# AIML-IfI/openset-imagenet

Hardware: AMD Instinct MI355X
Metric: images/sec (whole node) ResNet-50 + entropic-open-set, Protocol 2, 1/2/4/8 GPUs (higher is better)
Workload: dtype f32; 1 GPU; Protocol 2, ResNet-50, entropic open-set loss, batch 128/GPU; workload_key=p2, classes=30, batch_per_gpu=128, global_batch=128, image=3x224x224, loss=entropic, optimizer=adam lr=1e-3, parallelism=dp1

## Files before the change

### include/osi.h

```cpp
#ifndef OSI_H
#define OSI_H

#include <stddef.h>

#ifdef __cplusplus
extern "C" {
#endif

#define OSI_OK 0
#define OSI_ERR_ARG (-1)
#define OSI_ERR_LAUNCH (-2)
#define OSI_ERR_STATE (-3)

typedef void* osi_stream_t;

int osi_abi_version(void);
const char* osi_build_arch(void);
const char* osi_strerror(int code);
int osi_set_tuning(const char* name, int value);
int osi_get_tuning(const char* name, int* value);

typedef struct {
    int B, H, W, Cin;
    int Ho, Wo, Cout;
    int R, S, stride, pad;
} osi_conv_desc;

enum { OSI_TILE_AUTO = 0, OSI_TILE_128x128 = 1, OSI_TILE_128x64 = 2, OSI_TILE_64x128 = 3, OSI_TILE_64x64 = 4,
       OSI_TILE_64x64_S1 = 5, OSI_TILE_64x128_S1 = 6, OSI_TILE_128x128_S1 = 7, OSI_TILE_128x64_S1 = 8  };

int osi_conv_fwd(const osi_conv_desc* d, const float* x, const float* w, float* y, int tile, osi_stream_t stream);
size_t osi_conv_fwd_bnstats_workspace(const osi_conv_desc* d);
int osi_conv_fwd_bnstats(const osi_conv_desc* d, const float* x, const float* w, float* y, int tile, float* pstats,
                         size_t pstats_bytes, int* P, int* rows_per_block, osi_stream_t stream);
int osi_conv_fwd_act(const osi_conv_desc* d, const float* x, const float* in_scale, const float* in_shift, const float* w, float* y,
                     int tile, float* pstats, size_t pstats_bytes, int* P, int* rows_per_block, osi_stream_t stream);
int osi_conv_fwd_act2(const osi_conv_desc* d, const float* x, const float* in_scale, const float* in_shift, const float* res,
                      const float* w, float* y, int tile, float* pstats, size_t pstats_bytes, int* P, int* rows_per_block,
                      osi_stream_t stream);
int osi_conv_wino_eligible(const osi_conv_desc* d, int input_gradient);
size_t osi_conv_wino_workspace(const osi_conv_desc* d);
size_t osi_conv_wino_weights_bytes(const osi_conv_desc* d);
size_t osi_conv_wino_slab_bytes(void);
int osi_conv_wino_transform_weights(const osi_conv_desc* d, const float* w, int input_gradient, float* u, size_t u_bytes, osi_stream_t stream);
int osi_conv_fwd_wino_pre(const osi_conv_desc* d, const float* x, const float* in_scale, const float* in_shift, const float* u, float* y,
                          void* slab, size_t slab_bytes, float* pstats, size_t pstats_bytes, int* P, int* rows_per_block, osi_stream_t stream);
int osi_conv_fwd_wino(const osi_conv_desc* d, const float* x, const float* in_scale, const float* in_shift, const float* w, float* y,
                      void* ws, size_t ws_bytes, float* pstats, size_t pstats_bytes, int* P, int* rows_per_block, osi_stream_t stream);
typedef struct {
    const float* scale;
    const float* shift;
    const float* residual;
    int relu;
} osi_conv_epilogue;
size_t osi_conv_fwd_epilogue_workspace(const osi_conv_desc* d);
int osi_conv_fwd_epilogue(const osi_conv_desc* d, const float* x, const float* w, float* out, const osi_conv_epilogue* e, void* ws,
                          size_t ws_bytes, osi_stream_t stream);
int osi_conv_fwd_wino_epilogue_pre(const osi_conv_desc* d, const float* x, const float* u, float* out, const osi_conv_epilogue* e, void* slab,
                                   size_t slab_bytes, osi_stream_t stream);
int osi_conv_dgrad(const osi_conv_desc* d, const float* dy, const float* w, float* dx, int accumulate, int tile,
                   osi_stream_t stream);
typedef struct {
    const void* relu_mask;
    const float* y0;
    const float* mean0;
    const float* invstd0;
    const float* y1;
    const float* mean1;
    const float* invstd1;
    float* partials;
    size_t partials_bytes;
    const float* scale0;
    const float* shift0;
    const void* pool_idx;
    int pool_H, pool_W;
    int addend_stride;
} osi_dgrad_fusion;
size_t osi_conv_dgrad_fused_workspace(const osi_conv_desc* d);
int osi_conv_dgrad_fused(const osi_conv_desc* d, const float* dy, const float* w, float* dx, const float* addend,
                         const osi_dgrad_fusion* f, int tile, int* P, osi_stream_t stream);
int osi_conv_dgrad_fused_frozen(const osi_conv_desc* d, const float* dy, const float* w, float* dx, const osi_dgrad_fusion* f, int tile,
                                int* P, osi_stream_t stream);
int osi_conv_dgrad_fused_wino(const osi_conv_desc* d, const float* dy, const float* w, float* dx, const osi_dgrad_fusion* f, void* ws,
                              size_t ws_bytes, int* P, osi_stream_t stream);
int osi_conv_dgrad_fused_wino_pre(const osi_conv_desc* d, const float* dy, const float* u, float* dx, const osi_dgrad_fusion* f, void* slab,
                                  size_t slab_bytes, int* P, osi_stream_t stream);
size_t osi_conv_wgrad_workspace(const osi_conv_desc* d);
int osi_conv_wgrad(const osi_conv_desc* d, const float* dy, const float* x, float* dw, void* ws, size_t ws_bytes,
                   osi_stream_t stream);
int osi_conv_wgrad_act(const osi_conv_desc* d, const float* dy, const float* x, const float* in_scale, const float* in_shift, float* dw,
                       void* ws, size_t ws_bytes, osi_stream_t stream);
size_t osi_conv_wgrad_wino_workspace(const osi_conv_desc* d);
int osi_conv_wgrad_wino(const osi_conv_desc* d, const float* dy, const float* x, const float* in_scale, const float* in_shift, float* dw,
                        void* ws, size_t ws_bytes, osi_stream_t stream);
int osi_stem_weight_pack(const float* w_krsc3, float* w_packed, int Cout, osi_stream_t stream);
size_t osi_stem_wgrad_direct_workspace(const osi_conv_desc* d);
int osi_stem_wgrad_direct(const osi_conv_desc* d, const float* dy, const float* x4, float* dw_krsc3, void* ws, size_t ws_bytes,
                          osi_stream_t stream);
size_t osi_stem_wgrad_fused_workspace(const osi_conv_desc* d);
int osi_stem_wgrad_fused(const osi_conv_desc* d, const float* gpool, const void* pool_idx, const float* y, const float* x4,
                         const float* gamma, const float* mean, const float* invstd, const float* dgamma, const float* dbeta,
                         float* dw_krsc3, void* ws, size_t ws_bytes, osi_stream_t stream);
int osi_stem_grad_unpack(const float* g_packed, float* g_krsc3, int Cout, osi_stream_t stream);
int osi_stem_dgrad(const float* dy, const float* w_krsc3, float* dx_nchw, int B, int H, int W, osi_stream_t stream);
int osi_stem_dgrad_fgsm(const float* dy, const float* w_krsc3, const float* x_nhwc4, float* x_adv_nhwc4, float eps, float lo, float hi,
                        int B, int H, int W, osi_stream_t stream);

size_t osi_bn_workspace(int M, int C);
int osi_bn_train_stats(const float* y, int M, int C, const float* gamma, const float* beta, float eps, float momentum,
                       float* running_mean, float* running_var, float* mean, float* invstd, float* scale, float* shift,
                       void* ws, size_t ws_bytes, osi_stream_t stream);
int osi_bn_finalize_stats(float* pstats, size_t pstats_bytes, int P, int rows_per_block, int M, int C, const float* gamma,
                          const float* beta, float eps, float momentum, float* running_mean, float* running_var, float* mean,
                          float* invstd, float* scale, float* shift, osi_stream_t stream);
int osi_bn_eval_coeffs(const float* running_mean, const float* running_var, const float* gamma, const float* beta, float eps,
                       int C, float* scale, float* shift, osi_stream_t stream);
#define OSI_BN_MULTI_MAX 64
typedef struct {
    const float *running_mean, *running_var, *gamma, *beta;
    float *scale, *shift;
    int C;
} osi_bn_eval_layer;
int osi_bn_eval_coeffs_multi(const osi_bn_eval_layer* layers, int n, float eps, osi_stream_t stream);
#define OSI_BN_FROZEN_MAX 54
typedef struct {
    const float *running_mean, *running_var, *gamma, *beta;
    float *scale, *shift, *mean, *invstd;
    int C;
} osi_bn_frozen_layer;
int osi_bn_frozen_coeffs_multi(const osi_bn_frozen_layer* layers, int n, float eps, osi_stream_t stream);
int osi_bn_apply(const float* y, const float* residual, const float* scale, const float* shift, float* out, int M, int C,
                 int relu, osi_stream_t stream);
size_t osi_bn_backward_workspace(int M, int C);
int osi_bn_backward(const float* dout, const float* act, const float* y, const float* mean, const float* invstd,
                    const float* gamma, float* dy, float* gmasked, float* dgamma, float* dbeta, int M, int C, void* ws,
                    size_t ws_bytes, osi_stream_t stream);

size_t osi_bn_relu_mask_bytes(int M, int C);
int osi_bn_apply_relu_mask(const float* y, const float* residual, const float* scale, const float* shift, float* out,
                           void* relu_mask, int M, int C, osi_stream_t stream);
int osi_bn_apply_relu_mask2(const float* y, const float* scale, const float* shift, const float* res_y, const float* res_scale,
                            const float* res_shift, float* out, void* relu_mask, int M, int C, osi_stream_t stream);
int osi_bn_backward_relu_mask(const float* dout, const void* relu_mask, const float* y, const float* mean, const float* invstd,
                              const float* gamma, float* dy, float* gmasked, float* dgamma, float* dbeta, int M, int C, void* ws,
                              size_t ws_bytes, osi_stream_t stream);

int osi_bn_backward_fused(const float* g, const float* y, const float* mean, const float* invstd, const float* gamma,
                          const float* psum_g, const float* psum_gx, int P, float* dy, float* dgamma, float* dbeta, int M, int C,
                          void* ws, size_t ws_bytes, osi_stream_t stream);

typedef struct {
    const float *y, *mean, *invstd;
    const float* scale;
    float* dy;
    float *dgamma, *dbeta;
} osi_bn_frozen_consumer;
int osi_bn_backward_frozen(const float* dout, const void* relu_mask, const osi_bn_frozen_consumer* consumers, int n, float* gmasked, int M,
                           int C, void* ws, size_t ws_bytes, osi_stream_t stream);

int osi_nchw3_to_nhwc4(const float* x_nchw, float* y_nhwc4, int B, int H, int W, osi_stream_t stream);
int osi_u8hwc3_to_nhwc4(const unsigned char* x_u8_nhwc, const unsigned char* flip, float* y_nhwc4, int B, int H, int W,
                        osi_stream_t stream);
int osi_u8_crop_flip_to_nhwc4(const unsigned char* canvas_u8, const int* crop_xy, const unsigned char* flip, float* y_nhwc4, int B, int Hc,
                              int Wc, int H, int W, osi_stream_t stream);
int osi_maxpool3x3s2_fwd(const float* x, float* y, void* idx, int B, int H, int W, int C, osi_stream_t stream);
int osi_maxpool3x3s2_bwd(const float* dy, const void* idx, float* dx, int B, int H, int W, int C, osi_stream_t stream);
int osi_bn_backward_reduce(const float* psum_g, const float* psum_gx, int P, float* dgamma, float* dbeta, int M, int C, void* ws,
                           size_t ws_bytes, osi_stream_t stream);
int osi_bn_relu_maxpool_fwd(const float* y, const float* scale, const float* shift, float* pooled, void* idx, int B, int H, int W,
                            int C, osi_stream_t stream);
int osi_bn_relu_maxpool_bwd(const float* gpool, const void* idx, const float* y, const float* mean, const float* invstd,
                            const float* gamma, float* dy, float* dgamma, float* dbeta, int B, int H, int W, int C, void* ws,
                            size_t ws_bytes, osi_stream_t stream);
int osi_bn_relu_maxpool_bwd_frozen(const float* gpool, const void* idx, const float* y, const float* mean, const float* invstd,
                                   const float* scale, float* dy, float* dgamma, float* dbeta, int B, int H, int W, int C, void* ws,
                                   size_t ws_bytes, osi_stream_t stream);
int osi_avgpool_fwd(const float* x, float* y, int B, int HW, int C, osi_stream_t stream);
int osi_avgpool_bwd(const float* dy, float* dx, int B, int HW, int C, osi_stream_t stream);

int osi_linear_fwd(const float* x, const float* w, const float* bias, float* y, int B, int K, int O, osi_stream_t stream);
int osi_linear_bwd(const float* dy, const float* x, const float* w, float* dx, int dx_accumulate, float* dw, float* db, int B,
                   int K, int O, osi_stream_t stream);

enum { OSI_LOSS_ENTROPIC = 0, OSI_LOSS_SOFTMAX = 1, OSI_LOSS_GARBAGE = 2 };
int osi_loss_fwd_bwd(int mode, const float* logits, const long long* target, int B, int C, float unk_weight,
                     long long ignore_index, const float* class_weights, const float* features, int F, float xi, float alpha,
                     float* loss, float* dlogits, float* dfeatures, osi_stream_t stream);
int osi_softmax(const float* logits, float* out, int B, int C, osi_stream_t stream);
int osi_confidence_accumulate(const float* logits, const long long* target, int B, int C, float offset, long long unknown_class,
                              int last_valid_class, double* acc4, osi_stream_t stream);
int osi_confidence_from_scores(const float* scores, const long long* target, int B, int C, float offset, long long unknown_class,
                               int last_valid_class, double* acc4, osi_stream_t stream);

size_t osi_oscr_workspace(int N);
int osi_oscr_f32(const float* scores, const long long* gt, int N, int C, long long unk_label, void* ws, size_t ws_bytes,
                 float* taus, long long* ccr_count, long long* fpr_count, long long* totals, osi_stream_t stream);
int osi_oscr_f64(const double* scores, const long long* gt, int N, int C, long long unk_label, void* ws, size_t ws_bytes,
                 double* taus, long long* ccr_count, long long* fpr_count, long long* totals, osi_stream_t stream);

int osi_adam_step(float* param, const float* grad, float* exp_avg, float* exp_avg_sq, size_t n, double lr, double beta1,
                  double beta2, double eps, long long step, float grad_scale, osi_stream_t stream);
int osi_sgd_step(float* param, const float* grad, float* momentum_buf, size_t n, float lr, float momentum, int first_step,
                 float grad_scale, osi_stream_t stream);
#define OSI_OPT_MAX_SEGMENTS 192
#define OSI_OPT_MAX_GROUPS 16
typedef struct {
    unsigned int begin4, end4;
    int group;
} osi_opt_segment;
typedef struct {
    double lr, beta1, beta2, eps, weight_decay;
    long long step;
    int decoupled;
    int amsgrad, maximize;
} osi_adam_group;
typedef struct {
    double lr, momentum, dampening, weight_decay;
    int nesterov;
    int first_step;
    int maximize;
} osi_sgd_group;
int osi_adam_step_groups(float* param, const float* grad, float* exp_avg, float* exp_avg_sq, float* max_exp_avg_sq, size_t n,
                         const osi_opt_segment* segments, int n_segments, const osi_adam_group* groups, int n_groups,
                         float grad_scale, osi_stream_t stream);
int osi_sgd_step_groups(float* param, const float* grad, float* momentum_buf, size_t n, const osi_opt_segment* segments,
                        int n_segments, const osi_sgd_group* groups, int n_groups, float grad_scale, osi_stream_t stream);
int osi_fill_f32(float* p, size_t n, float value, osi_stream_t stream);
int osi_scale_f32(float* p, size_t n, float s, osi_stream_t stream);
int osi_grad_accumulate(float* dst, const float* src, size_t n, osi_stream_t stream);
int osi_i64_add(long long* p, int n, long long inc, osi_stream_t stream);

typedef struct osi_resnet50* osi_resnet50_t;

int osi_resnet50_create(osi_resnet50_t* out, int B, int H, int W, int fc_dim, int out_features, int logit_bias);
void osi_resnet50_destroy(osi_resnet50_t net);
int osi_resnet50_num_tensors(osi_resnet50_t net);
int osi_resnet50_tensor_info(osi_resnet50_t net, int i, char* name, int name_cap, int* ndim, int* shape, size_t* offset,
                             size_t* numel);
size_t osi_resnet50_param_floats(osi_resnet50_t net);
int osi_resnet50_num_bn(osi_resnet50_t net);
int osi_resnet50_bn_info(osi_resnet50_t net, int j, char* prefix, int cap, int* C, size_t* rm_offset, size_t* rv_offset);
size_t osi_resnet50_buffer_floats(osi_resnet50_t net);
size_t osi_resnet50_workspace_bytes(osi_resnet50_t net);
int osi_resnet50_num_stages(osi_resnet50_t net);
int osi_resnet50_geometry(osi_resnet50_t net, int* B, int* H, int* W);
int osi_resnet50_stage_grad_range(osi_resnet50_t net, int s, size_t* lo, size_t* hi);

int osi_resnet50_stage_input_u8(osi_resnet50_t net, const unsigned char* images_u8_nhwc, const unsigned char* flip,
                                void* workspace, osi_stream_t stream);
int osi_resnet50_bind_input_nhwc4(osi_resnet50_t net, const float* x_nhwc4);
int osi_resnet50_forward(osi_resnet50_t net, const float* params, float* buffers, long long* nbt, const float* image,
                         void* workspace, float* logits, float* features, int training, osi_stream_t stream);
int osi_resnet50_forward_frozen(osi_resnet50_t net, const float* params, const float* buffers, const float* image, void* workspace,
                                float* logits, float* features, osi_stream_t stream);
int osi_resnet50_backward(osi_resnet50_t net, const float* params, float* grads, void* workspace, const float* dlogits,
                          const float* dfeatures, int stage_lo, int stage_hi, osi_stream_t stream);

int osi_resnet50_backward_ex(osi_resnet50_t net, const float* params, float* grads, void* workspace, const float* dlogits,
                             const float* dfeatures, float* dimage, int param_grads, int stage_lo, int stage_hi,
                             osi_stream_t stream);

int osi_resnet50_backward_adv(osi_resnet50_t net, const float* params, float* grads, void* workspace, const float* dlogits,
                              const float* dfeatures, float* x_adv_nhwc4, float eps, float lo, float hi, int stage_lo, int stage_hi,
                              osi_stream_t stream);

int osi_resnet50_grads_ready(osi_resnet50_t net, osi_stream_t main_stream, osi_stream_t waiter_stream);

int osi_resnet50_num_units(osi_resnet50_t net);
int osi_resnet50_tensor_unit(osi_resnet50_t net, int i);
int osi_resnet50_bn_unit(osi_resnet50_t net, int j);
int osi_resnet50_set_trainable(osi_resnet50_t net, unsigned unit_mask, int eval_prefix_units);
int osi_resnet50_get_trainable(osi_resnet50_t net, unsigned* unit_mask, int* eval_prefix_units);

int osi_resnet50_set_option(osi_resnet50_t net, const char* name, int value);

enum { OSI_PROF_START = 0, OSI_PROF_CONV_FWD = 1, OSI_PROF_CONV_DGRAD = 2, OSI_PROF_CONV_WGRAD = 3, OSI_PROF_BN_FWD = 4,
       OSI_PROF_BN_BWD = 5, OSI_PROF_OTHER = 6, OSI_PROF_NCLASS = 7 };
int osi_resnet50_profile(osi_resnet50_t net, int enable);
int osi_resnet50_profile_read(osi_resnet50_t net, double* ms_per_class, int* ops_per_class);
int osi_resnet50_timeline_read(osi_resnet50_t net, double* t_ms, int* cls, int* on_side, int cap, int* count);


int osi_resnet50_debug_num_gates(osi_resnet50_t net);
int osi_resnet50_debug_gate_shape(osi_resnet50_t net, int i, int* C, int* H, int* W);
int osi_resnet50_debug_gate(osi_resnet50_t net, void* workspace, int i, unsigned char* gate_nchw, int* pool_argmax_nchw,
                            osi_stream_t stream);

#ifdef __cplusplus
}
#endif
#endif
```

### openset-imagenet_amd/csrc/abi.hip

```cpp
#include "osi_common.h"

#include <cstring>

OsiTuning g_osi_tuning = { 0,  2048,  1,  1024,  128,  2,  768,  0,  0,  2,  1,  0,  8,  16,  1,  8,  8,  1024,  2048,  1,  1,  1,  1,  1,  1,  1,  2,  0};

namespace {
int* tuning_slot(const char* name) {
    if (!name) return nullptr;
    if (!strcmp(name, "wgrad_tile")) return &g_osi_tuning.wgrad_tile;
    if (!strcmp(name, "wgrad_blocks")) return &g_osi_tuning.wgrad_blocks;
    if (!strcmp(name, "wgrad_nst")) return &g_osi_tuning.wgrad_nst;
    if (!strcmp(name, "bn_grid")) return &g_osi_tuning.bn_grid;
    if (!strcmp(name, "bn_single_p")) return &g_osi_tuning.bn_single_p;
    if (!strcmp(name, "wgrad_group")) return &g_osi_tuning.wgrad_group;
    if (!strcmp(name, "wgrad3")) return &g_osi_tuning.wgrad3;
    if (!strcmp(name, "fwd_wide")) return &g_osi_tuning.fwd_wide;
    if (!strcmp(name, "dgrad_wide")) return &g_osi_tuning.dgrad_wide;
    if (!strcmp(name, "wgrad3_blocks")) return &g_osi_tuning.wgrad3_blocks;
    if (!strcmp(name, "tail_split")) return &g_osi_tuning.tail_split;
    if (!strcmp(name, "tail_cus")) return &g_osi_tuning.tail_cus;
    if (!strcmp(name, "tail_smax")) return &g_osi_tuning.tail_smax;
    if (!strcmp(name, "tail_mint")) return &g_osi_tuning.tail_mint;
    if (!strcmp(name, "stem_direct")) return &g_osi_tuning.stem_direct;
    if (!strcmp(name, "bn_wide_p")) return &g_osi_tuning.bn_wide_p;
    if (!strcmp(name, "bn_grid_bwd")) return &g_osi_tuning.bn_grid_bwd;
    if (!strcmp(name, "tail_gain")) return &g_osi_tuning.tail_gain;
    if (!strcmp(name, "tail_qmax")) return &g_osi_tuning.tail_qmax;
    if (!strcmp(name, "dp_reserved_cus")) return &g_osi_tuning.dp_reserved_cus;
    if (!strcmp(name, "fwd_rows")) return &g_osi_tuning.fwd_rows;
    if (!strcmp(name, "fwd_w3")) return &g_osi_tuning.fwd_w3;
    if (!strcmp(name, "dgrad_w3")) return &g_osi_tuning.dgrad_w3;
    if (!strcmp(name, "fwd_wino")) return &g_osi_tuning.fwd_wino;
    if (!strcmp(name, "dgrad_wino")) return &g_osi_tuning.dgrad_wino;
    if (!strcmp(name, "wino_streamk")) return &g_osi_tuning.wino_streamk;
    if (!strcmp(name, "wgrad_wino")) return &g_osi_tuning.wgrad_wino;
    if (!strcmp(name, "wino_wide")) return &g_osi_tuning.wino_wide;
    return nullptr;
}
}

extern "C" {
int osi_abi_version(void) { return 13; }
int osi_set_tuning(const char* name, int value) {
    int* s = tuning_slot(name);
    if (!s) return OSI_ERR_ARG;
    OsiTuning& t = g_osi_tuning;
    auto in = [&](int lo, int hi) { return value >= lo && value <= hi; };
    bool good = true;
    if (s == &t.wgrad_tile) good = value == 0 || value == 64;
    else if (s == &t.wgrad_blocks || s == &t.wgrad3_blocks) good = in(1, 1 << 20);
    else if (s == &t.wgrad_nst) good = in(1, 2);
    else if (s == &t.bn_grid || s == &t.bn_grid_bwd) good = in(1, 1 << 20);
    else if (s == &t.bn_single_p) good = in(1, 1 << 20);
    else if (s == &t.bn_wide_p) good = in(0, 2048);
    else if (s == &t.wgrad3 || s == &t.wgrad_group) good = in(0, 2);
    else if (s == &t.fwd_wide || s == &t.dgrad_wide || s == &t.tail_split || s == &t.stem_direct || s == &t.fwd_w3 || s == &t.dgrad_w3 || s == &t.fwd_wino || s == &t.dgrad_wino || s == &t.wgrad_wino || s == &t.wino_wide) good = in(0, 1);
    else if (s == &t.wino_streamk) good = in(0, 3);
    else if (s == &t.tail_cus) good = in(0, 4096);
    else if (s == &t.tail_smax) good = in(1, 64);
    else if (s == &t.tail_mint) good = in(1, 4096);
    else if (s == &t.tail_gain) good = in(0, 100);
    else if (s == &t.tail_qmax) good = in(0, 4096);
    else if (s == &t.dp_reserved_cus) good = in(0, 128);
    else if (s == &t.fwd_rows) good = in(0, 2);
    if (!good) return OSI_ERR_ARG;
    *s = value;
    return OSI_OK;
}
int osi_get_tuning(const char* name, int* value) {
    int* s = tuning_slot(name);
    if (!s || !value) return OSI_ERR_ARG;
    *value = *s;
    return OSI_OK;
}
const char* osi_build_arch(void) { return "gfx950"; }
const char* osi_strerror(int code) {
    switch (code) {
        case OSI_OK: return "ok";
        case OSI_ERR_ARG: return "invalid argument (shape, pointer or alignment precondition)";
        case OSI_ERR_LAUNCH: return "HIP launch failed";
        case OSI_ERR_STATE: return "executor called out of order, or a plan-relevant tuning knob changed after osi_resnet50_create";
        default: return "unknown error";
    }
}
}
```

### openset-imagenet_amd/csrc/bn.hip

```cpp
#include "osi_common.h"

namespace {

constexpr int NT = 256;
constexpr int OSI_BN_GROUPS = 32;

struct RowSplit { int CV, RL, G; };
__host__ __device__ inline RowSplit row_split(int C) {
    RowSplit s;
    int c4 = C / 4;
    s.CV = c4 < NT ? c4 : NT;
    s.RL = NT / s.CV;
    s.G = (c4 + s.CV - 1) / s.CV;
    return s;
}

__global__ __launch_bounds__(NT) void k_bn_stats_partial(const float* __restrict__ y, int M, int C, int rows_per_blk,
                                                        float* __restrict__ pmean, float* __restrict__ pm2) {
    const int P = gridDim.x;
    __shared__ f32x4 red[2][NT];
    const RowSplit sp = row_split(C);
    const int tid = threadIdx.x;
    const int cv = tid % sp.CV, rl = tid / sp.CV;
    const int r0 = blockIdx.x * rows_per_blk;
    const int r1 = min(M, r0 + rows_per_blk);
    const float n = (float)(r1 - r0);
    const bool active = rl < sp.RL;
    for (int g = 0; g < sp.G; ++g) {
        const int c4 = g * sp.CV + cv;
        const bool colok = active && c4 * 4 < C;
        f32x4 s1 = {0, 0, 0, 0}, s2 = {0, 0, 0, 0}, shift = {0, 0, 0, 0};
        if (colok) {
            const f32x4* base = reinterpret_cast<const f32x4*>(y) + c4;
            const size_t ld = C / 4;
            shift = base[(size_t)r0 * ld];
            int r = r0 + rl;
            for (; r + 3 * sp.RL < r1; r += 4 * sp.RL) {
                f32x4 v0 = base[(size_t)r * ld], v1 = base[(size_t)(r + sp.RL) * ld];
                f32x4 v2 = base[(size_t)(r + 2 * sp.RL) * ld], v3 = base[(size_t)(r + 3 * sp.RL) * ld];
                v0 -= shift; v1 -= shift; v2 -= shift; v3 -= shift;
                s1 += (v0 + v1) + (v2 + v3);
                s2 += (v0 * v0 + v1 * v1) + (v2 * v2 + v3 * v3);
            }
            for (; r < r1; r += sp.RL) {
                f32x4 v = base[(size_t)r * ld] - shift;
                s1 += v; s2 += v * v;
            }
        }
        red[0][tid] = s1; red[1][tid] = s2;
        __syncthreads();
        if (colok && rl == 0) {
            for (int k = 1; k < sp.RL; ++k) { s1 += red[0][k * sp.CV + cv]; s2 += red[1][k * sp.CV + cv]; }
            f32x4 mean = shift + s1 / n;
            f32x4 m2 = s2 - s1 * s1 / n;
#pragma unroll
            for (int k = 0; k < 4; ++k) {
                pmean[(size_t)(c4 * 4 + k) * P + blockIdx.x] = mean[k];
                pm2[(size_t)(c4 * 4 + k) * P + blockIdx.x] = m2[k];
            }
        }
        __syncthreads();
    }
}

__device__ __forceinline__ void bn_finish(int c, float mean, float m2, int M, const float* gamma, const float* beta, float eps,
                                          float momentum, float* running_mean, float* running_var, float* mean_out,
                                          float* invstd_out, float* scale_out, float* shift_out) {
    float var = m2 / (float)M;
    float invstd = 1.0f / sqrtf(var + eps);
    mean_out[c] = mean; invstd_out[c] = invstd;
    float sc = invstd * gamma[c];
    scale_out[c] = sc; shift_out[c] = beta[c] - mean * sc;
    if (running_mean) {
        float unb = M > 1 ? m2 / (float)(M - 1) : var;
        running_mean[c] = (1.f - momentum) * running_mean[c] + momentum * mean;
        running_var[c] = (1.f - momentum) * running_var[c] + momentum * unb;
    }
}
__global__ __launch_bounds__(NT) void k_bn_stats_final_rows(const float* __restrict__ pmean, const float* __restrict__ pm2, int P,
                                                           int rows_per_blk, int M, int C, const float* __restrict__ gamma,
                                                           const float* __restrict__ beta, float eps, float momentum,
                                                           float* running_mean, float* running_var, float* __restrict__ mean_out,
                                                           float* __restrict__ invstd_out, float* __restrict__ scale_out,
                                                           float* __restrict__ shift_out) {
    __shared__ float red[16][16];
    __shared__ float smean[16];
    const int cl = threadIdx.x & 15, pl = threadIdx.x >> 4;
    const int c = blockIdx.x * 16 + cl;
    const bool ok = c < C;
    const int last = P - 1;
    const float nfull = (float)rows_per_blk, nlast = (float)(M - last * rows_per_blk);
    float a0 = 0.f, a1 = 0.f;
    if (ok) {
        int b = pl;
        for (; b + 16 < P; b += 32) {
            a0 += (b == last ? nlast : nfull) * pmean[(size_t)b * C + c];
            a1 += (b + 16 == last ? nlast : nfull) * pmean[(size_t)(b + 16) * C + c];
        }
        if (b < P) a0 += (b == last ? nlast : nfull) * pmean[(size_t)b * C + c];
    }
    red[pl][cl] = a0 + a1;
    __syncthreads();
    if (pl == 0) {
        float s = 0.f;
        for (int k = 0; k < 16; ++k) s += red[k][cl];
        smean[cl] = s / (float)M;
    }
    __syncthreads();
    const float mean = smean[cl];
    a0 = 0.f; a1 = 0.f;
    if (ok) {
        int b = pl;
        for (; b + 16 < P; b += 32) {
            const float d0 = pmean[(size_t)b * C + c] - mean, d1 = pmean[(size_t)(b + 16) * C + c] - mean;
            a0 += pm2[(size_t)b * C + c] + (b == last ? nlast : nfull) * d0 * d0;
            a1 += pm2[(size_t)(b + 16) * C + c] + (b + 16 == last ? nlast : nfull) * d1 * d1;
        }
        if (b < P) { const float d0 = pmean[(size_t)b * C + c] - mean; a0 += pm2[(size_t)b * C + c] + (b == last ? nlast : nfull) * d0 * d0; }
    }
    __syncthreads();
    red[pl][cl] = a0 + a1;
    __syncthreads();
    if (pl == 0 && ok) {
        float m2 = 0.f;
        for (int k = 0; k < 16; ++k) m2 += red[k][cl];
        bn_finish(c, mean, m2, M, gamma, beta, eps, momentum, running_mean, running_var, mean_out, invstd_out, scale_out, shift_out);
    }
}
constexpr int WPL = 64;
__device__ __forceinline__ float wide_reduce(float (*red)[16], float v, int pl, int cl) {
    red[pl][cl] = v;
    __syncthreads();
    float t = 0.f;
    if (pl < 4) {
#pragma unroll
        for (int k = 0; k < 16; ++k) t += red[pl * 16 + k][cl];
    }
    __syncthreads();
    if (pl < 4) red[pl][cl] = t;
    __syncthreads();
    if (pl == 0) t = (red[0][cl] + red[1][cl]) + (red[2][cl] + red[3][cl]);
    __syncthreads();
    return t;
}
__global__ __launch_bounds__(16 * WPL) void k_bn_stats_final_wide(const float* __restrict__ pmean, const float* __restrict__ pm2, int P,
                                                                 int rows_per_blk, int M, int C, const float* __restrict__ gamma,
                                                                 const float* __restrict__ beta, float eps, float momentum,
                                                                 float* running_mean, float* running_var, float* __restrict__ mean_out,
                                                                 float* __restrict__ invstd_out, float* __restrict__ scale_out,
                                                                 float* __restrict__ shift_out) {
    __shared__ float red[WPL][16];
    const int cl = threadIdx.x & 15, pl = threadIdx.x >> 4;
    const int c = min(blockIdx.x * 16 + cl, C - 1);
    const bool ok = blockIdx.x * 16 + cl < C;
    const int last = P - 1;
    const float nfull = (float)rows_per_blk, nlast = (float)(M - last * rows_per_blk);
    const float* pa = pmean + c;
    const float* pb = pm2 + c;
    const float pv = wide_reduce(red, pa[(size_t)min(pl, last) * C], pl, cl) * (1.f / WPL);
    if (pl == 0) red[0][cl] = pv;
    __syncthreads();
    const float pvv = red[0][cl];
    __syncthreads();
    float s1a = 0.f, s1b = 0.f, s2a = 0.f, s2b = 0.f;
    int b = pl;
    for (; b + 3 * WPL < P; b += 4 * WPL) {
        const float m0 = pa[(size_t)b * C], m1 = pa[(size_t)(b + WPL) * C], m2_ = pa[(size_t)(b + 2 * WPL) * C], m3 = pa[(size_t)(b + 3 * WPL) * C];
        const float q0 = pb[(size_t)b * C], q1 = pb[(size_t)(b + WPL) * C], q2 = pb[(size_t)(b + 2 * WPL) * C], q3 = pb[(size_t)(b + 3 * WPL) * C];
        const float d0 = m0 - pvv, d1 = m1 - pvv, d2 = m2_ - pvv, d3 = m3 - pvv;
        const float n3 = b + 3 * WPL == last ? nlast : nfull;
        s1a += nfull * d0; s1b += nfull * d1; s1a += nfull * d2; s1b += n3 * d3;
        s2a += q0 + nfull * d0 * d0; s2b += q1 + nfull * d1 * d1; s2a += q2 + nfull * d2 * d2; s2b += q3 + n3 * d3 * d3;
    }
    for (; b < P; b += WPL) {
        const float d = pa[(size_t)b * C] - pvv, n = b == last ? nlast : nfull;
        s1a += n * d; s2a += pb[(size_t)b * C] + n * d * d;
    }
    const float S1 = wide_reduce(red, s1a + s1b, pl, cl);
    const float S2 = wide_reduce(red, s2a + s2b, pl, cl);
    if (pl == 0 && ok) {
        const float mean = pvv + S1 / (float)M;
        const float m2 = fmaxf(S2 - S1 * S1 / (float)M, 0.f);
        bn_finish(c, mean, m2, M, gamma, beta, eps, momentum, running_mean, running_var, mean_out, invstd_out, scale_out, shift_out);
    }
}
__global__ __launch_bounds__(NT) void k_bn_stats_group(const float* __restrict__ pmean, const float* __restrict__ pm2, int P, int Pc,
                                                      int rows_per_blk, int M, int C, int S, float* __restrict__ gmean,
                                                      float* __restrict__ gm2) {
    __shared__ float red[2][16][16];
    const int cl = threadIdx.x & 15, pl = threadIdx.x >> 4;
    const int c = min(blockIdx.x * 16 + cl, C - 1), s = blockIdx.y;
    const bool ok = blockIdx.x * 16 + cl < C;
    const int b0 = s * Pc, b1 = min(P, b0 + Pc), last = P - 1;
    const float nfull = (float)rows_per_blk, nlast = (float)(M - last * rows_per_blk);
    const float ng = (float)(min(M, b1 * rows_per_blk) - b0 * rows_per_blk);
    const float* pa = pmean + c;
    const float* pb = pm2 + c;
    red[0][pl][cl] = pa[(size_t)min(b0 + pl, b1 - 1) * C];
    __syncthreads();
    float pv = 0.f;
#pragma unroll
    for (int k = 0; k < 16; ++k) pv += red[0][k][cl];
    pv *= 1.f / 16.f;
    __syncthreads();
    float s1a = 0.f, s1b = 0.f, s2a = 0.f, s2b = 0.f;
    int b = b0 + pl;
    for (; b + 48 < b1; b += 64) {
        const float m0 = pa[(size_t)b * C], m1 = pa[(size_t)(b + 16) * C], m2_ = pa[(size_t)(b + 32) * C], m3 = pa[(size_t)(b + 48) * C];
        const float q0 = pb[(size_t)b * C], q1 = pb[(size_t)(b + 16) * C], q2 = pb[(size_t)(b + 32) * C], q3 = pb[(size_t)(b + 48) * C];
        const float d0 = m0 - pv, d1 = m1 - pv, d2 = m2_ - pv, d3 = m3 - pv;
        const float n3 = b + 48 == last ? nlast : nfull;
        s1a += nfull * d0; s1b += nfull * d1; s1a += nfull * d2; s1b += n3 * d3;
        s2a += q0 + nfull * d0 * d0; s2b += q1 + nfull * d1 * d1; s2a += q2 + nfull * d2 * d2; s2b += q3 + n3 * d3 * d3;
    }
    for (; b < b1; b += 16) {
        const float d = pa[(size_t)b * C] - pv, n = b == last ? nlast : nfull;
        s1a += n * d; s2a += pb[(size_t)b * C] + n * d * d;
    }
    red[0][pl][cl] = s1a + s1b; red[1][pl][cl] = s2a + s2b;
    __syncthreads();
    if (pl == 0 && ok) {
        float S1 = 0.f, S2 = 0.f;
#pragma unroll
        for (int k = 0; k < 16; ++k) { S1 += red[0][k][cl]; S2 += red[1][k][cl]; }
        gmean[(size_t)c * S + s] = pv + S1 / ng;
        gm2[(size_t)c * S + s] = fmaxf(S2 - S1 * S1 / ng, 0.f);
    }
}
__global__ __launch_bounds__(NT) void k_bn_stats_final(const float* __restrict__ pmean, const float* __restrict__ pm2, int P,
                                                      int rows_per_blk, int M, int C, const float* __restrict__ gamma,
                                                      const float* __restrict__ beta, float eps, float momentum,
                                                      float* running_mean, float* running_var, float* __restrict__ mean_out,
                                                      float* __restrict__ invstd_out, float* __restrict__ scale_out,
                                                      float* __restrict__ shift_out) {
    const int lane = threadIdx.x & 63;
    const int c = blockIdx.x * (NT / 64) + (threadIdx.x >> 6);
    if (c >= C) return;
    float n = 0.f, mean = 0.f, m2 = 0.f;
    for (int b = lane; b < P; b += 64) {
        const float nb = (float)min(rows_per_blk, M - b * rows_per_blk);
        chan_merge(n, mean, m2, nb, pmean[(size_t)c * P + b], pm2[(size_t)c * P + b]);
    }
#pragma unroll
    for (int o = 1; o < 64; o <<= 1) {
        const float nb = __shfl_xor(n, o, 64), mb = __shfl_xor(mean, o, 64), sb = __shfl_xor(m2, o, 64);
        if (lane & o) { float na = nb, ma = mb, sa = sb; chan_merge(na, ma, sa, n, mean, m2); n = na; mean = ma; m2 = sa; }
        else chan_merge(n, mean, m2, nb, mb, sb);
    }
    if (lane == 0)
        bn_finish(c, mean, m2, M, gamma, beta, eps, momentum, running_mean, running_var, mean_out, invstd_out, scale_out, shift_out);
}

__global__ void k_bn_eval_coeffs(const float* rm, const float* rv, const float* gamma, const float* beta, float eps, int C,
                                 float* scale, float* shift) {
    int c = blockIdx.x * blockDim.x + threadIdx.x;
    if (c >= C) return;
    float sc = gamma[c] * (1.0f / sqrtf(rv[c] + eps));
    scale[c] = sc; shift[c] = beta[c] - rm[c] * sc;
}

struct BnEvalTable { osi_bn_eval_layer l[OSI_BN_MULTI_MAX]; };
__global__ void k_bn_eval_coeffs_multi(BnEvalTable t, float eps) {
    const osi_bn_eval_layer& L = t.l[blockIdx.y];
    const int c = blockIdx.x * blockDim.x + threadIdx.x;
    if (c >= L.C) return;
    const float sc = L.gamma[c] * (1.0f / sqrtf(L.running_var[c] + eps));
    L.scale[c] = sc; L.shift[c] = L.beta[c] - L.running_mean[c] * sc;
}

struct BnFrozenTable { osi_bn_frozen_layer l[OSI_BN_FROZEN_MAX]; };
__global__ void k_bn_frozen_coeffs_multi(BnFrozenTable t, float eps) {
    const osi_bn_frozen_layer& L = t.l[blockIdx.y];
    const int c = blockIdx.x * blockDim.x + threadIdx.x;
    if (c >= L.C) return;
    const float is = 1.0f / sqrtf(L.running_var[c] + eps);
    const float sc = L.gamma[c] * is;
    L.scale[c] = sc; L.shift[c] = L.beta[c] - L.running_mean[c] * sc;
    L.mean[c] = L.running_mean[c]; L.invstd[c] = is;
}

typedef unsigned long long u64;
#ifndef OSI_BN_REVERSE
#define OSI_BN_REVERSE 3
#endif
template <int RES, bool RELU, bool BITS>
__global__ __launch_bounds__(NT) void k_bn_apply(const f32x4* __restrict__ y, const f32x4* __restrict__ res,
                                                const f32x4* __restrict__ scale, const f32x4* __restrict__ shift,
                                                const f32x4* __restrict__ rscale, const f32x4* __restrict__ rshift,
                                                f32x4* __restrict__ out, u64* __restrict__ bits, size_t n4, int c4n) {
    const size_t nq = (n4 + NT - 1) / NT;
    for (size_t q = blockIdx.x; q < nq; q += gridDim.x) {
        const size_t i = ((OSI_BN_REVERSE & 1) ? nq - 1 - q : q) * NT + threadIdx.x;
        if (i >= n4) continue;
        int c4 = (int)(i % (size_t)c4n);
        const f32x4 yv = __builtin_nontemporal_load(y + i), sc = scale[c4], sh = shift[c4];
        f32x4 v;
#pragma unroll
        for (int e = 0; e < 4; ++e) v[e] = __builtin_fmaf(yv[e], sc[e], sh[e]);
        if (RES == 1) v += __builtin_nontemporal_load(res + i);
        if (RES == 2) {
            const f32x4 rv = __builtin_nontemporal_load(res + i), rs = rscale[c4], rh = rshift[c4];
            f32x4 t;
#pragma unroll
            for (int e = 0; e < 4; ++e) t[e] = __builtin_fmaf(rv[e], rs[e], rh[e]);
            v += t;
        }
        if (BITS) {
            const u64 b0 = __ballot(v.x > 0.f), b1 = __ballot(v.y > 0.f), b2 = __ballot(v.z > 0.f), b3 = __ballot(v.w > 0.f);
            if ((threadIdx.x & 63) == 0) {
                u64* w = bits + (i >> 6) * 4;
                w[0] = b0; w[1] = b1; w[2] = b2; w[3] = b3;
            }
        }
        if (RELU) { v.x = fmaxf(v.x, 0.f); v.y = fmaxf(v.y, 0.f); v.z = fmaxf(v.z, 0.f); v.w = fmaxf(v.w, 0.f); }
        out[i] = v;
    }
}
__device__ __forceinline__ f32x4 mask_by_bits(f32x4 g, const u64* __restrict__ bits, size_t i) {
    const u64* w = bits + (i >> 6) * 4;
    const int b = (int)(i & 63);
    g.x = (w[0] >> b) & 1 ? g.x : 0.f; g.y = (w[1] >> b) & 1 ? g.y : 0.f;
    g.z = (w[2] >> b) & 1 ? g.z : 0.f; g.w = (w[3] >> b) & 1 ? g.w : 0.f;
    return g;
}

template <int MODE>
__device__ __forceinline__ f32x4 masked(f32x4 gv, const void* m, size_t i) {
    if (MODE == 1) {
        f32x4 a = reinterpret_cast<const f32x4*>(m)[i];
        gv.x = a.x > 0.f ? gv.x : 0.f; gv.y = a.y > 0.f ? gv.y : 0.f;
        gv.z = a.z > 0.f ? gv.z : 0.f; gv.w = a.w > 0.f ? gv.w : 0.f;
    } else if (MODE == 2) {
        gv = mask_by_bits(gv, reinterpret_cast<const u64*>(m), i);
    }
    return gv;
}
struct PoolSrc {
    const uint32_t* idx;
    FastDiv dW, dH;
    int H, W, Ho, Wo;
};
__device__ __forceinline__ f32x4 pool_gather(const f32x4* __restrict__ gp, const PoolSrc& ps, uint32_t pix, int c4, int c4n) {
    const uint32_t row = fdiv(pix, ps.dW);
    const int w = (int)(pix - row * ps.dW.d);
    const uint32_t b = fdiv(row, ps.dH);
    const int h = (int)(row - b * ps.dH.d);
    f32x4 acc = {0, 0, 0, 0};
    for (int ho = h >> 1; ho <= (h + 1) >> 1; ++ho) {
        if (ho >= ps.Ho) continue;
        const int r = h - (ho * 2 - 1);
        for (int wo = w >> 1; wo <= (w + 1) >> 1; ++wo) {
            if (wo >= ps.Wo) continue;
            const int s = w - (wo * 2 - 1);
            const size_t o = ((size_t)(b * ps.Ho + ho) * ps.Wo + wo) * c4n + c4;
            const uint32_t id = ps.idx[o];
            const f32x4 g = gp[o];
            const uint32_t me = (uint32_t)(r * 3 + s) | 0x80u;
#pragma unroll
            for (int k = 0; k < 4; ++k)
                if (((id >> (8 * k)) & 0xffu) == me) acc[k] += g[k];
        }
    }
    return acc;
}

template <int MODE>
__global__ __launch_bounds__(NT) void k_bn_bwd_partial(const float* __restrict__ dA, const void* __restrict__ msk,
                                                      const float* __restrict__ y, const float* __restrict__ mean,
                                                      const float* __restrict__ invstd, int M, int C, int rows_per_blk,
                                                      float* __restrict__ pdb, float* __restrict__ pdg, PoolSrc ps) {
    __shared__ f32x4 red[2][NT];
    const int P = gridDim.x;
    const RowSplit sp = row_split(C);
    const int tid = threadIdx.x;
    const int cv = tid % sp.CV, rl = tid / sp.CV;
    const int r0 = blockIdx.x * rows_per_blk;
    const int r1 = min(M, r0 + rows_per_blk);
    const bool active = rl < sp.RL;
    const size_t ld = C / 4;
    for (int g = 0; g < sp.G; ++g) {
        const int c4 = g * sp.CV + cv;
        const bool colok = active && c4 * 4 < C;
        f32x4 sb = {0, 0, 0, 0}, sg = {0, 0, 0, 0}, sb2 = {0, 0, 0, 0}, sg2 = {0, 0, 0, 0};
        if (colok) {
            const f32x4 mu = reinterpret_cast<const f32x4*>(mean)[c4];
            const f32x4 is = reinterpret_cast<const f32x4*>(invstd)[c4];
            const f32x4* pd = reinterpret_cast<const f32x4*>(dA);
            const f32x4* py = reinterpret_cast<const f32x4*>(y);
            int r = r0 + rl;
            for (; r + sp.RL < r1; r += 2 * sp.RL) {
                const size_t i0 = (size_t)r * ld + c4, i1 = (size_t)(r + sp.RL) * ld + c4;
                f32x4 g0, g1, y0 = py[i0], y1 = py[i1];
                if (MODE == 3) {
                    g0 = pool_gather(pd, ps, (uint32_t)r, c4, (int)ld); g1 = pool_gather(pd, ps, (uint32_t)(r + sp.RL), c4, (int)ld);
                } else {
                    g0 = masked<MODE>(pd[i0], msk, i0); g1 = masked<MODE>(pd[i1], msk, i1);
                }
                sb += g0; sg += g0 * ((y0 - mu) * is);
                sb2 += g1; sg2 += g1 * ((y1 - mu) * is);
            }
            for (; r < r1; r += sp.RL) {
                const size_t i0 = (size_t)r * ld + c4;
                f32x4 g0 = MODE == 3 ? pool_gather(pd, ps, (uint32_t)r, c4, (int)ld) : masked<MODE>(pd[i0], msk, i0);
                sb += g0; sg += g0 * ((py[i0] - mu) * is);
            }
            sb += sb2; sg += sg2;
        }
        red[0][tid] = sb; red[1][tid] = sg;
        __syncthreads();
        if (colok && rl == 0) {
            for (int k = 1; k < sp.RL; ++k) { sb += red[0][k * sp.CV + cv]; sg += red[1][k * sp.CV + cv]; }
#pragma unroll
            for (int k = 0; k < 4; ++k) {
                pdb[(size_t)(c4 * 4 + k) * P + blockIdx.x] = sb[k];
                pdg[(size_t)(c4 * 4 + k) * P + blockIdx.x] = sg[k];
            }
        }
        __syncthreads();
    }
}

__global__ __launch_bounds__(NT) void k_bn_bwd_final(const float* __restrict__ pdb, const float* __restrict__ pdg, int P, int M,
                                                    int C, float* __restrict__ dgamma, float* __restrict__ dbeta,
                                                    float* __restrict__ c1, float* __restrict__ c2) {
    const int lane = threadIdx.x & 63;
    const int c = blockIdx.x * (NT / 64) + (threadIdx.x >> 6);
    if (c >= C) return;
    float ab = 0.f, ag = 0.f;
    for (int b = lane; b < P; b += 64) { ab += pdb[(size_t)c * P + b]; ag += pdg[(size_t)c * P + b]; }
    ab = wave_sum(ab); ag = wave_sum(ag);
    if (lane == 0) {
        dbeta[c] = ab; dgamma[c] = ag;
        c1[c] = ab / (float)M; c2[c] = ag / (float)M;
    }
}

__global__ __launch_bounds__(NT) void k_colsum2_group(const float* __restrict__ a, const float* __restrict__ b, int P, int Pc, int C,
                                                     int S, float* __restrict__ ga, float* __restrict__ gb) {
    __shared__ float ra[16][16], rb[16][16];
    const int cl = threadIdx.x & 15, pl = threadIdx.x >> 4;
    const int c = min(blockIdx.x * 16 + cl, C - 1), s = blockIdx.y;
    const bool ok = blockIdx.x * 16 + cl < C;
    const int b0 = s * Pc, b1 = min(P, b0 + Pc);
    const float* pa = a + c;
    const float* pb = b + c;
    float xa0 = 0.f, xa1 = 0.f, xb0 = 0.f, xb1 = 0.f;
    int r = b0 + pl;
    for (; r + 48 < b1; r += 64) {
        const float a0 = pa[(size_t)r * C], a1 = pa[(size_t)(r + 16) * C], a2 = pa[(size_t)(r + 32) * C], a3 = pa[(size_t)(r + 48) * C];
        const float v0 = pb[(size_t)r * C], v1 = pb[(size_t)(r + 16) * C], v2 = pb[(size_t)(r + 32) * C], v3 = pb[(size_t)(r + 48) * C];
        xa0 += a0; xa1 += a1; xa0 += a2; xa1 += a3;
        xb0 += v0; xb1 += v1; xb0 += v2; xb1 += v3;
    }
    for (; r < b1; r += 16) { xa0 += pa[(size_t)r * C]; xb0 += pb[(size_t)r * C]; }
    float xa = xa0 + xa1, xb = xb0 + xb1;
    ra[pl][cl] = xa; rb[pl][cl] = xb;
    __syncthreads();
    if (pl == 0 && ok) {
        for (int k = 1; k < 16; ++k) { xa += ra[k][cl]; xb += rb[k][cl]; }
        ga[(size_t)c * S + s] = xa; gb[(size_t)c * S + s] = xb;
    }
}

__global__ __launch_bounds__(16 * WPL) void k_bn_bwd_final_wide(const float* __restrict__ a, const float* __restrict__ b, int P, int M, int C,
                                                               float* __restrict__ dgamma, float* __restrict__ dbeta,
                                                               float* __restrict__ c1, float* __restrict__ c2) {
    __shared__ float red[WPL][16];
    const int cl = threadIdx.x & 15, pl = threadIdx.x >> 4;
    const int c = min(blockIdx.x * 16 + cl, C - 1);
    const bool ok = blockIdx.x * 16 + cl < C;
    const float* pa = a + c;
    const float* pb = b + c;
    float xa0 = 0.f, xa1 = 0.f, xb0 = 0.f, xb1 = 0.f;
    int r = pl;
    for (; r + 3 * WPL < P; r += 4 * WPL) {
        const float a0 = pa[(size_t)r * C], a1 = pa[(size_t)(r + WPL) * C], a2 = pa[(size_t)(r + 2 * WPL) * C], a3 = pa[(size_t)(r + 3 * WPL) * C];
        const float b0 = pb[(size_t)r * C], b1 = pb[(size_t)(r + WPL) * C], b2 = pb[(size_t)(r + 2 * WPL) * C], b3 = pb[(size_t)(r + 3 * WPL) * C];
        xa0 += a0; xa1 += a1; xa0 += a2; xa1 += a3;
        xb0 += b0; xb1 += b1; xb0 += b2; xb1 += b3;
    }
    for (; r < P; r += WPL) { xa0 += pa[(size_t)r * C]; xb0 += pb[(size_t)r * C]; }
    const float sa = wide_reduce(red, xa0 + xa1, pl, cl);
    const float sb = wide_reduce(red, xb0 + xb1, pl, cl);
    if (pl == 0 && ok) {
        dbeta[c] = sa; dgamma[c] = sb;
        c1[c] = sa / (float)M; c2[c] = sb / (float)M;
    }
}

template <int MODE, bool EMITG>
__global__ __launch_bounds__(NT) void k_bn_bwd_apply(const f32x4* dA , const void* __restrict__ msk,
                                                    const f32x4* __restrict__ y, const f32x4* __restrict__ mean,
                                                    const f32x4* __restrict__ invstd, const f32x4* __restrict__ gamma,
                                                    const f32x4* __restrict__ c1, const f32x4* __restrict__ c2,
                                                    f32x4* dy, f32x4* __restrict__ gout, size_t n4, int c4n, PoolSrc ps) {
    const size_t nq = (n4 + NT - 1) / NT;
    for (size_t q = blockIdx.x; q < nq; q += gridDim.x) {
        const size_t i = ((OSI_BN_REVERSE & 2) ? nq - 1 - q : q) * NT + threadIdx.x;
        if (i >= n4) continue;
        int c4 = (int)(i % (size_t)c4n);
        f32x4 gv = MODE == 3 ? pool_gather(dA, ps, (uint32_t)(i / (size_t)c4n), c4, c4n) : masked<MODE>(__builtin_nontemporal_load(dA + i), msk, i);
        f32x4 is = invstd[c4];
        f32x4 xh = (__builtin_nontemporal_load(y + i) - mean[c4]) * is;
        f32x4 r = (gv - c1[c4] - xh * c2[c4]) * (gamma[c4] * is);
        if (EMITG) gout[i] = gv;
        dy[i] = r;
    }
}

template <int MODE, bool EMITG, bool TWO>
__global__ __launch_bounds__(NT) void k_bn_frozen_apply(const f32x4* dA, const void* __restrict__ msk, const f32x4* __restrict__ scale0,
                                                       const f32x4* __restrict__ scale1, f32x4* dy0, f32x4* __restrict__ dy1,
                                                       f32x4* __restrict__ gout, size_t n4, int c4n, PoolSrc ps) {
    const size_t nq = (n4 + NT - 1) / NT;
    for (size_t q = blockIdx.x; q < nq; q += gridDim.x) {
        const size_t i = ((OSI_BN_REVERSE & 2) ? nq - 1 - q : q) * NT + threadIdx.x;
        if (i >= n4) continue;
        const int c4 = (int)(i % (size_t)c4n);
        const f32x4 gv = MODE == 3 ? pool_gather(dA, ps, (uint32_t)(i / (size_t)c4n), c4, c4n) : masked<MODE>(__builtin_nontemporal_load(dA + i), msk, i);
        if (EMITG) gout[i] = gv;
        if (TWO) dy1[i] = gv * scale1[c4];
        dy0[i] = gv * scale0[c4];
    }
}

static int rows_per_block(int M, int C, int& P) {
    long rows = (256l * 1024) / ((long)C * 4);
    if (rows < 8) rows = 8;
    long minrows = (M + 1023) / 1024;
    if (rows < minrows) rows = minrows;
    if (rows > M) rows = M;
    P = (int)((M + rows - 1) / rows);
    return (int)rows;
}
static int stream_grid(size_t n4, bool backward = false) {
    const size_t cap = (size_t)(backward ? g_osi_tuning.bn_grid_bwd : g_osi_tuning.bn_grid);
    size_t g = (n4 + NT - 1) / NT;
    return (int)(g > cap ? cap : g);
}

}

extern "C" {

size_t osi_bn_workspace(int M, int C) {
    if (M <= 0 || C <= 0) return 0;
    int P;
    rows_per_block(M, C, P);
    return (size_t)2 * P * C * sizeof(float);
}

int osi_bn_train_stats(const float* y, int M, int C, const float* gamma, const float* beta, float eps, float momentum,
                       float* running_mean, float* running_var, float* mean, float* invstd, float* scale, float* shift,
                       void* ws, size_t ws_bytes, osi_stream_t stream) {
    OSI_REQUIRE(y && gamma && beta && mean && invstd && scale && shift && ws);
    OSI_REQUIRE(M > 0 && C > 0 && C % 4 == 0);
    OSI_REQUIRE((running_mean == nullptr) == (running_var == nullptr));
    int P;
    int rpb = rows_per_block(M, C, P);
    OSI_REQUIRE(ws_bytes >= (size_t)2 * P * C * sizeof(float));
    hipStream_t st = (hipStream_t)stream;
    float* pmean = (float*)ws;
    float* pm2 = pmean + (size_t)P * C;
    hipLaunchKernelGGL(k_bn_stats_partial, dim3(P), dim3(NT), 0, st, y, M, C, rpb, pmean, pm2);
    OSI_LAUNCH_CHECK();
    hipLaunchKernelGGL(k_bn_stats_final, dim3(osi_cdiv(C, NT / 64)), dim3(NT), 0, st, pmean, pm2, P, rpb, M, C, gamma, beta, eps,
                       momentum, running_mean, running_var, mean, invstd, scale, shift);
    OSI_LAUNCH_CHECK();
    return OSI_OK;
}

int osi_bn_finalize_stats(float* pstats, size_t pstats_bytes, int P, int rows_per_block, int M, int C, const float* gamma,
                          const float* beta, float eps, float momentum, float* running_mean, float* running_var, float* mean,
                          float* invstd, float* scale, float* shift, osi_stream_t stream) {
    OSI_REQUIRE(pstats && gamma && beta && mean && invstd && scale && shift);
    OSI_REQUIRE(P > 0 && rows_per_block > 0 && M > 0 && C > 0 && (long)(P - 1) * rows_per_block < M && (long)P * rows_per_block >= M);
    OSI_REQUIRE((running_mean == nullptr) == (running_var == nullptr));
    OSI_REQUIRE(pstats_bytes >= ((size_t)2 * P * C + 2 * (size_t)OSI_BN_GROUPS * C) * sizeof(float));
    hipStream_t st = (hipStream_t)stream;
    const float* pmean = pstats;
    const float* pm2 = pstats + (size_t)P * C;
    if (P <= g_osi_tuning.bn_single_p) {
        hipLaunchKernelGGL(k_bn_stats_final_rows, dim3(osi_cdiv(C, 16)), dim3(NT), 0, st, pmean, pm2, P, rows_per_block, M, C, gamma,
                           beta, eps, momentum, running_mean, running_var, mean, invstd, scale, shift);
        OSI_LAUNCH_CHECK();
        return OSI_OK;
    }
    if (P <= g_osi_tuning.bn_wide_p) {
        hipLaunchKernelGGL(k_bn_stats_final_wide, dim3(osi_cdiv(C, 16)), dim3(16 * WPL), 0, st, pmean, pm2, P, rows_per_block, M, C, gamma,
                           beta, eps, momentum, running_mean, running_var, mean, invstd, scale, shift);
        OSI_LAUNCH_CHECK();
        return OSI_OK;
    }
    int S = osi_cdiv(P, 64);
    if (S > OSI_BN_GROUPS) S = OSI_BN_GROUPS;
    const int Pc = osi_cdiv(P, S);
    S = osi_cdiv(P, Pc);
    float* gmean = pstats + (size_t)2 * P * C;
    float* gm2 = gmean + (size_t)S * C;
    hipLaunchKernelGGL(k_bn_stats_group, dim3(osi_cdiv(C, 16), S), dim3(NT), 0, st, pmean, pm2, P, Pc, rows_per_block, M, C, S, gmean, gm2);
    OSI_LAUNCH_CHECK();
    hipLaunchKernelGGL(k_bn_stats_final, dim3(osi_cdiv(C, NT / 64)), dim3(NT), 0, st, (const float*)gmean, (const float*)gm2, S,
                       Pc * rows_per_block, M, C, gamma, beta, eps, momentum, running_mean, running_var, mean, invstd, scale, shift);
    OSI_LAUNCH_CHECK();
    return OSI_OK;
}

int osi_bn_eval_coeffs(const float* running_mean, const float* running_var, const float* gamma, const float* beta, float eps,
                       int C, float* scale, float* shift, osi_stream_t stream) {
    OSI_REQUIRE(running_mean && running_var && gamma && beta && scale && shift && C > 0);
    hipLaunchKernelGGL(k_bn_eval_coeffs, dim3(osi_cdiv(C, 256)), dim3(256), 0, (hipStream_t)stream, running_mean, running_var,
                       gamma, beta, eps, C, scale, shift);
    OSI_LAUNCH_CHECK();
    return OSI_OK;
}

int osi_bn_eval_coeffs_multi(const osi_bn_eval_layer* layers, int n, float eps, osi_stream_t stream) {
    OSI_REQUIRE(layers && n > 0 && n <= OSI_BN_MULTI_MAX);
    BnEvalTable t{};
    int cmax = 0;
    for (int i = 0; i < n; ++i) {
        const osi_bn_eval_layer& L = layers[i];
        OSI_REQUIRE(L.running_mean && L.running_var && L.gamma && L.beta && L.scale && L.shift && L.C > 0);
        t.l[i] = L;
        if (L.C > cmax) cmax = L.C;
    }
    hipLaunchKernelGGL(k_bn_eval_coeffs_multi, dim3(osi_cdiv(cmax, 256), n), dim3(256), 0, (hipStream_t)stream, t, eps);
    OSI_LAUNCH_CHECK();
    return OSI_OK;
}

int osi_bn_frozen_coeffs_multi(const osi_bn_frozen_layer* layers, int n, float eps, osi_stream_t stream) {
    OSI_REQUIRE(layers && n > 0 && n <= OSI_BN_FROZEN_MAX);
    BnFrozenTable t{};
    int cmax = 0;
    for (int i = 0; i < n; ++i) {
        const osi_bn_frozen_layer& L = layers[i];
        OSI_REQUIRE(L.running_mean && L.running_var && L.gamma && L.beta && L.scale && L.shift && L.mean && L.invstd && L.C > 0);
        t.l[i] = L;
        if (L.C > cmax) cmax = L.C;
    }
    hipLaunchKernelGGL(k_bn_frozen_coeffs_multi, dim3(osi_cdiv(cmax, 256), n), dim3(256), 0, (hipStream_t)stream, t, eps);
    OSI_LAUNCH_CHECK();
    return OSI_OK;
}

static int bn_apply_impl(const float* y, const float* residual, const float* scale, const float* shift, float* out, void* bits,
                         int M, int C, int relu, hipStream_t st, const float* rscale = nullptr, const float* rshift = nullptr) {
    OSI_REQUIRE(y && scale && shift && out && M > 0 && C > 0 && C % 4 == 0);
    OSI_REQUIRE(!bits || relu);
    OSI_REQUIRE((rscale == nullptr) == (rshift == nullptr) && (!rscale || (residual && bits)));
    const size_t n4 = (size_t)M * C / 4;
    const int grid = stream_grid(n4), c4n = C / 4;
    auto Y = (const f32x4*)y; auto R = (const f32x4*)residual; auto S = (const f32x4*)scale; auto H = (const f32x4*)shift;
    auto RS = (const f32x4*)rscale; auto RH = (const f32x4*)rshift;
    auto O = (f32x4*)out; auto B = (u64*)bits;
#define OSI_APPLY(RES_, RELU_, BITS_) hipLaunchKernelGGL((k_bn_apply<RES_, RELU_, BITS_>), dim3(grid), dim3(NT), 0, st, Y, R, S, H, RS, RH, O, B, n4, c4n)
    if (rscale) OSI_APPLY(2, true, true);
    else if (bits && residual) OSI_APPLY(1, true, true);
    else if (bits) OSI_APPLY(0, true, true);
    else if (residual && relu) OSI_APPLY(1, true, false);
    else if (residual) OSI_APPLY(1, false, false);
    else if (relu) OSI_APPLY(0, true, false);
    else OSI_APPLY(0, false, false);
#undef OSI_APPLY
    OSI_LAUNCH_CHECK();
    return OSI_OK;
}

int osi_bn_apply(const float* y, const float* residual, const float* scale, const float* shift, float* out, int M, int C,
                 int relu, osi_stream_t stream) {
    return bn_apply_impl(y, residual, scale, shift, out, nullptr, M, C, relu, (hipStream_t)stream);
}

size_t osi_bn_relu_mask_bytes(int M, int C) {
    if (M <= 0 || C <= 0) return 0;
    const size_t n4 = (size_t)M * C / 4;
    return (n4 + 63) / 64 * 4 * sizeof(u64);
}

int osi_bn_apply_relu_mask(const float* y, const float* residual, const float* scale, const float* shift, float* out,
                           void* relu_mask, int M, int C, osi_stream_t stream) {
    OSI_REQUIRE(relu_mask);
    return bn_apply_impl(y, residual, scale, shift, out, relu_mask, M, C, 1, (hipStream_t)stream);
}

int osi_bn_apply_relu_mask2(const float* y, const float* scale, const float* shift, const float* res_y, const float* res_scale,
                            const float* res_shift, float* out, void* relu_mask, int M, int C, osi_stream_t stream) {
    OSI_REQUIRE(relu_mask && res_y && res_scale && res_shift);
    return bn_apply_impl(y, res_y, scale, shift, out, relu_mask, M, C, 1, (hipStream_t)stream, res_scale, res_shift);
}

static int bn_backward_impl(const float* dout, const void* msk, int mode, const float* y, const float* mean, const float* invstd,
                            const float* gamma, float* dy, float* gmasked, float* dgamma, float* dbeta, int M, int C, void* ws,
                            size_t ws_bytes, hipStream_t st, PoolSrc ps = PoolSrc{}) {
    OSI_REQUIRE(dout && y && mean && invstd && gamma && (dy || mode == 3) && dgamma && dbeta && ws);
    OSI_REQUIRE(M > 0 && C > 0 && C % 4 == 0);
    int P;
    int rpb = rows_per_block(M, C, P);
    OSI_REQUIRE(ws_bytes >= ((size_t)2 * P * C + 2 * (size_t)C) * sizeof(float));
    float* pdb = (float*)ws;
    float* pdg = pdb + (size_t)P * C;
    float* c1 = pdg + (size_t)P * C;
    float* c2 = c1 + C;
    if (mode == 3) hipLaunchKernelGGL(k_bn_bwd_partial<3>, dim3(P), dim3(NT), 0, st, dout, msk, y, mean, invstd, M, C, rpb, pdb, pdg, ps);
    else if (mode == 2) hipLaunchKernelGGL(k_bn_bwd_partial<2>, dim3(P), dim3(NT), 0, st, dout, msk, y, mean, invstd, M, C, rpb, pdb, pdg, ps);
    else if (mode == 1) hipLaunchKernelGGL(k_bn_bwd_partial<1>, dim3(P), dim3(NT), 0, st, dout, msk, y, mean, invstd, M, C, rpb, pdb, pdg, ps);
    else hipLaunchKernelGGL(k_bn_bwd_partial<0>, dim3(P), dim3(NT), 0, st, dout, msk, y, mean, invstd, M, C, rpb, pdb, pdg, ps);
    OSI_LAUNCH_CHECK();
    hipLaunchKernelGGL(k_bn_bwd_final, dim3(osi_cdiv(C, NT / 64)), dim3(NT), 0, st, pdb, pdg, P, M, C, dgamma, dbeta, c1, c2);
    OSI_LAUNCH_CHECK();
    if (!dy) return OSI_OK;
    const size_t n4 = (size_t)M * C / 4;
    const int grid = stream_grid(n4, true), c4n = C / 4;
    auto D = (const f32x4*)dout; auto Y = (const f32x4*)y;
    auto MU = (const f32x4*)mean; auto IS = (const f32x4*)invstd; auto G = (const f32x4*)gamma;
    auto C1 = (const f32x4*)c1; auto C2 = (const f32x4*)c2;
    auto DY = (f32x4*)dy; auto GO = (f32x4*)gmasked;
#define OSI_BWD_APPLY(MODE_, EMIT_) hipLaunchKernelGGL((k_bn_bwd_apply<MODE_, EMIT_>), dim3(grid), dim3(NT), 0, st, D, msk, Y, MU, IS, G, C1, C2, DY, GO, n4, c4n, ps)
    if (mode == 3) OSI_BWD_APPLY(3, false);
    else if (mode == 2) { if (gmasked) OSI_BWD_APPLY(2, true); else OSI_BWD_APPLY(2, false); }
    else if (mode == 1) { if (gmasked) OSI_BWD_APPLY(1, true); else OSI_BWD_APPLY(1, false); }
    else { if (gmasked) OSI_BWD_APPLY(0, true); else OSI_BWD_APPLY(0, false); }
#undef OSI_BWD_APPLY
    OSI_LAUNCH_CHECK();
    return OSI_OK;
}

static int bwd_reduce_partials(const float* psum_g, const float* psum_gx, int P, int M, int C, float* gb, float* gg, int S, int Pc,
                               float* dgamma, float* dbeta, float* c1, float* c2, hipStream_t st) {
    if (P <= g_osi_tuning.bn_wide_p) {
        hipLaunchKernelGGL(k_bn_bwd_final_wide, dim3(osi_cdiv(C, 16)), dim3(16 * WPL), 0, st, psum_g, psum_gx, P, M, C, dgamma, dbeta, c1, c2);
        OSI_LAUNCH_CHECK();
        return OSI_OK;
    }
    hipLaunchKernelGGL(k_colsum2_group, dim3(osi_cdiv(C, 16), S), dim3(NT), 0, st, psum_g, psum_gx, P, Pc, C, S, gb, gg);
    OSI_LAUNCH_CHECK();
    hipLaunchKernelGGL(k_bn_bwd_final, dim3(osi_cdiv(C, NT / 64)), dim3(NT), 0, st, (const float*)gb, (const float*)gg, S, M, C, dgamma,
                       dbeta, c1, c2);
    OSI_LAUNCH_CHECK();
    return OSI_OK;
}

int osi_bn_backward_fused(const float* g, const float* y, const float* mean, const float* invstd, const float* gamma,
                          const float* psum_g, const float* psum_gx, int P, float* dy, float* dgamma, float* dbeta, int M, int C,
                          void* ws, size_t ws_bytes, osi_stream_t stream) {
    OSI_REQUIRE(g && y && mean && invstd && gamma && psum_g && psum_gx && dy && dgamma && dbeta && ws);
    OSI_REQUIRE(M > 0 && C > 0 && C % 4 == 0 && P > 0);
    int S = osi_cdiv(P, 64);
    if (S > OSI_BN_GROUPS) S = OSI_BN_GROUPS;
    const int Pc = osi_cdiv(P, S);
    S = osi_cdiv(P, Pc);
    OSI_REQUIRE(ws_bytes >= ((size_t)2 * S * C + 2 * (size_t)C) * sizeof(float));
    hipStream_t st = (hipStream_t)stream;
    float* gb = (float*)ws;
    float* gg = gb + (size_t)S * C;
    float* c1 = gg + (size_t)S * C;
    float* c2 = c1 + C;
    if (int e = bwd_reduce_partials(psum_g, psum_gx, P, M, C, gb, gg, S, Pc, dgamma, dbeta, c1, c2, st)) return e;
    const size_t n4 = (size_t)M * C / 4;
    hipLaunchKernelGGL((k_bn_bwd_apply<0, false>), dim3(stream_grid(n4, true)), dim3(NT), 0, st, (const f32x4*)g, (const void*)nullptr,
                       (const f32x4*)y, (const f32x4*)mean, (const f32x4*)invstd, (const f32x4*)gamma, (const f32x4*)c1,
                       (const f32x4*)c2, (f32x4*)dy, (f32x4*)nullptr, n4, C / 4, PoolSrc{});
    OSI_LAUNCH_CHECK();
    return OSI_OK;
}

int osi_bn_backward_reduce(const float* psum_g, const float* psum_gx, int P, float* dgamma, float* dbeta, int M, int C, void* ws,
                           size_t ws_bytes, osi_stream_t stream) {
    OSI_REQUIRE(psum_g && psum_gx && dgamma && dbeta && ws && M > 0 && C > 0 && P > 0);
    int S = osi_cdiv(P, 64);
    if (S > OSI_BN_GROUPS) S = OSI_BN_GROUPS;
    const int Pc = osi_cdiv(P, S);
    S = osi_cdiv(P, Pc);
    OSI_REQUIRE(ws_bytes >= ((size_t)2 * S * C + 2 * (size_t)C) * sizeof(float));
    hipStream_t st = (hipStream_t)stream;
    float* gb = (float*)ws;
    float* gg = gb + (size_t)S * C;
    float* c1 = gg + (size_t)S * C;
    float* c2 = c1 + C;
    if (int e = bwd_reduce_partials(psum_g, psum_gx, P, M, C, gb, gg, S, Pc, dgamma, dbeta, c1, c2, st)) return e;
    return OSI_OK;
}

static int bn_frozen_impl(const float* dout, const void* msk, int mode, const osi_bn_frozen_consumer* cs, int n, float* gmasked, int M, int C,
                          void* ws, size_t ws_bytes, hipStream_t st, PoolSrc ps = PoolSrc{}) {
    OSI_REQUIRE(dout && cs && (n == 1 || n == 2) && M > 0 && C > 0 && C % 4 == 0);
    OSI_REQUIRE(mode != 3 || (n == 1 && !gmasked));
    for (int k = 0; k < n; ++k) {
        OSI_REQUIRE(cs[k].scale && cs[k].dy && (cs[k].dgamma == nullptr) == (cs[k].dbeta == nullptr));
        if (cs[k].dgamma) {
            int P;
            rows_per_block(M, C, P);
            OSI_REQUIRE(cs[k].y && cs[k].mean && cs[k].invstd && ws && ws_bytes >= ((size_t)2 * P * C + 2 * (size_t)C) * sizeof(float));
        }
    }
    OSI_REQUIRE(n == 1 || (cs[1].dy != cs[0].dy && cs[1].dy != dout));
    for (int k = 0; k < n; ++k) {
        if (!cs[k].dgamma) continue;
        int P;
        const int rpb = rows_per_block(M, C, P);
        float* pdb = (float*)ws;
        float* pdg = pdb + (size_t)P * C;
        float* c1 = pdg + (size_t)P * C;
        if (mode == 3) hipLaunchKernelGGL(k_bn_bwd_partial<3>, dim3(P), dim3(NT), 0, st, dout, msk, cs[k].y, cs[k].mean, cs[k].invstd, M, C, rpb, pdb, pdg, ps);
        else if (mode == 2) hipLaunchKernelGGL(k_bn_bwd_partial<2>, dim3(P), dim3(NT), 0, st, dout, msk, cs[k].y, cs[k].mean, cs[k].invstd, M, C, rpb, pdb, pdg, ps);
        else hipLaunchKernelGGL(k_bn_bwd_partial<0>, dim3(P), dim3(NT), 0, st, dout, msk, cs[k].y, cs[k].mean, cs[k].invstd, M, C, rpb, pdb, pdg, ps);
        OSI_LAUNCH_CHECK();
        hipLaunchKernelGGL(k_bn_bwd_final, dim3(osi_cdiv(C, NT / 64)), dim3(NT), 0, st, pdb, pdg, P, M, C, cs[k].dgamma, cs[k].dbeta, c1, c1 + C);
        OSI_LAUNCH_CHECK();
    }
    const size_t n4 = (size_t)M * C / 4;
    const int grid = stream_grid(n4, true), c4n = C / 4;
    auto D = (const f32x4*)dout; auto S0 = (const f32x4*)cs[0].scale; auto S1 = (const f32x4*)(n == 2 ? cs[1].scale : nullptr);
    auto DY0 = (f32x4*)cs[0].dy; auto DY1 = (f32x4*)(n == 2 ? cs[1].dy : nullptr); auto GO = (f32x4*)gmasked;
#define OSI_FRZ_APPLY(MODE_, EMIT_, TWO_) hipLaunchKernelGGL((k_bn_frozen_apply<MODE_, EMIT_, TWO_>), dim3(grid), dim3(NT), 0, st, D, msk, S0, S1, DY0, DY1, GO, n4, c4n, ps)
    if (mode == 3) OSI_FRZ_APPLY(3, false, false);
    else if (mode == 2) {
        if (n == 2) { if (gmasked) OSI_FRZ_APPLY(2, true, true); else OSI_FRZ_APPLY(2, false, true); }
        else { if (gmasked) OSI_FRZ_APPLY(2, true, false); else OSI_FRZ_APPLY(2, false, false); }
    } else {
        if (n == 2) { if (gmasked) OSI_FRZ_APPLY(0, true, true); else OSI_FRZ_APPLY(0, false, true); }
        else { if (gmasked) OSI_FRZ_APPLY(0, true, false); else OSI_FRZ_APPLY(0, false, false); }
    }
#undef OSI_FRZ_APPLY
    OSI_LAUNCH_CHECK();
    return OSI_OK;
}

int osi_bn_backward_frozen(const float* dout, const void* relu_mask, const osi_bn_frozen_consumer* consumers, int n, float* gmasked, int M,
                           int C, void* ws, size_t ws_bytes, osi_stream_t stream) {
    return bn_frozen_impl(dout, relu_mask, relu_mask ? 2 : 0, consumers, n, gmasked, M, C, ws, ws_bytes, (hipStream_t)stream);
}

int osi_bn_relu_maxpool_bwd_frozen(const float* gpool, const void* idx, const float* y, const float* mean, const float* invstd,
                                   const float* scale, float* dy, float* dgamma, float* dbeta, int B, int H, int W, int C, void* ws,
                                   size_t ws_bytes, osi_stream_t stream) {
    OSI_REQUIRE(idx && B > 0 && H > 0 && W > 0 && (long)B * H * W < (1l << 31));
    PoolSrc ps;
    ps.idx = (const uint32_t*)idx;
    ps.dW = make_fastdiv((uint32_t)W); ps.dH = make_fastdiv((uint32_t)H);
    ps.H = H; ps.W = W; ps.Ho = (H + 2 - 3) / 2 + 1; ps.Wo = (W + 2 - 3) / 2 + 1;
    const osi_bn_frozen_consumer c{y, mean, invstd, scale, dy, dgamma, dbeta};
    return bn_frozen_impl(gpool, nullptr, 3, &c, 1, nullptr, B * H * W, C, ws, ws_bytes, (hipStream_t)stream, ps);
}

int osi_bn_relu_maxpool_bwd(const float* gpool, const void* idx, const float* y, const float* mean, const float* invstd,
                            const float* gamma, float* dy, float* dgamma, float* dbeta, int B, int H, int W, int C, void* ws,
                            size_t ws_bytes, osi_stream_t stream) {
    OSI_REQUIRE(idx && B > 0 && H > 0 && W > 0 && (long)B * H * W < (1l << 31));
    PoolSrc ps;
    ps.idx = (const uint32_t*)idx;
    ps.dW = make_fastdiv((uint32_t)W); ps.dH = make_fastdiv((uint32_t)H);
    ps.H = H; ps.W = W; ps.Ho = (H + 2 - 3) / 2 + 1; ps.Wo = (W + 2 - 3) / 2 + 1;
    return bn_backward_impl(gpool, nullptr, 3, y, mean, invstd, gamma, dy, nullptr, dgamma, dbeta, B * H * W, C, ws, ws_bytes,
                            (hipStream_t)stream, ps);
}

int osi_bn_backward(const float* dout, const float* act, const float* y, const float* mean, const float* invstd,
                    const float* gamma, float* dy, float* gmasked, float* dgamma, float* dbeta, int M, int C, void* ws,
                    size_t ws_bytes, osi_stream_t stream) {
    return bn_backward_impl(dout, act, act ? 1 : 0, y, mean, invstd, gamma, dy, gmasked, dgamma, dbeta, M, C, ws, ws_bytes,
                            (hipStream_t)stream);
}

int osi_bn_backward_relu_mask(const float* dout, const void* relu_mask, const float* y, const float* mean, const float* invstd,
                              const float* gamma, float* dy, float* gmasked, float* dgamma, float* dbeta, int M, int C, void* ws,
                              size_t ws_bytes, osi_stream_t stream) {
    OSI_REQUIRE(relu_mask);
    return bn_backward_impl(dout, relu_mask, 2, y, mean, invstd, gamma, dy, gmasked, dgamma, dbeta, M, C, ws, ws_bytes,
                            (hipStream_t)stream);
}

size_t osi_bn_backward_workspace(int M, int C) {
    if (M <= 0 || C <= 0) return 0;
    int P;
    rows_per_block(M, C, P);
    return ((size_t)2 * P * C + 2 * (size_t)C) * sizeof(float);
}

}
```

### openset-imagenet_amd/csrc/resnet50_exec.hip

```cpp
#include "osi_common.h"
#include <string>
#include <vector>
#include <cstring>
#include <cstdio>

#define OSI_TRY(x)                 \
    do {                           \
        int e__ = (x);             \
        if (e__ != OSI_OK) return e__; \
    } while (0)

namespace {

struct Tensor {
    std::string name;
    int ndim; int shape[4];
    size_t off, numel;
    int unit;
};
struct BN {
    std::string prefix;
    int C, M;
    size_t g_off, b_off;
    size_t rm_off, rv_off;
    size_t mean, invstd, scale, shift;
    size_t dsink;
    int unit;
};
struct Conv {
    osi_conv_desc d;
    size_t w_off;
    int bn;
    size_t y;
    size_t a;
    size_t mask;
    size_t u_fw = (size_t)-1, u_bw = (size_t)-1;
    int unit;
};
struct Block {
    int c1, c2, c3, ds;
    size_t x_in;
    size_t out;
    int stage;
};

constexpr size_t ALIGN_F = 64;
constexpr unsigned EV_FLAGS = hipEventDisableTiming | hipEventDisableSystemFence;
constexpr unsigned EV_FLAGS_HANDOFF = hipEventDisableTiming;
static size_t up(size_t v, size_t a) { return (v + a - 1) / a * a; }
static int device_cus() {
    int v = 0, dev = 0;
    if (hipGetDevice(&dev) != hipSuccess || hipDeviceGetAttribute(&v, hipDeviceAttributeMultiprocessorCount, dev) != hipSuccess) return 0;
    return v;
}

}

struct osi_resnet50 {
    int B, H, W, F, O, logit_bias;
    std::vector<Tensor> tensors;
    std::vector<BN> bns;
    std::vector<Conv> convs;
    std::vector<Block> blocks;
    size_t param_floats = 0, buffer_floats = 0, ws_floats = 0;
    int t_fc_w, t_fc_b, t_lg_w, t_lg_b;
    int Hs, Ws, Hp, Wp;
    size_t x4, wpack, gpack, a_pool, pool_idx, pooled, feat, logits_ws;
    size_t bn_ws, bn_ws2, bn_ws_bytes, wg_ws, wg_ws_bytes, dg_ws, dg_ws_bytes;
    size_t stem_ws = 0, stem_ws_bytes = 0;
    size_t wino_ws = 0, wino_ws_bytes = 0;
    static constexpr int NSCR = 12;
    size_t scratch[NSCR], scratch_floats;
    size_t dfeat, dpooled;
    int Hf, Wf;
    int n_stages = 4;
    size_t stage_lo[4], stage_hi[4];
    bool fwd_done = false;
    bool any_fwd = false;
    int next_stage = 0;
    int cur_grad = -1;
    bool go_fused = false;
    int fused_P = 0;
    std::vector<int> free_list;
    bool prof_on = false;
    bool prof_timeline = false;
    std::vector<int> prof_side;
    std::vector<hipEvent_t> prof_ev;
    std::vector<int> prof_cls;
    int prof_n = 0;
    int mark(int cls, hipStream_t st) {
        if (!prof_on) return OSI_OK;
        if (prof_n == (int)prof_ev.size()) {
            hipEvent_t e;
            if (hipEventCreate(&e) != hipSuccess) return OSI_ERR_LAUNCH;
            prof_ev.push_back(e); prof_cls.push_back(0); prof_side.push_back(0);
        }
        prof_cls[prof_n] = cls;
        prof_side[prof_n] = (side != nullptr && st == side) ? 1 : 0;
        if (hipEventRecord(prof_ev[prof_n], st) != hipSuccess) return OSI_ERR_LAUNCH;
        ++prof_n;
        return OSI_OK;
    }

    static constexpr int NUNITS = 18;
    int cur_unit = 0;
    unsigned unit_mask = (1u << NUNITS) - 1;
    int eval_prefix = 0;
    int fw_prefix = 0;
    bool trainable(int unit) const { return (unit_mask >> unit) & 1u; }
    int cut() const { int c = 0; while (!((unit_mask >> c) & 1u)) ++c; return c; }
    int bw_stop() const { return (bw_pg && !bw_dimage && !bw_adv) ? cut() : 0; }

    size_t add_tensor(const std::string& name, int ndim, const int* shape) {
        Tensor t; t.name = name; t.ndim = ndim; t.numel = 1;
        for (int i = 0; i < 4; ++i) t.shape[i] = i < ndim ? shape[i] : 1;
        for (int i = 0; i < ndim; ++i) t.numel *= (size_t)shape[i];
        t.off = param_floats;
        t.unit = cur_unit;
        param_floats = up(param_floats + t.numel, 4);
        tensors.push_back(t);
        return t.off;
    }
    size_t ws_alloc(size_t floats) {
        size_t o = ws_floats;
        ws_floats = up(ws_floats + floats, ALIGN_F);
        return o;
    }
    int add_conv_bn(const std::string& cname, const std::string& bname, int Bn, int Hin, int Win, int Cin, int Cout, int k, int s,
                    int pad, bool keep_act) {
        Conv c{};
        c.d.B = Bn; c.d.H = Hin; c.d.W = Win; c.d.Cin = Cin; c.d.Cout = Cout; c.d.R = k; c.d.S = k; c.d.stride = s; c.d.pad = pad;
        c.d.Ho = (Hin + 2 * pad - k) / s + 1; c.d.Wo = (Win + 2 * pad - k) / s + 1;
        int shp[4] = {Cout, Cin == 4 && k == 7 ? 3 : Cin, k, k};
        c.w_off = add_tensor(cname + ".weight", 4, shp);
        BN b; b.prefix = bname; b.C = Cout; b.M = Bn * c.d.Ho * c.d.Wo;
        int s1[1] = {Cout};
        b.g_off = add_tensor(bname + ".weight", 1, s1);
        b.b_off = add_tensor(bname + ".bias", 1, s1);
        b.rm_off = buffer_floats; buffer_floats += up(Cout, 4);
        b.rv_off = buffer_floats; buffer_floats += up(Cout, 4);
        b.mean = ws_alloc(Cout); b.invstd = ws_alloc(Cout); b.scale = ws_alloc(Cout); b.shift = ws_alloc(Cout);
        b.unit = c.unit = cur_unit;
        c.bn = (int)bns.size();
        bns.push_back(b);
        size_t n = (size_t)b.M * Cout;
        c.y = ws_alloc(n);
        c.a = keep_act ? ws_alloc(n) : (size_t)-1;
        c.mask = keep_act ? ws_alloc(osi_bn_relu_mask_bytes(b.M, Cout) / sizeof(float)) : (size_t)-1;
        convs.push_back(c);
        return (int)convs.size() - 1;
    }
    void* staged_ws = nullptr;
    bool overlap = true;
    bool fwd_fork = true;
    bool side_prio_normal = false;
    const float* x4_ext = nullptr;
    const float* x4_cur = nullptr;
    int stem_stats_P = 0;
    float* bw_dimage = nullptr;
    bool bw_pg = true;
    float* bw_adv = nullptr;
    float bw_eps = 0.f, bw_lo = 0.f, bw_hi = 0.f;
    float* dgam(float* grads, float* ws, const BN& b) const { return bw_pg && trainable(b.unit) ? grads + b.g_off : ws + b.dsink; }
    float* dbet(float* grads, float* ws, const BN& b) const { return bw_pg && trainable(b.unit) ? grads + b.b_off : ws + b.dsink + b.C; }
    bool stem_tail_fused() const { return !frozen && !bw_dimage && !bw_adv && stem_ws_bytes > 0; }
    bool frozen = false;
    bool eval_fused = true;
    bool stage_join = true;
    OsiTuning plan_knobs;
    int plan_hw_cus = 0;
    bool plan_unchanged() const {
        const OsiTuning &a = plan_knobs, &b = g_osi_tuning;
        return plan_hw_cus == device_cus() && a.wgrad_tile == b.wgrad_tile && a.wgrad_blocks == b.wgrad_blocks && a.wgrad3 == b.wgrad3 && a.wgrad3_blocks == b.wgrad3_blocks &&
               a.tail_split == b.tail_split && a.tail_cus == b.tail_cus && a.tail_smax == b.tail_smax && a.tail_mint == b.tail_mint &&
               a.tail_gain == b.tail_gain && a.tail_qmax == b.tail_qmax && a.stem_direct == b.stem_direct && a.wgrad_group == b.wgrad_group &&
               a.dp_reserved_cus == b.dp_reserved_cus && a.fwd_wino == b.fwd_wino && a.dgrad_wino == b.dgrad_wino && a.wgrad_wino == b.wgrad_wino;
    }
    hipStream_t side = nullptr;
    hipEvent_t ev_fork = nullptr, ev_join = nullptr, ev_rmain = nullptr, ev_rside = nullptr, ev_wt = nullptr;
    bool wt_pending = false;
    hipEvent_t buf_ev[NSCR] = {};
    bool buf_pending[NSCR] = {};
    bool side_dirty = false;
    int ensure_side() {
        if (side) return OSI_OK;
        int lo = 0, hi = 0;
        if (hipDeviceGetStreamPriorityRange(&lo, &hi) != hipSuccess) return OSI_ERR_LAUNCH;
        const int prio = side_prio_normal ? 0 : lo;
        if (hipStreamCreateWithPriority(&side, hipStreamNonBlocking, prio) != hipSuccess) return OSI_ERR_LAUNCH;
        if (hipEventCreateWithFlags(&ev_fork, EV_FLAGS) != hipSuccess) return OSI_ERR_LAUNCH;
        if (hipEventCreateWithFlags(&ev_join, EV_FLAGS) != hipSuccess) return OSI_ERR_LAUNCH;
        if (hipEventCreateWithFlags(&ev_wt, EV_FLAGS) != hipSuccess) return OSI_ERR_LAUNCH;
        for (int i = 0; i < NSCR; ++i)
            if (hipEventCreateWithFlags(&buf_ev[i], EV_FLAGS) != hipSuccess) return OSI_ERR_LAUNCH;
        return OSI_OK;
    }
    bool async_wgrad() const { return overlap && (!prof_on || prof_timeline) && side != nullptr; }
    int take(hipStream_t st) {
        if (free_list.empty()) return OSI_ERR_STATE;
        int i = free_list.front(); free_list.erase(free_list.begin());
        if (buf_pending[i]) {
            if (hipStreamWaitEvent(st, buf_ev[i], 0) != hipSuccess) return OSI_ERR_LAUNCH;
            buf_pending[i] = false;
        }
        return i;
    }
    void give(int i) { free_list.push_back(i); }
    int fork_side(hipStream_t st) {
        if (hipEventRecord(ev_fork, st) != hipSuccess) return OSI_ERR_LAUNCH;
        if (hipStreamWaitEvent(side, ev_fork, 0) != hipSuccess) return OSI_ERR_LAUNCH;
        return OSI_OK;
    }
    int wait_weight_transforms(hipStream_t st) {
        if (!wt_pending) return OSI_OK;
        if (hipStreamWaitEvent(st, ev_wt, 0) != hipSuccess) return OSI_ERR_LAUNCH;
        wt_pending = false;
        return OSI_OK;
    }
    int join_side(hipStream_t st) {
        if (!side_dirty) return OSI_OK;
        if (hipEventRecord(ev_join, side) != hipSuccess) return OSI_ERR_LAUNCH;
        if (hipStreamWaitEvent(st, ev_join, 0) != hipSuccess) return OSI_ERR_LAUNCH;
        for (int i = 0; i < NSCR; ++i) buf_pending[i] = false;
        side_dirty = false;
        return OSI_OK;
    }
    ~osi_resnet50() {
        for (hipEvent_t e : prof_ev) (void)hipEventDestroy(e);
        if (side) {
            (void)hipStreamSynchronize(side);
            (void)hipEventDestroy(ev_fork); (void)hipEventDestroy(ev_join); (void)hipEventDestroy(ev_wt);
            for (int i = 0; i < NSCR; ++i) (void)hipEventDestroy(buf_ev[i]);
            (void)hipStreamDestroy(side);
        }
        if (ev_rmain) (void)hipEventDestroy(ev_rmain);
        if (ev_rside) (void)hipEventDestroy(ev_rside);
    }
};

extern "C" {

int osi_resnet50_create(osi_resnet50_t* out, int B, int H, int W, int fc_dim, int out_features, int logit_bias) {
    OSI_REQUIRE(out && B > 0 && H >= 32 && W >= 32 && fc_dim > 0 && out_features > 0);
    osi_resnet50* n = new osi_resnet50();
    n->B = B; n->H = H; n->W = W; n->F = fc_dim; n->O = out_features; n->logit_bias = logit_bias ? 1 : 0;
    const std::string rb = "resnet_base.";
    n->x4 = n->ws_alloc((size_t)B * H * W * 4);
    n->wpack = n->ws_alloc(64 * 224);
    n->gpack = n->ws_alloc(64 * 224);
    n->cur_unit = 0;
    int stem = n->add_conv_bn(rb + "conv1", rb + "bn1", B, H, W, 4, 64, 7, 2, 3, false);
    n->Hs = n->convs[stem].d.Ho; n->Ws = n->convs[stem].d.Wo;
    n->Hp = (n->Hs + 2 - 3) / 2 + 1; n->Wp = (n->Ws + 2 - 3) / 2 + 1;
    n->a_pool = n->ws_alloc((size_t)B * n->Hp * n->Wp * 64);
    n->pool_idx = n->ws_alloc((size_t)B * n->Hp * n->Wp * 64 / 4);
    const int planes[4] = {64, 128, 256, 512}, nblk[4] = {3, 4, 6, 3}, strides[4] = {1, 2, 2, 2};
    int inpl = 64, h = n->Hp, w = n->Wp;
    size_t x = n->a_pool;
    for (int s = 0; s < 4; ++s) {
        size_t lo = n->param_floats;
        for (int b = 0; b < nblk[s]; ++b) {
            const std::string pre = rb + "layer" + std::to_string(s + 1) + "." + std::to_string(b) + ".";
            const int st = b == 0 ? strides[s] : 1;
            Block blk{};
            n->cur_unit = (int)n->blocks.size() + 1;
            blk.x_in = x; blk.stage = 3 - s;
            blk.c1 = n->add_conv_bn(pre + "conv1", pre + "bn1", B, h, w, inpl, planes[s], 1, 1, 0, false);
            blk.c2 = n->add_conv_bn(pre + "conv2", pre + "bn2", B, h, w, planes[s], planes[s], 3, st, 1, false);
            const int ho = n->convs[blk.c2].d.Ho, wo = n->convs[blk.c2].d.Wo;
            blk.c3 = n->add_conv_bn(pre + "conv3", pre + "bn3", B, ho, wo, planes[s], planes[s] * 4, 1, 1, 0, true);
            blk.ds = -1;
            if (b == 0) blk.ds = n->add_conv_bn(pre + "downsample.0", pre + "downsample.1", B, h, w, inpl, planes[s] * 4, 1, st, 0, false);
            blk.out = n->convs[blk.c3].a;
            n->blocks.push_back(blk);
            x = blk.out; inpl = planes[s] * 4; h = ho; w = wo;
        }
        n->stage_lo[3 - s] = lo; n->stage_hi[3 - s] = n->param_floats;
    }
    n->stage_lo[3] = 0;
    n->Hf = h; n->Wf = w;
    n->cur_unit = osi_resnet50::NUNITS - 1;
    { int shp[2] = {fc_dim, 2048}; n->t_fc_w = (int)n->tensors.size(); n->add_tensor(rb + "fc.weight", 2, shp); }
    { int shp[1] = {fc_dim}; n->t_fc_b = (int)n->tensors.size(); n->add_tensor(rb + "fc.bias", 1, shp); }
    { int shp[2] = {out_features, fc_dim}; n->t_lg_w = (int)n->tensors.size(); n->add_tensor("logits.weight", 2, shp); }
    n->t_lg_b = -1;
    if (n->logit_bias) { int shp[1] = {out_features}; n->t_lg_b = (int)n->tensors.size(); n->add_tensor("logits.bias", 1, shp); }
    n->stage_hi[0] = n->param_floats;
    n->pooled = n->ws_alloc((size_t)B * 2048);
    n->feat = n->ws_alloc((size_t)B * fc_dim);
    n->logits_ws = n->ws_alloc((size_t)B * out_features);
    n->dfeat = n->ws_alloc((size_t)B * fc_dim);
    n->dpooled = n->ws_alloc((size_t)B * 2048);
    size_t maxact = 0, bnws = 0, wgws = 0, dgws = 0, winows = 0;
    for (auto& c : n->convs) {
        size_t e = (size_t)c.d.B * c.d.Ho * c.d.Wo * c.d.Cout;
        if (e > maxact) maxact = e;
        size_t ein = (size_t)c.d.B * c.d.H * c.d.W * c.d.Cin;
        if (ein > maxact) maxact = ein;
        size_t b1 = osi_bn_workspace(n->bns[c.bn].M, c.d.Cout), b2 = osi_bn_backward_workspace(n->bns[c.bn].M, c.d.Cout);
        if (b1 > bnws) bnws = b1;
        if (b2 > bnws) bnws = b2;
        size_t b3 = osi_conv_fwd_bnstats_workspace(&c.d);
        if (b3 > bnws) bnws = b3;
        size_t wg = osi_conv_wgrad_workspace(&c.d);
        if (wg > wgws) wgws = wg;
        wg = osi_stem_wgrad_direct_workspace(&c.d);
        if (wg > wgws) wgws = wg;
        wg = osi_conv_wgrad_wino_workspace(&c.d);
        if (wg > wgws) wgws = wg;
        if (!(c.d.Cin == 4 && c.d.R == 7)) { size_t dg = osi_conv_dgrad_fused_workspace(&c.d); if (dg > dgws) dgws = dg; }
        if (osi_conv_wino_eligible(&c.d, 0) || osi_conv_wino_eligible(&c.d, 1)) {
            const size_t Pw = ((size_t)c.d.B * ((c.d.H + 1) / 2) * ((c.d.W + 1) / 2) + 15) / 16;
            if (osi_conv_wino_eligible(&c.d, 0)) c.u_fw = n->ws_alloc(osi_conv_wino_weights_bytes(&c.d) / sizeof(float));
            if (osi_conv_wino_eligible(&c.d, 1)) c.u_bw = n->ws_alloc(osi_conv_wino_weights_bytes(&c.d) / sizeof(float));
            size_t w = osi_conv_wino_slab_bytes();
            if (w > winows) winows = w;
            w = (2 * Pw + 64) * c.d.Cout * sizeof(float);
            if (w > bnws) bnws = w;
            w = 3 * Pw * c.d.Cin * sizeof(float);
            if (w > dgws) dgws = w;
        }
    }
    n->wino_ws_bytes = winows; n->wino_ws = n->ws_alloc(winows / 4 + 4);
    n->bn_ws_bytes = bnws; n->bn_ws = n->ws_alloc(bnws / 4 + 4); n->bn_ws2 = n->ws_alloc(bnws / 4 + 4);
    n->wg_ws_bytes = wgws; n->wg_ws = n->ws_alloc(wgws / 4 + 4);
    n->stem_ws_bytes = osi_stem_wgrad_fused_workspace(&n->convs[0].d);
    n->stem_ws = n->stem_ws_bytes ? n->ws_alloc(n->stem_ws_bytes / 4 + 4) : n->wg_ws;
    n->plan_knobs = g_osi_tuning;
    n->plan_hw_cus = device_cus();
    n->dg_ws_bytes = dgws; n->dg_ws = n->ws_alloc(dgws / 4 + 4);
    n->scratch_floats = maxact;
    for (int i = 0; i < osi_resnet50::NSCR; ++i) n->scratch[i] = n->ws_alloc(maxact);
    for (auto& b : n->bns) b.dsink = n->ws_alloc(2 * (size_t)b.C);
    *out = n;
    return OSI_OK;
}

void osi_resnet50_destroy(osi_resnet50_t net) { delete net; }
int osi_resnet50_num_tensors(osi_resnet50_t net) { return net ? (int)net->tensors.size() : 0; }
size_t osi_resnet50_param_floats(osi_resnet50_t net) { return net ? net->param_floats : 0; }
int osi_resnet50_num_bn(osi_resnet50_t net) { return net ? (int)net->bns.size() : 0; }
size_t osi_resnet50_buffer_floats(osi_resnet50_t net) { return net ? net->buffer_floats : 0; }
size_t osi_resnet50_workspace_bytes(osi_resnet50_t net) { return net ? net->ws_floats * sizeof(float) : 0; }
int osi_resnet50_num_stages(osi_resnet50_t net) { return net ? net->n_stages : 0; }
int osi_resnet50_num_units(osi_resnet50_t net) { return net ? osi_resnet50::NUNITS : 0; }
int osi_resnet50_tensor_unit(osi_resnet50_t net, int i) { return net && i >= 0 && i < (int)net->tensors.size() ? net->tensors[i].unit : -1; }
int osi_resnet50_bn_unit(osi_resnet50_t net, int j) { return net && j >= 0 && j < (int)net->bns.size() ? net->bns[j].unit : -1; }
int osi_resnet50_set_trainable(osi_resnet50_t net, unsigned unit_mask, int eval_prefix_units) {
    OSI_REQUIRE(net && unit_mask != 0 && (unit_mask >> osi_resnet50::NUNITS) == 0 && eval_prefix_units >= 0);
    int c = 0;
    while (!((unit_mask >> c) & 1u)) ++c;
    OSI_REQUIRE(eval_prefix_units <= c);
    if (net->fwd_done) return OSI_ERR_STATE;
    net->unit_mask = unit_mask;
    net->eval_prefix = eval_prefix_units;
    return OSI_OK;
}
int osi_resnet50_get_trainable(osi_resnet50_t net, unsigned* unit_mask, int* eval_prefix_units) {
    OSI_REQUIRE(net && unit_mask && eval_prefix_units);
    *unit_mask = net->unit_mask;
    *eval_prefix_units = net->eval_prefix;
    return OSI_OK;
}
int osi_resnet50_geometry(osi_resnet50_t net, int* B, int* H, int* W) {
    OSI_REQUIRE(net);
    if (B) *B = net->B;
    if (H) *H = net->H;
    if (W) *W = net->W;
    return OSI_OK;
}

int osi_resnet50_tensor_info(osi_resnet50_t net, int i, char* name, int name_cap, int* ndim, int* shape, size_t* offset,
                             size_t* numel) {
    OSI_REQUIRE(net && i >= 0 && i < (int)net->tensors.size());
    const Tensor& t = net->tensors[i];
    if (name && name_cap > 0) { std::strncpy(name, t.name.c_str(), name_cap - 1); name[name_cap - 1] = 0; }
    if (ndim) *ndim = t.ndim;
    if (shape) for (int k = 0; k < 4; ++k) shape[k] = t.shape[k];
    if (offset) *offset = t.off;
    if (numel) *numel = t.numel;
    return OSI_OK;
}
int osi_resnet50_bn_info(osi_resnet50_t net, int j, char* prefix, int cap, int* C, size_t* rm_offset, size_t* rv_offset) {
    OSI_REQUIRE(net && j >= 0 && j < (int)net->bns.size());
    const BN& b = net->bns[j];
    if (prefix && cap > 0) { std::strncpy(prefix, b.prefix.c_str(), cap - 1); prefix[cap - 1] = 0; }
    if (C) *C = b.C;
    if (rm_offset) *rm_offset = b.rm_off;
    if (rv_offset) *rv_offset = b.rv_off;
    return OSI_OK;
}
int osi_resnet50_stage_grad_range(osi_resnet50_t net, int s, size_t* lo, size_t* hi) {
    OSI_REQUIRE(net && s >= 0 && s < net->n_stages && lo && hi);
    *lo = net->stage_lo[s]; *hi = net->stage_hi[s];
    return OSI_OK;
}

int osi_resnet50_profile(osi_resnet50_t n, int enable) {
    OSI_REQUIRE(n);
    n->prof_on = enable != 0;
    n->prof_timeline = enable == 2;
    n->prof_n = 0;
    return OSI_OK;
}
int osi_resnet50_timeline_read(osi_resnet50_t n, double* t_ms, int* cls, int* on_side, int cap, int* count) {
    OSI_REQUIRE(n && t_ms && cls && on_side && count && cap > 0);
    *count = 0;
    if (n->prof_n == 0) return OSI_OK;
    for (int i = 0; i < n->prof_n; ++i)
        if (hipEventSynchronize(n->prof_ev[i]) != hipSuccess) return OSI_ERR_LAUNCH;
    const int m = n->prof_n < cap ? n->prof_n : cap;
    for (int i = 0; i < m; ++i) {
        float t = 0.f;
        if (i > 0 && hipEventElapsedTime(&t, n->prof_ev[0], n->prof_ev[i]) != hipSuccess) return OSI_ERR_LAUNCH;
        t_ms[i] = t; cls[i] = n->prof_cls[i]; on_side[i] = n->prof_side[i];
    }
    *count = m;
    n->prof_n = 0;
    return OSI_OK;
}
int osi_resnet50_profile_read(osi_resnet50_t n, double* ms, int* count) {
    OSI_REQUIRE(n && ms && count);
    for (int k = 0; k < OSI_PROF_NCLASS; ++k) { ms[k] = 0; count[k] = 0; }
    if (n->prof_n == 0) return OSI_OK;
    if (hipEventSynchronize(n->prof_ev[n->prof_n - 1]) != hipSuccess) return OSI_ERR_LAUNCH;
    for (int i = 1; i < n->prof_n; ++i) {
        int c = n->prof_cls[i];
        if (c == OSI_PROF_START) continue;
        float t = 0.f;
        if (hipEventElapsedTime(&t, n->prof_ev[i - 1], n->prof_ev[i]) != hipSuccess) return OSI_ERR_LAUNCH;
        ms[c] += t; count[c] += 1;
    }
    n->prof_n = 0;
    return OSI_OK;
}

static int conv_bn_fwd(osi_resnet50* n, int ci, const float* params, float* buffers, float* ws, const float* x, const float* w,
                       int training, hipStream_t st, size_t bn_ws_off, int in_bn = -1) {
    Conv& c = n->convs[ci];
    BN& b = n->bns[c.bn];
    const float* isc = in_bn >= 0 ? ws + n->bns[in_bn].scale : nullptr;
    const float* ish = in_bn >= 0 ? ws + n->bns[in_bn].shift : nullptr;
    const bool wino = n->plan_knobs.fwd_wino && isc && (n->side == nullptr || st != n->side) && c.u_fw != (size_t)-1;
    if (wino) OSI_TRY(n->wait_weight_transforms(st));
    if (training == 1) {
        int P = 0, rows = 0;
        if (isc && wino) OSI_TRY(osi_conv_fwd_wino_pre(&c.d, x, isc, ish, ws + c.u_fw, ws + c.y, ws + n->wino_ws, n->wino_ws_bytes, ws + bn_ws_off, n->bn_ws_bytes, &P, &rows, st));
        else if (isc) OSI_TRY(osi_conv_fwd_act(&c.d, x, isc, ish, w, ws + c.y, OSI_TILE_AUTO, ws + bn_ws_off, n->bn_ws_bytes, &P, &rows, st));
        else OSI_TRY(osi_conv_fwd_bnstats(&c.d, x, w, ws + c.y, OSI_TILE_AUTO, ws + bn_ws_off, n->bn_ws_bytes, &P, &rows, st));
        OSI_TRY(n->mark(OSI_PROF_CONV_FWD, st));
        OSI_TRY(osi_bn_finalize_stats(ws + bn_ws_off, n->bn_ws_bytes, P, rows, b.M, b.C, params + b.g_off, params + b.b_off, 1e-5f, 0.1f,
                                      buffers + b.rm_off, buffers + b.rv_off, ws + b.mean, ws + b.invstd, ws + b.scale,
                                      ws + b.shift, st));
    } else {
        if (isc && wino) OSI_TRY(osi_conv_fwd_wino_pre(&c.d, x, isc, ish, ws + c.u_fw, ws + c.y, ws + n->wino_ws, n->wino_ws_bytes, nullptr, 0, nullptr, nullptr, st));
        else if (isc) OSI_TRY(osi_conv_fwd_act(&c.d, x, isc, ish, w, ws + c.y, OSI_TILE_AUTO, nullptr, 0, nullptr, nullptr, st));
        else OSI_TRY(osi_conv_fwd(&c.d, x, w, ws + c.y, OSI_TILE_AUTO, st));
        OSI_TRY(n->mark(OSI_PROF_CONV_FWD, st));
        if (training != 2)
        OSI_TRY(osi_bn_eval_coeffs(buffers + b.rm_off, buffers + b.rv_off, params + b.g_off, params + b.b_off, 1e-5f, b.C,
                                   ws + b.scale, ws + b.shift, st));
    }
    OSI_TRY(n->mark(OSI_PROF_BN_FWD, st));
    return OSI_OK;
}

int osi_resnet50_stage_input_u8(osi_resnet50_t n, const unsigned char* images_u8_nhwc, const unsigned char* flip, void* workspace,
                                osi_stream_t stream) {
    OSI_REQUIRE(n && images_u8_nhwc && workspace);
    OSI_TRY(osi_u8hwc3_to_nhwc4(images_u8_nhwc, flip, (float*)workspace + n->x4, n->B, n->H, n->W, stream));
    n->staged_ws = workspace;
    return OSI_OK;
}

int osi_resnet50_bind_input_nhwc4(osi_resnet50_t n, const float* x_nhwc4) {
    OSI_REQUIRE(n && x_nhwc4 && ((size_t)x_nhwc4 & 15) == 0);
    n->x4_ext = x_nhwc4;
    return OSI_OK;
}

static int head_fwd(osi_resnet50* n, const float* params, float* ws, float* logits, float* features, hipStream_t st) {
    const float* last = ws + n->blocks.back().out;
    OSI_TRY(osi_avgpool_fwd(last, ws + n->pooled, n->B, n->Hf * n->Wf, 2048, st));
    const Tensor& fw = n->tensors[n->t_fc_w]; const Tensor& fb = n->tensors[n->t_fc_b]; const Tensor& lw = n->tensors[n->t_lg_w];
    OSI_TRY(osi_linear_fwd(ws + n->pooled, params + fw.off, params + fb.off, ws + n->feat, n->B, 2048, n->F, st));
    const float* lb = n->t_lg_b >= 0 ? params + n->tensors[n->t_lg_b].off : nullptr;
    OSI_TRY(osi_linear_fwd(ws + n->feat, params + lw.off, lb, ws + n->logits_ws, n->B, n->F, n->O, st));
    if (hipMemcpyAsync(features, ws + n->feat, (size_t)n->B * n->F * sizeof(float), hipMemcpyDeviceToDevice, st) != hipSuccess)
        return OSI_ERR_LAUNCH;
    if (hipMemcpyAsync(logits, ws + n->logits_ws, (size_t)n->B * n->O * sizeof(float), hipMemcpyDeviceToDevice, st) != hipSuccess)
        return OSI_ERR_LAUNCH;
    return OSI_OK;
}

static int eval_coeffs(osi_resnet50* n, const float* params, const float* buffers, float* ws, int units, hipStream_t st) {
    osi_bn_eval_layer tab[OSI_BN_MULTI_MAX];
    int nb = 0;
    for (const BN& b : n->bns) {
        if (b.unit >= units) continue;
        if (nb == OSI_BN_MULTI_MAX) return OSI_ERR_STATE;
        tab[nb++] = osi_bn_eval_layer{buffers + b.rm_off, buffers + b.rv_off, params + b.g_off, params + b.b_off, ws + b.scale, ws + b.shift, b.C};
    }
    OSI_TRY(osi_bn_eval_coeffs_multi(tab, nb, 1e-5f, st));
    return n->mark(OSI_PROF_BN_FWD, st);
}
static int stem_fwd_eval(osi_resnet50* n, float* ws, const float* x4, hipStream_t st) {
    Conv& c0 = n->convs[0];
    OSI_TRY(osi_conv_fwd(&c0.d, x4, ws + n->wpack, ws + c0.y, OSI_TILE_AUTO, st));
    OSI_TRY(n->mark(OSI_PROF_CONV_FWD, st));
    BN& b0 = n->bns[c0.bn];
    OSI_TRY(osi_bn_relu_maxpool_fwd(ws + c0.y, ws + b0.scale, ws + b0.shift, ws + n->a_pool, ws + n->pool_idx, n->B, n->Hs, n->Ws, 64, st));
    return n->mark(OSI_PROF_BN_FWD, st);
}
static int block_fwd_eval(osi_resnet50* n, Block& k, const float* params, float* ws, hipStream_t st) {
    auto epi = [&](int ci, const float* res, int relu) {
        const BN& b = n->bns[n->convs[ci].bn];
        return osi_conv_epilogue{ws + b.scale, ws + b.shift, res, relu};
    };
    const float* x = ws + k.x_in;
    Conv &c1 = n->convs[k.c1], &c2 = n->convs[k.c2], &c3 = n->convs[k.c3];
    const bool fork = k.ds >= 0 && n->fwd_fork && n->async_wgrad();
    if (k.ds >= 0) {
        Conv& cd = n->convs[k.ds];
        hipStream_t ds_st = st;
        if (fork) {
            OSI_TRY(n->fork_side(st));
            ds_st = n->side;
        }
        const osi_conv_epilogue e = epi(k.ds, nullptr, 0);
        OSI_TRY(osi_conv_fwd_epilogue(&cd.d, x, params + cd.w_off, ws + cd.y, &e, ws + (fork ? n->bn_ws2 : n->bn_ws), n->bn_ws_bytes, ds_st));
        OSI_TRY(n->mark(OSI_PROF_CONV_FWD, ds_st));
        if (fork && hipEventRecord(n->ev_join, n->side) != hipSuccess) return OSI_ERR_LAUNCH;
    }
    {
        const osi_conv_epilogue e = epi(k.c1, nullptr, 1);
        OSI_TRY(osi_conv_fwd_epilogue(&c1.d, x, params + c1.w_off, ws + c1.y, &e, ws + n->bn_ws, n->bn_ws_bytes, st));
        OSI_TRY(n->mark(OSI_PROF_CONV_FWD, st));
    }
    {
        const osi_conv_epilogue e = epi(k.c2, nullptr, 1);
        if (n->plan_knobs.fwd_wino && c2.u_fw != (size_t)-1) {
            OSI_TRY(n->wait_weight_transforms(st));
            OSI_TRY(osi_conv_fwd_wino_epilogue_pre(&c2.d, ws + c1.y, ws + c2.u_fw, ws + c2.y, &e, ws + n->wino_ws, n->wino_ws_bytes, st));
        } else {
            OSI_TRY(osi_conv_fwd_epilogue(&c2.d, ws + c1.y, params + c2.w_off, ws + c2.y, &e, ws + n->bn_ws, n->bn_ws_bytes, st));
        }
        OSI_TRY(n->mark(OSI_PROF_CONV_FWD, st));
    }
    if (fork && hipStreamWaitEvent(st, n->ev_join, 0) != hipSuccess) return OSI_ERR_LAUNCH;
    {
        const osi_conv_epilogue e = epi(k.c3, k.ds >= 0 ? ws + n->convs[k.ds].y : x, 1);
        OSI_TRY(osi_conv_fwd_epilogue(&c3.d, ws + c2.y, params + c3.w_off, ws + c3.a, &e, ws + n->bn_ws, n->bn_ws_bytes, st));
        OSI_TRY(n->mark(OSI_PROF_CONV_FWD, st));
    }
    return OSI_OK;
}
static int forward_eval_fused(osi_resnet50* n, const float* params, const float* buffers, float* ws, const float* x4, float* logits,
                              float* features, hipStream_t st) {
    OSI_TRY(eval_coeffs(n, params, buffers, ws, osi_resnet50::NUNITS, st));
    OSI_TRY(stem_fwd_eval(n, ws, x4, st));
    for (Block& k : n->blocks) OSI_TRY(block_fwd_eval(n, k, params, ws, st));
    OSI_TRY(head_fwd(n, params, ws, logits, features, st));
    n->any_fwd = false;
    OSI_TRY(n->mark(OSI_PROF_OTHER, st));
    return OSI_OK;
}

static int forward_impl(osi_resnet50_t n, const float* params, float* buffers, long long* nbt, const float* image,
                        void* workspace, float* logits, float* features, int training, osi_stream_t stream);

int osi_resnet50_forward(osi_resnet50_t n, const float* params, float* buffers, long long* nbt, const float* image,
                         void* workspace, float* logits, float* features, int training, osi_stream_t stream) {
    OSI_REQUIRE(n && params && buffers && workspace && logits && features);
    OSI_REQUIRE(!training || nbt);
    return forward_impl(n, params, buffers, nbt, image, workspace, logits, features, training ? 1 : 0, stream);
}

int osi_resnet50_forward_frozen(osi_resnet50_t n, const float* params, const float* buffers, const float* image, void* workspace,
                                float* logits, float* features, osi_stream_t stream) {
    OSI_REQUIRE(n && params && buffers && workspace && logits && features);
    return forward_impl(n, params, const_cast<float*>(buffers), nullptr, image, workspace, logits, features, 2, stream);
}

static int forward_impl(osi_resnet50_t n, const float* params, float* buffers, long long* nbt, const float* image,
                        void* workspace, float* logits, float* features, int training, osi_stream_t stream) {
    if (!n->plan_unchanged()) return OSI_ERR_STATE;
    const float* ext = n->x4_ext;
    n->x4_ext = nullptr;
    if (!image && !ext && n->staged_ws != workspace) return OSI_ERR_STATE;
    n->staged_ws = nullptr;
    hipStream_t st = (hipStream_t)stream;
    float* ws = (float*)workspace;
    const float* x4 = (!image && ext) ? ext : ws + n->x4;
    n->x4_cur = x4;
    n->fwd_done = false;
    n->frozen = false;
    const int p = training ? n->eval_prefix : 0;
    if (training && n->overlap && (!n->prof_on || n->prof_timeline)) OSI_TRY(n->ensure_side());
    OSI_TRY(n->mark(OSI_PROF_START, st));
    if (n->plan_knobs.fwd_wino || (training == 1 && n->plan_knobs.dgrad_wino)) {
        const bool aside = training == 1 && n->async_wgrad();
        hipStream_t wt = aside ? n->side : st;
        if (aside) OSI_TRY(n->fork_side(st));
        for (auto& c : n->convs)
            if (n->plan_knobs.fwd_wino && c.u_fw != (size_t)-1)
                OSI_TRY(osi_conv_wino_transform_weights(&c.d, params + c.w_off, 0, ws + c.u_fw, osi_conv_wino_weights_bytes(&c.d), wt));
        OSI_TRY(n->mark(OSI_PROF_CONV_FWD, wt));
        if (training == 1 && n->plan_knobs.dgrad_wino) {
            int nt = 0;
            for (auto& c : n->convs)
                if (c.u_bw != (size_t)-1 && c.unit >= p) {
                    OSI_TRY(osi_conv_wino_transform_weights(&c.d, params + c.w_off, 1, ws + c.u_bw, osi_conv_wino_weights_bytes(&c.d), wt));
                    ++nt;
                }
            if (nt) OSI_TRY(n->mark(OSI_PROF_CONV_DGRAD, wt));
        }
        if (aside) {
            if (hipEventRecord(n->ev_wt, n->side) != hipSuccess) return OSI_ERR_LAUNCH;
            n->wt_pending = true;
        }
    }
    if (image) OSI_TRY(osi_nchw3_to_nhwc4(image, ws + n->x4, n->B, n->H, n->W, st));
    Conv& c0 = n->convs[0];
    OSI_TRY(osi_stem_weight_pack(params + c0.w_off, ws + n->wpack, 64, st));
    OSI_TRY(n->mark(OSI_PROF_OTHER, st));
    if (!training && n->eval_fused) return forward_eval_fused(n, params, buffers, ws, x4, logits, features, st);
    if (p > 0) OSI_TRY(eval_coeffs(n, params, buffers, ws, p, st));
    if (training == 2) {
        osi_bn_frozen_layer tab[OSI_BN_FROZEN_MAX];
        int nb = 0;
        for (const BN& b : n->bns) {
            if (b.unit < p) continue;
            if (nb == OSI_BN_FROZEN_MAX) return OSI_ERR_STATE;
            tab[nb++] = osi_bn_frozen_layer{buffers + b.rm_off, buffers + b.rv_off, params + b.g_off, params + b.b_off, ws + b.scale, ws + b.shift,
                                            ws + b.mean, ws + b.invstd, b.C};
        }
        if (nb) {
            OSI_TRY(osi_bn_frozen_coeffs_multi(tab, nb, 1e-5f, st));
            OSI_TRY(n->mark(OSI_PROF_BN_FWD, st));
        }
    }
    if (p > 0) {
        OSI_TRY(stem_fwd_eval(n, ws, x4, st));
    } else {
    OSI_TRY(conv_bn_fwd(n, 0, params, buffers, ws, x4, ws + n->wpack, training, st, n->bn_ws));
    BN& b0 = n->bns[c0.bn];
    OSI_TRY(osi_bn_relu_maxpool_fwd(ws + c0.y, ws + b0.scale, ws + b0.shift, ws + n->a_pool, ws + n->pool_idx, n->B, n->Hs, n->Ws, 64, st));
    OSI_TRY(n->mark(OSI_PROF_BN_FWD, st));
    }
    for (Block& k : n->blocks) {
        if (n->convs[k.c1].unit < p) {
            OSI_TRY(block_fwd_eval(n, k, params, ws, st));
            continue;
        }
        const float* x = ws + k.x_in;
        const bool fork = k.ds >= 0 && n->fwd_fork && n->async_wgrad();
        if (k.ds >= 0) {
            Conv& c = n->convs[k.ds];
            if (fork) OSI_TRY(n->fork_side(st));
            OSI_TRY(conv_bn_fwd(n, k.ds, params, buffers, ws, x, params + c.w_off, training, fork ? n->side : st, fork ? n->bn_ws2 : n->bn_ws));
            if (fork && hipEventRecord(n->ev_join, n->side) != hipSuccess) return OSI_ERR_LAUNCH;
        }
        Conv &c1 = n->convs[k.c1], &c2 = n->convs[k.c2], &c3 = n->convs[k.c3];
        OSI_TRY(conv_bn_fwd(n, k.c1, params, buffers, ws, x, params + c1.w_off, training, st, n->bn_ws));
        OSI_TRY(conv_bn_fwd(n, k.c2, params, buffers, ws, ws + c1.y, params + c2.w_off, training, st, n->bn_ws, c1.bn));
        OSI_TRY(conv_bn_fwd(n, k.c3, params, buffers, ws, ws + c2.y, params + c3.w_off, training, st, n->bn_ws, c2.bn));
        if (fork && hipStreamWaitEvent(st, n->ev_join, 0) != hipSuccess) return OSI_ERR_LAUNCH;
        BN& b3 = n->bns[c3.bn];
        if (k.ds >= 0) {
            Conv& cd = n->convs[k.ds];
            BN& bd = n->bns[cd.bn];
            OSI_TRY(osi_bn_apply_relu_mask2(ws + c3.y, ws + b3.scale, ws + b3.shift, ws + cd.y, ws + bd.scale, ws + bd.shift, ws + c3.a,
                                            ws + c3.mask, b3.M, b3.C, st));
        } else {
            OSI_TRY(osi_bn_apply_relu_mask(ws + c3.y, x, ws + b3.scale, ws + b3.shift, ws + c3.a, ws + c3.mask, b3.M, b3.C, st));
        }
        OSI_TRY(n->mark(OSI_PROF_BN_FWD, st));
    }
    OSI_TRY(head_fwd(n, params, ws, logits, features, st));
    n->any_fwd = true;
    if (training) {
        if (training == 1) {
            int j0 = 0;
            while (j0 < (int)n->bns.size() && n->bns[j0].unit < p) ++j0;
            if (j0 < (int)n->bns.size()) OSI_TRY(osi_i64_add(nbt + j0, (int)n->bns.size() - j0, 1, st));
        }
        n->fw_prefix = p;
        n->frozen = training == 2;
        n->fwd_done = true;
        n->next_stage = 0;
    }
    OSI_TRY(n->mark(OSI_PROF_OTHER, st));
    return OSI_OK;
}

static int wgrad_launch(osi_resnet50* n, int ci, float* grads, float* ws, int gi, const float* conv_in, hipStream_t st, int in_bn,
                        bool async) {
    Conv& c = n->convs[ci];
    const float* dy = ws + n->scratch[gi];
    hipStream_t ws_st = st;
    if (async) {
        OSI_TRY(n->fork_side(st));
        ws_st = n->side;
    }
    if (ci == 0) {
        if (osi_stem_wgrad_direct_workspace(&c.d) > 0) {
            OSI_TRY(osi_stem_wgrad_direct(&c.d, dy, conv_in, grads + c.w_off, ws + n->wg_ws, n->wg_ws_bytes, ws_st));
        } else {
            OSI_TRY(osi_conv_wgrad(&c.d, dy, conv_in, ws + n->gpack, ws + n->wg_ws, n->wg_ws_bytes, ws_st));
            OSI_TRY(osi_stem_grad_unpack(ws + n->gpack, grads + c.w_off, 64, ws_st));
        }
    } else if (in_bn >= 0 && n->plan_knobs.wgrad_wino && osi_conv_wgrad_wino_workspace(&c.d) > 0) {
        OSI_TRY(osi_conv_wgrad_wino(&c.d, dy, conv_in, ws + n->bns[in_bn].scale, ws + n->bns[in_bn].shift, grads + c.w_off, ws + n->wg_ws,
                                    n->wg_ws_bytes, ws_st));
    } else if (in_bn >= 0) {
        OSI_TRY(osi_conv_wgrad_act(&c.d, dy, conv_in, ws + n->bns[in_bn].scale, ws + n->bns[in_bn].shift, grads + c.w_off, ws + n->wg_ws,
                                   n->wg_ws_bytes, ws_st));
    } else {
        OSI_TRY(osi_conv_wgrad(&c.d, dy, conv_in, grads + c.w_off, ws + n->wg_ws, n->wg_ws_bytes, ws_st));
    }
    if (async) {
        if (hipEventRecord(n->buf_ev[gi], n->side) != hipSuccess) return OSI_ERR_LAUNCH;
        n->buf_pending[gi] = true;
        n->side_dirty = true;
    }
    OSI_TRY(n->mark(OSI_PROF_CONV_WGRAD, ws_st));
    return OSI_OK;
}

static int wgrad(osi_resnet50* n, int ci, float* grads, float* ws, int gi, const float* conv_in, hipStream_t st, int in_bn = -1) {
    if (!n->bw_pg) return OSI_OK;
    if (!n->trainable(n->convs[ci].unit)) return OSI_OK;
    return wgrad_launch(n, ci, grads, ws, gi, conv_in, st, in_bn, n->async_wgrad());
}

static int dgrad_plain(osi_resnet50* n, const osi_conv_desc* d, const float* dy, const float* w, float* dx, int accumulate, hipStream_t st) {
    OSI_TRY(osi_conv_dgrad(d, dy, w, dx, accumulate, OSI_TILE_AUTO, st));
    return n->mark(OSI_PROF_CONV_DGRAD, st);
}

static int bn_conv_wgrad(osi_resnet50* n, int ci, const float* params, float* grads, float* ws, int gi,
                         float* gmasked, const float* conv_in, hipStream_t st) {
    Conv& c = n->convs[ci];
    BN& b = n->bns[c.bn];
    float* g = ws + n->scratch[gi];
    OSI_TRY(osi_bn_backward_relu_mask(g, ws + c.mask, ws + c.y, ws + b.mean, ws + b.invstd, params + b.g_off, g, gmasked,
                                      n->dgam(grads, ws, b), n->dbet(grads, ws, b), b.M, b.C, ws + n->bn_ws, n->bn_ws_bytes, st));
    OSI_TRY(n->mark(OSI_PROF_BN_BWD, st));
    return wgrad(n, ci, grads, ws, gi, conv_in, st);
}

static int bn_bwd_fused(osi_resnet50* n, int ci, const float* params, float* grads, float* ws, int gi, int dyi, int which,
                        hipStream_t st) {
    Conv& c = n->convs[ci];
    BN& b = n->bns[c.bn];
    const float* psum_g = ws + n->dg_ws;
    const float* psum_gx = psum_g + (size_t)(1 + which) * n->fused_P * b.C;
    OSI_TRY(osi_bn_backward_fused(ws + n->scratch[gi], ws + c.y, ws + b.mean, ws + b.invstd, params + b.g_off, psum_g, psum_gx,
                                  n->fused_P, ws + n->scratch[dyi], n->dgam(grads, ws, b), n->dbet(grads, ws, b), b.M, b.C, ws + n->bn_ws,
                                  n->bn_ws_bytes, st));
    OSI_TRY(n->mark(OSI_PROF_BN_BWD, st));
    return OSI_OK;
}

static int bn_reduce_frozen(osi_resnet50* n, int ci, float* grads, float* ws, int which, hipStream_t st) {
    if (!n->bw_pg) return OSI_OK;
    BN& b = n->bns[n->convs[ci].bn];
    if (!n->trainable(b.unit)) return OSI_OK;
    const float* psum_g = ws + n->dg_ws;
    const float* psum_gx = psum_g + (size_t)(1 + which) * n->fused_P * b.C;
    OSI_TRY(osi_bn_backward_reduce(psum_g, psum_gx, n->fused_P, grads + b.g_off, grads + b.b_off, b.M, b.C, ws + n->bn_ws, n->bn_ws_bytes, st));
    return n->mark(OSI_PROF_BN_BWD, st);
}
static int bn_bwd_frozen(osi_resnet50* n, int ci, int cj, float* grads, float* ws, int gi, int dyi, int dyj, int gmasked, bool masked,
                         hipStream_t st) {
    osi_bn_frozen_consumer cs[2];
    const int idx[2] = {ci, cj}, out[2] = {dyi, dyj};
    const int nc = cj >= 0 ? 2 : 1;
    for (int k = 0; k < nc; ++k) {
        Conv& c = n->convs[idx[k]];
        BN& b = n->bns[c.bn];
        const bool red = masked && n->bw_pg && n->trainable(b.unit);
        cs[k] = osi_bn_frozen_consumer{ws + c.y, ws + b.mean, ws + b.invstd, ws + b.scale, ws + n->scratch[out[k]],
                                       red ? grads + b.g_off : nullptr, red ? grads + b.b_off : nullptr};
    }
    Conv& c = n->convs[ci];
    BN& b = n->bns[c.bn];
    OSI_TRY(osi_bn_backward_frozen(ws + n->scratch[gi], masked ? ws + c.mask : nullptr, cs, nc, gmasked >= 0 ? ws + n->scratch[gmasked] : nullptr,
                                   b.M, b.C, ws + n->bn_ws, n->bn_ws_bytes, st));
    return n->mark(OSI_PROF_BN_BWD, st);
}
static int dgrad_frozen(osi_resnet50* n, int ci, const float* params, float* grads, float* ws, int dyi, int dxi, int pc, hipStream_t st) {
    Conv& c = n->convs[ci];
    Conv& p0 = n->convs[pc];
    BN& b0 = n->bns[p0.bn];
    osi_dgrad_fusion f{};
    f.scale0 = ws + b0.scale; f.shift0 = ws + b0.shift;
    f.y0 = ws + p0.y; f.mean0 = ws + b0.mean; f.invstd0 = ws + b0.invstd;
    f.partials = ws + n->dg_ws; f.partials_bytes = n->dg_ws_bytes;
    int P = 0;
    OSI_TRY(osi_conv_dgrad_fused_frozen(&c.d, ws + n->scratch[dyi], params + c.w_off, ws + n->scratch[dxi], &f, OSI_TILE_AUTO, &P, st));
    n->fused_P = P;
    OSI_TRY(n->mark(OSI_PROF_CONV_DGRAD, st));
    return bn_reduce_frozen(n, pc, grads, ws, 0, st);
}

static int dgrad_fused(osi_resnet50* n, int ci, const float* params, float* ws, int dyi, int dxi, int addi, int pc, int pd,
                       hipStream_t st, bool add_even = false) {
    Conv& c = n->convs[ci];
    Conv& p0 = n->convs[pc];
    BN& b0 = n->bns[p0.bn];
    osi_dgrad_fusion f{};
    if (p0.mask != (size_t)-1) f.relu_mask = ws + p0.mask;
    else { f.scale0 = ws + b0.scale; f.shift0 = ws + b0.shift; }
    f.y0 = ws + p0.y; f.mean0 = ws + b0.mean; f.invstd0 = ws + b0.invstd;
    if (pd >= 0) {
        Conv& p1 = n->convs[pd];
        BN& b1 = n->bns[p1.bn];
        f.y1 = ws + p1.y; f.mean1 = ws + b1.mean; f.invstd1 = ws + b1.invstd;
    }
    f.partials = ws + n->dg_ws; f.partials_bytes = n->dg_ws_bytes;
    f.addend_stride = add_even ? 2 : 1;
    int P = 0;
    OSI_TRY(n->wait_weight_transforms(st));
    if (n->plan_knobs.dgrad_wino && f.scale0 && pd < 0 && addi < 0 && c.u_bw != (size_t)-1)
        OSI_TRY(osi_conv_dgrad_fused_wino_pre(&c.d, ws + n->scratch[dyi], ws + c.u_bw, ws + n->scratch[dxi], &f, ws + n->wino_ws,
                                              n->wino_ws_bytes, &P, st));
    else
    OSI_TRY(osi_conv_dgrad_fused(&c.d, ws + n->scratch[dyi], params + c.w_off, ws + n->scratch[dxi],
                                 addi >= 0 ? ws + n->scratch[addi] : nullptr, &f, OSI_TILE_AUTO, &P, st));
    n->fused_P = P;
    return n->mark(OSI_PROF_CONV_DGRAD, st);
}

static int block_backward(osi_resnet50* n, int bi, const float* params, float* grads, float* ws, hipStream_t st, bool no_dx) {
    Block& k = n->blocks[bi];
    auto S = [&](int i) { return ws + n->scratch[i]; };
    Conv &c1 = n->convs[k.c1], &c2 = n->convs[k.c2], &c3 = n->convs[k.c3];
    const float* x = ws + k.x_in;
    const bool has_ds = k.ds >= 0;
    const bool ds_sparse = has_ds && bi > 0 && n->convs[k.ds].d.stride == 2 && n->convs[k.ds].d.R == 1;
    int go = n->cur_grad;
    int d3 = -1, dxbase = -1;
    if (n->frozen) {
        int t1 = -1;
        if (has_ds) { t1 = n->take(st); if (t1 < 0) return t1; }
        if (n->go_fused) {
            OSI_TRY(bn_reduce_frozen(n, k.c3, grads, ws, 0, st));
            if (has_ds) OSI_TRY(bn_reduce_frozen(n, k.ds, grads, ws, 1, st));
            d3 = n->take(st);
            if (d3 < 0) return d3;
            OSI_TRY(bn_bwd_frozen(n, k.c3, k.ds, grads, ws, go, d3, t1, -1, false, st));
            if (has_ds) n->give(go);
            else dxbase = go;
        } else {
            if (!has_ds) { dxbase = n->take(st); if (dxbase < 0) return dxbase; }
            OSI_TRY(bn_bwd_frozen(n, k.c3, k.ds, grads, ws, go, go, t1, has_ds ? -1 : dxbase, true, st));
            d3 = go;
        }
        if (has_ds) {
            Conv& cd = n->convs[k.ds];
            OSI_TRY(wgrad(n, k.ds, grads, ws, t1, x, st));
            if (!no_dx) {
                dxbase = n->take(st);
                if (dxbase < 0) return dxbase;
                OSI_TRY(dgrad_plain(n, &cd.d, S(t1), params + cd.w_off, S(dxbase), ds_sparse ? 2 : 0, st));
            }
            n->give(t1);
        }
    } else if (n->go_fused) {
        if (has_ds) {
            Conv& cd = n->convs[k.ds];
            int t1 = n->take(st);
            if (t1 < 0) return t1;
            OSI_TRY(bn_bwd_fused(n, k.ds, params, grads, ws, go, t1, 1, st));
            OSI_TRY(wgrad(n, k.ds, grads, ws, t1, x, st));
            if (!no_dx) {
                dxbase = n->take(st);
                if (dxbase < 0) return dxbase;
                OSI_TRY(dgrad_plain(n, &cd.d, S(t1), params + cd.w_off, S(dxbase), ds_sparse ? 2 : 0, st));
            }
            n->give(t1);
        }
        d3 = n->take(st);
        if (d3 < 0) return d3;
        OSI_TRY(bn_bwd_fused(n, k.c3, params, grads, ws, go, d3, 0, st));
        if (has_ds) n->give(go);
        else dxbase = go;
    } else {
        dxbase = n->take(st);
        if (dxbase < 0) return dxbase;
        if (has_ds) {
            Conv& cd = n->convs[k.ds];
            BN& bd = n->bns[cd.bn];
            int t1 = n->take(st);
            if (t1 < 0) return t1;
            OSI_TRY(osi_bn_backward_relu_mask(S(go), ws + c3.mask, ws + cd.y, ws + bd.mean, ws + bd.invstd, params + bd.g_off,
                                              S(t1), nullptr, n->dgam(grads, ws, bd), n->dbet(grads, ws, bd), bd.M, bd.C, ws + n->bn_ws,
                                              n->bn_ws_bytes, st));
            OSI_TRY(n->mark(OSI_PROF_BN_BWD, st));
            OSI_TRY(wgrad(n, k.ds, grads, ws, t1, x, st));
            if (!no_dx) OSI_TRY(dgrad_plain(n, &cd.d, S(t1), params + cd.w_off, S(dxbase), ds_sparse ? 2 : 0, st));
            n->give(t1);
        }
        BN& b3 = n->bns[c3.bn];
        OSI_TRY(osi_bn_backward_relu_mask(S(go), ws + c3.mask, ws + c3.y, ws + b3.mean, ws + b3.invstd, params + b3.g_off, S(go),
                                          has_ds ? nullptr : S(dxbase), n->dgam(grads, ws, b3), n->dbet(grads, ws, b3), b3.M, b3.C,
                                          ws + n->bn_ws, n->bn_ws_bytes, st));
        OSI_TRY(n->mark(OSI_PROF_BN_BWD, st));
        d3 = go;
    }
    OSI_TRY(wgrad(n, k.c3, grads, ws, d3, ws + c2.y, st, c2.bn));
    int t2 = n->take(st);
    if (t2 < 0) return t2;
    if (n->frozen) OSI_TRY(dgrad_frozen(n, k.c3, params, grads, ws, d3, t2, k.c2, st));
    else OSI_TRY(dgrad_fused(n, k.c3, params, ws, d3, t2, -1, k.c2, -1, st));
    n->give(d3);
    if (!n->frozen) OSI_TRY(bn_bwd_fused(n, k.c2, params, grads, ws, t2, t2, 0, st));
    OSI_TRY(wgrad(n, k.c2, grads, ws, t2, ws + c1.y, st, c1.bn));
    int t3 = n->take(st);
    if (t3 < 0) return t3;
    if (n->frozen) OSI_TRY(dgrad_frozen(n, k.c2, params, grads, ws, t2, t3, k.c1, st));
    else OSI_TRY(dgrad_fused(n, k.c2, params, ws, t2, t3, -1, k.c1, -1, st));
    n->give(t2);
    if (!n->frozen) OSI_TRY(bn_bwd_fused(n, k.c1, params, grads, ws, t3, t3, 0, st));
    OSI_TRY(wgrad(n, k.c1, grads, ws, t3, x, st));
    if (no_dx) {
        if (dxbase >= 0) n->give(dxbase);
        n->cur_grad = -1;
        n->go_fused = false;
    } else if (bi > 0) {
        Block& pk = n->blocks[bi - 1];
        int dxn = has_ds ? dxbase : n->take(st);
        if (dxn < 0) return dxn;
        OSI_TRY(dgrad_fused(n, k.c1, params, ws, t3, dxn, dxbase, pk.c3, pk.ds, st, ds_sparse));
        if (dxn != dxbase) n->give(dxbase);
        n->cur_grad = dxn;
        n->go_fused = true;
    } else {
        Conv& c0 = n->convs[0];
        if (n->stem_tail_fused()) {
            BN& b0 = n->bns[c0.bn];
            osi_dgrad_fusion f{};
            f.y0 = ws + c0.y; f.mean0 = ws + b0.mean; f.invstd0 = ws + b0.invstd;
            f.partials = ws + n->dg_ws; f.partials_bytes = n->dg_ws_bytes;
            f.pool_idx = ws + n->pool_idx; f.pool_H = n->Hs; f.pool_W = n->Ws;
            int P = 0;
            OSI_TRY(osi_conv_dgrad_fused(&c1.d, S(t3), params + c1.w_off, S(dxbase), S(dxbase), &f, OSI_TILE_AUTO, &P, st));
            n->stem_stats_P = P;
            OSI_TRY(n->mark(OSI_PROF_CONV_DGRAD, st));
        } else {
            OSI_TRY(dgrad_plain(n, &c1.d, S(t3), params + c1.w_off, S(dxbase), 1, st));
        }
        n->cur_grad = dxbase;
        n->go_fused = false;
    }
    n->give(t3);
    return OSI_OK;
}

int osi_resnet50_backward(osi_resnet50_t n, const float* params, float* grads, void* workspace, const float* dlogits,
                          const float* dfeatures, int stage_lo, int stage_hi, osi_stream_t stream) {
    return osi_resnet50_backward_ex(n, params, grads, workspace, dlogits, dfeatures, nullptr, 1, stage_lo, stage_hi, stream);
}

struct BwRequest {
    float* dimage;
    int param_grads;
    float* x_adv;
    float eps, lo, hi;
};

static int backward_stages(osi_resnet50_t n, const float* params, float* grads, void* workspace, const float* dlogits,
                           const float* dfeatures, const BwRequest& rq, int stage_lo, int stage_hi, osi_stream_t stream);

int osi_resnet50_backward_ex(osi_resnet50_t n, const float* params, float* grads, void* workspace, const float* dlogits,
                             const float* dfeatures, float* dimage, int param_grads, int stage_lo, int stage_hi, osi_stream_t stream) {
    OSI_REQUIRE(n && params && workspace);
    OSI_REQUIRE(param_grads == 0 || param_grads == 1);
    OSI_REQUIRE(!param_grads || grads);
    OSI_REQUIRE(param_grads || dimage);
    OSI_REQUIRE(((uintptr_t)dimage & 3) == 0);
    return backward_stages(n, params, grads, workspace, dlogits, dfeatures, BwRequest{dimage, param_grads, nullptr, 0.f, 0.f, 0.f}, stage_lo,
                           stage_hi, stream);
}

int osi_resnet50_backward_adv(osi_resnet50_t n, const float* params, float* grads, void* workspace, const float* dlogits,
                              const float* dfeatures, float* x_adv_nhwc4, float eps, float lo, float hi, int stage_lo, int stage_hi,
                              osi_stream_t stream) {
    OSI_REQUIRE(n && params && grads && workspace && x_adv_nhwc4);
    OSI_REQUIRE(((uintptr_t)x_adv_nhwc4 & 15) == 0 && eps >= 0.f && lo <= hi);
    const size_t img_bytes = (size_t)n->B * n->H * n->W * 4 * sizeof(float);
    auto apart = [&](const void* p, size_t bytes) {
        const uintptr_t a = (uintptr_t)x_adv_nhwc4, b = (uintptr_t)p;
        return a + img_bytes <= b || b + bytes <= a;
    };
    OSI_REQUIRE(apart(workspace, n->ws_floats * sizeof(float)));
    OSI_REQUIRE(!n->x4_cur || apart(n->x4_cur, img_bytes));
    return backward_stages(n, params, grads, workspace, dlogits, dfeatures, BwRequest{nullptr, 1, x_adv_nhwc4, eps, lo, hi}, stage_lo,
                           stage_hi, stream);
}

static int backward_stages(osi_resnet50_t n, const float* params, float* grads, void* workspace, const float* dlogits,
                           const float* dfeatures, const BwRequest& rq, int stage_lo, int stage_hi, osi_stream_t stream) {
    float* const dimage = rq.dimage;
    const int param_grads = rq.param_grads;
    OSI_REQUIRE(stage_lo >= 0 && stage_lo < stage_hi && stage_hi <= n->n_stages);
    if (!n->fwd_done || stage_lo != n->next_stage || !n->plan_unchanged()) return OSI_ERR_STATE;
    if (n->fw_prefix > 0 && (dimage || rq.x_adv)) return OSI_ERR_STATE;
    if (stage_lo == 0) {
        n->bw_dimage = dimage;
        n->bw_pg = param_grads != 0;
        n->bw_adv = rq.x_adv; n->bw_eps = rq.eps; n->bw_lo = rq.lo; n->bw_hi = rq.hi;
    } else if (n->bw_dimage != dimage || n->bw_pg != (param_grads != 0) || n->bw_adv != rq.x_adv || n->bw_eps != rq.eps ||
               n->bw_lo != rq.lo || n->bw_hi != rq.hi) {
        return OSI_ERR_STATE;
    }
    hipStream_t st = (hipStream_t)stream;
    float* ws = (float*)workspace;
    auto S = [&](int i) { return ws + n->scratch[i]; };
    if (n->overlap && (!n->prof_on || n->prof_timeline)) OSI_TRY(n->ensure_side());
    OSI_TRY(n->mark(OSI_PROF_START, st));
    const int stop = n->bw_stop();
    const int head = osi_resnet50::NUNITS - 1;

    for (int stage = stage_lo; stage < stage_hi; ++stage) {
        if (stage == 0) {
            OSI_REQUIRE(dlogits);
            n->free_list.clear();
            for (int i = 0; i < osi_resnet50::NSCR; ++i) { n->free_list.push_back(i); n->buf_pending[i] = false; }
            const Tensor& fw = n->tensors[n->t_fc_w]; const Tensor& fb = n->tensors[n->t_fc_b]; const Tensor& lw = n->tensors[n->t_lg_w];
            float* dfeat = ws + n->dfeat;
            int acc = 0;
            if (dfeatures) {
                if (hipMemcpyAsync(dfeat, dfeatures, (size_t)n->B * n->F * sizeof(float), hipMemcpyDeviceToDevice, st) != hipSuccess)
                    return OSI_ERR_LAUNCH;
                acc = 1;
            }
            const bool pg = n->bw_pg && n->trainable(head);
            float* dlb = pg && n->t_lg_b >= 0 ? grads + n->tensors[n->t_lg_b].off : nullptr;
            OSI_TRY(osi_linear_bwd(dlogits, ws + n->feat, params + lw.off, dfeat, acc, pg ? grads + lw.off : nullptr, dlb, n->B, n->F,
                                   n->O, st));
            const bool below = stop < head;
            OSI_TRY(osi_linear_bwd(dfeat, ws + n->pooled, params + fw.off, below ? ws + n->dpooled : nullptr, 0, pg ? grads + fw.off : nullptr,
                                   pg ? grads + fb.off : nullptr, n->B, 2048, n->F, st));
            n->cur_grad = -1;
            if (below) {
                int g = n->take(st);
                if (g < 0) return g;
                OSI_TRY(osi_avgpool_bwd(ws + n->dpooled, S(g), n->B, n->Hf * n->Wf, 2048, st));
                n->cur_grad = g;
            }
            OSI_TRY(n->mark(OSI_PROF_OTHER, st));
            n->go_fused = false;
        }
        for (int bi = (int)n->blocks.size() - 1; bi >= 0; --bi) {
            Block& k = n->blocks[bi];
            if (k.stage != stage || bi + 1 < stop) continue;
            OSI_TRY(block_backward(n, bi, params, grads, ws, st, bi + 1 == stop));
        }
        if (stage == n->n_stages - 1 && stop > 0) {
            n->cur_grad = -1;
            n->fwd_done = false;
        } else if (stage == n->n_stages - 1) {
            Conv& c0 = n->convs[0];
            int go = n->cur_grad;
            int t = n->take(st);
            if (t < 0) return t;
            BN& b0 = n->bns[c0.bn];
            const float* x4c = n->x4_cur ? n->x4_cur : ws + n->x4;
            if (n->stem_tail_fused()) {
                n->give(t);
                const float* psum_g = ws + n->dg_ws;
                OSI_TRY(osi_bn_backward_reduce(psum_g, psum_g + (size_t)n->stem_stats_P * 64, n->stem_stats_P, grads + b0.g_off,
                                               grads + b0.b_off, n->B * n->Hs * n->Ws, 64, ws + n->bn_ws, n->bn_ws_bytes, st));
                OSI_TRY(n->mark(OSI_PROF_BN_BWD, st));
                OSI_TRY(osi_stem_wgrad_fused(&c0.d, S(go), ws + n->pool_idx, ws + c0.y, x4c, params + b0.g_off, ws + b0.mean, ws + b0.invstd,
                                             grads + b0.g_off, grads + b0.b_off, grads + c0.w_off, ws + n->stem_ws, n->stem_ws_bytes, st));
                OSI_TRY(n->mark(OSI_PROF_CONV_WGRAD, st));
                n->give(go);
            } else {
                if (n->frozen)
                    OSI_TRY(osi_bn_relu_maxpool_bwd_frozen(S(go), ws + n->pool_idx, ws + c0.y, ws + b0.mean, ws + b0.invstd, ws + b0.scale, S(t),
                                                           n->bw_pg && n->trainable(0) ? grads + b0.g_off : nullptr,
                                                           n->bw_pg && n->trainable(0) ? grads + b0.b_off : nullptr, n->B,
                                                           n->Hs, n->Ws, 64, ws + n->bn_ws, n->bn_ws_bytes, st));
                else
                OSI_TRY(osi_bn_relu_maxpool_bwd(S(go), ws + n->pool_idx, ws + c0.y, ws + b0.mean, ws + b0.invstd, params + b0.g_off, S(t),
                                                n->dgam(grads, ws, b0), n->dbet(grads, ws, b0), n->B, n->Hs, n->Ws, 64, ws + n->bn_ws,
                                                n->bn_ws_bytes, st));
                OSI_TRY(n->mark(OSI_PROF_BN_BWD, st));
                n->give(go);
                OSI_TRY(wgrad(n, 0, grads, ws, t, x4c, st));
                if (n->bw_dimage) {
                    OSI_TRY(osi_stem_dgrad(S(t), params + c0.w_off, n->bw_dimage, n->B, n->H, n->W, st));
                    OSI_TRY(n->mark(OSI_PROF_CONV_DGRAD, st));
                } else if (n->bw_adv) {
                    OSI_TRY(osi_stem_dgrad_fgsm(S(t), params + c0.w_off, x4c, n->bw_adv, n->bw_eps, n->bw_lo, n->bw_hi, n->B, n->H, n->W, st));
                    OSI_TRY(n->mark(OSI_PROF_CONV_DGRAD, st));
                }
                n->give(t);
            }
            n->cur_grad = -1;
            n->fwd_done = false;
        }
        n->next_stage = stage + 1;
    }
    if (n->stage_join || stage_hi == n->n_stages) OSI_TRY(n->join_side(st));
    return OSI_OK;
}

int osi_resnet50_grads_ready(osi_resnet50_t n, osi_stream_t main_stream, osi_stream_t waiter_stream) {
    OSI_REQUIRE(n);
    hipStream_t mn = (hipStream_t)main_stream, wt = (hipStream_t)waiter_stream;
    if (!n->ev_rmain) {
        if (hipEventCreateWithFlags(&n->ev_rmain, EV_FLAGS_HANDOFF) != hipSuccess) return OSI_ERR_LAUNCH;
        if (hipEventCreateWithFlags(&n->ev_rside, EV_FLAGS_HANDOFF) != hipSuccess) return OSI_ERR_LAUNCH;
    }
    if (hipEventRecord(n->ev_rmain, mn) != hipSuccess) return OSI_ERR_LAUNCH;
    if (hipStreamWaitEvent(wt, n->ev_rmain, 0) != hipSuccess) return OSI_ERR_LAUNCH;
    if (n->side && n->side_dirty) {
        if (hipEventRecord(n->ev_rside, n->side) != hipSuccess) return OSI_ERR_LAUNCH;
        if (hipStreamWaitEvent(wt, n->ev_rside, 0) != hipSuccess) return OSI_ERR_LAUNCH;
    }
    return OSI_OK;
}

namespace {
__global__ __launch_bounds__(256) void k_dbg_gate_bits(const unsigned long long* __restrict__ bits, unsigned char* __restrict__ out,
                                                       size_t n, int HW, int C) {
    const size_t e = (size_t)blockIdx.x * 256 + threadIdx.x;
    if (e >= n) return;
    const size_t i4 = e >> 2;
    const unsigned long long w = bits[(i4 >> 6) * 4 + (e & 3)];
    const size_t pix = e / C;
    const int c = (int)(e - pix * C);
    const size_t b = pix / HW, hw = pix - b * HW;
    out[(b * C + c) * HW + hw] = (unsigned char)((w >> (i4 & 63)) & 1);
}
__global__ __launch_bounds__(256) void k_dbg_gate_fma(const float* __restrict__ y, const float* __restrict__ scale,
                                                      const float* __restrict__ shift, unsigned char* __restrict__ out, size_t n, int HW,
                                                      int C) {
    const size_t e = (size_t)blockIdx.x * 256 + threadIdx.x;
    if (e >= n) return;
    const size_t pix = e / C;
    const int c = (int)(e - pix * C);
    const size_t b = pix / HW, hw = pix - b * HW;
    out[(b * C + c) * HW + hw] = __builtin_fmaf(y[e], scale[c], shift[c]) > 0.f ? 1 : 0;
}
__global__ __launch_bounds__(256) void k_dbg_gate_pool(const uint32_t* __restrict__ idx, unsigned char* __restrict__ gate,
                                                       int* __restrict__ argmax, size_t n, int Ws, int Hp, int Wp, int C) {
    const size_t e = (size_t)blockIdx.x * 256 + threadIdx.x;
    if (e >= n) return;
    const uint32_t byte = (idx[e >> 2] >> (8 * (e & 3))) & 0xffu;
    const size_t pix = e / C;
    const int c = (int)(e - pix * C);
    const size_t b = pix / ((size_t)Hp * Wp), hw = pix - b * Hp * Wp;
    const int ho = (int)(hw / Wp), wo = (int)(hw - (size_t)ho * Wp);
    const int tap = byte & 0x7f, r = tap / 3, s = tap - 3 * r;
    const size_t o = (b * C + c) * ((size_t)Hp * Wp) + hw;
    gate[o] = (unsigned char)(byte >> 7);
    if (argmax) argmax[o] = (ho * 2 - 1 + r) * Ws + (wo * 2 - 1 + s);
}
}

int osi_resnet50_debug_num_gates(osi_resnet50_t n) { return n ? 1 + 3 * (int)n->blocks.size() : 0; }

int osi_resnet50_debug_gate_shape(osi_resnet50_t n, int i, int* C, int* H, int* W) {
    OSI_REQUIRE(n && C && H && W && i >= 0 && i < 1 + 3 * (int)n->blocks.size());
    if (i == 0) { *C = 64; *H = n->Hp; *W = n->Wp; return OSI_OK; }
    const Block& k = n->blocks[(i - 1) / 3];
    const int which = (i - 1) % 3;
    const osi_conv_desc& d = n->convs[which == 0 ? k.c1 : which == 1 ? k.c2 : k.c3].d;
    *C = d.Cout; *H = d.Ho; *W = d.Wo;
    return OSI_OK;
}

int osi_resnet50_debug_gate(osi_resnet50_t n, void* workspace, int i, unsigned char* gate_nchw, int* pool_argmax_nchw,
                            osi_stream_t stream) {
    OSI_REQUIRE(n && workspace && gate_nchw && i >= 0 && i < 1 + 3 * (int)n->blocks.size());
    OSI_REQUIRE(i == 0 || !pool_argmax_nchw);
    if (!n->any_fwd) return OSI_ERR_STATE;
    if ((i == 0 ? 0 : (i - 1) / 3 + 1) < n->fw_prefix) return OSI_ERR_STATE;
    hipStream_t st = (hipStream_t)stream;
    float* ws = (float*)workspace;
    if (i == 0) {
        const size_t e = (size_t)n->B * n->Hp * n->Wp * 64;
        hipLaunchKernelGGL(k_dbg_gate_pool, dim3((unsigned)((e + 255) / 256)), dim3(256), 0, st, (const uint32_t*)(ws + n->pool_idx),
                           gate_nchw, pool_argmax_nchw, e, n->Ws, n->Hp, n->Wp, 64);
        OSI_LAUNCH_CHECK();
        return OSI_OK;
    }
    const Block& k = n->blocks[(i - 1) / 3];
    const int which = (i - 1) % 3;
    const Conv& c = n->convs[which == 0 ? k.c1 : which == 1 ? k.c2 : k.c3];
    const BN& b = n->bns[c.bn];
    const size_t e = (size_t)b.M * b.C;
    const int HW = c.d.Ho * c.d.Wo;
    if (which == 2)
        hipLaunchKernelGGL(k_dbg_gate_bits, dim3((unsigned)((e + 255) / 256)), dim3(256), 0, st,
                           (const unsigned long long*)(ws + c.mask), gate_nchw, e, HW, b.C);
    else
        hipLaunchKernelGGL(k_dbg_gate_fma, dim3((unsigned)((e + 255) / 256)), dim3(256), 0, st, ws + c.y, ws + b.scale, ws + b.shift,
                           gate_nchw, e, HW, b.C);
    OSI_LAUNCH_CHECK();
    return OSI_OK;
}

int osi_resnet50_set_option(osi_resnet50_t n, const char* name, int value) {
    OSI_REQUIRE(n && name);
    if (!strcmp(name, "overlap")) n->overlap = value != 0;
    else if (!strcmp(name, "fwd_fork")) n->fwd_fork = value != 0;
    else if (!strcmp(name, "stage_join")) n->stage_join = value != 0;
    else if (!strcmp(name, "eval_fused")) n->eval_fused = value != 0;
    else if (!strcmp(name, "forget_forward")) { if (value) n->fwd_done = false; }
    else if (!strcmp(name, "side_priority_normal")) {
        if (n->side) return OSI_ERR_STATE;
        n->side_prio_normal = value != 0;
    } else return OSI_ERR_ARG;
    return OSI_OK;
}

}
```

### openset-imagenet_amd/openset_imagenet/_native.py

```python
import ctypes
import os
from ctypes import c_char_p, c_double, c_float, c_int, c_longlong, c_size_t, c_void_p, POINTER, Structure

_HERE = os.path.dirname(os.path.abspath(__file__))
CSRC_DIR = os.path.normpath(os.path.join(_HERE, "..", "csrc"))
LIB_PATH = os.path.join(CSRC_DIR, "libosi_hip.so")
TORCH_LIB_PATH = os.path.join(CSRC_DIR, "libosi_torch.so")

OSI_OK = 0
TILE_AUTO, TILE_128x128, TILE_128x64, TILE_64x128, TILE_64x64 = 0, 1, 2, 3, 4
LOSS_ENTROPIC, LOSS_SOFTMAX, LOSS_GARBAGE = 0, 1, 2


class ConvDesc(Structure):
    _fields_ = [(n, c_int) for n in ("B", "H", "W", "Cin", "Ho", "Wo", "Cout", "R", "S", "stride", "pad")]

    @classmethod
    def make(cls, B, H, W, Cin, Cout, k, stride, pad):
        Ho = (H + 2 * pad - k) // stride + 1
        Wo = (W + 2 * pad - k) // stride + 1
        return cls(B, H, W, Cin, Ho, Wo, Cout, k, k, stride, pad)


class ConvEpilogue(Structure):
    _fields_ = [("scale", c_void_p), ("shift", c_void_p), ("residual", c_void_p), ("relu", c_int)]


class BnEvalLayer(Structure):
    _fields_ = [("running_mean", c_void_p), ("running_var", c_void_p), ("gamma", c_void_p), ("beta", c_void_p), ("scale", c_void_p),
                ("shift", c_void_p), ("C", c_int)]


class BnFrozenLayer(Structure):
    _fields_ = [("running_mean", c_void_p), ("running_var", c_void_p), ("gamma", c_void_p), ("beta", c_void_p), ("scale", c_void_p),
                ("shift", c_void_p), ("mean", c_void_p), ("invstd", c_void_p), ("C", c_int)]


class BnFrozenConsumer(Structure):
    _fields_ = [("y", c_void_p), ("mean", c_void_p), ("invstd", c_void_p), ("scale", c_void_p), ("dy", c_void_p), ("dgamma", c_void_p),
                ("dbeta", c_void_p)]


class OptSegment(Structure):
    _fields_ = [("begin4", ctypes.c_uint), ("end4", ctypes.c_uint), ("group", c_int)]


class AdamGroup(Structure):
    _fields_ = [("lr", c_double), ("beta1", c_double), ("beta2", c_double), ("eps", c_double), ("weight_decay", c_double),
                ("step", c_longlong), ("decoupled", c_int), ("amsgrad", c_int), ("maximize", c_int)]


class SgdGroup(Structure):
    _fields_ = [("lr", c_double), ("momentum", c_double), ("dampening", c_double), ("weight_decay", c_double),
                ("nesterov", c_int), ("first_step", c_int), ("maximize", c_int)]


OPT_MAX_SEGMENTS, OPT_MAX_GROUPS = 192, 16

P = c_void_p
_PD = POINTER(ConvDesc)

_SIGS = {
    "osi_abi_version": (c_int, []),
    "osi_build_arch": (c_char_p, []),
    "osi_strerror": (c_char_p, [c_int]),
    "osi_set_tuning": (c_int, [c_char_p, c_int]),
    "osi_get_tuning": (c_int, [c_char_p, POINTER(c_int)]),
    "osi_conv_fwd": (c_int, [_PD, P, P, P, c_int, P]),
    "osi_conv_fwd_act": (c_int, [_PD, P, P, P, P, P, c_int, P, c_size_t, POINTER(c_int), POINTER(c_int), P]),
    "osi_conv_fwd_act2": (c_int, [_PD, P, P, P, P, P, P, c_int, P, c_size_t, POINTER(c_int), POINTER(c_int), P]),
    "osi_conv_fwd_epilogue_workspace": (c_size_t, [_PD]),
    "osi_conv_fwd_epilogue": (c_int, [_PD, P, P, P, POINTER(ConvEpilogue), P, c_size_t, P]),
    "osi_conv_fwd_wino_epilogue_pre": (c_int, [_PD, P, P, P, POINTER(ConvEpilogue), P, c_size_t, P]),
    "osi_bn_eval_coeffs_multi": (c_int, [POINTER(BnEvalLayer), c_int, c_float, P]),
    "osi_conv_wgrad_act": (c_int, [_PD, P, P, P, P, P, P, c_size_t, P]),
    "osi_conv_wino_eligible": (c_int, [_PD, c_int]),
    "osi_conv_wino_workspace": (c_size_t, [_PD]),
    "osi_conv_fwd_wino": (c_int, [_PD, P, P, P, P, P, P, c_size_t, P, c_size_t, POINTER(c_int), POINTER(c_int), P]),
    "osi_conv_dgrad_fused_wino": (c_int, [_PD, P, P, P, P, P, c_size_t, POINTER(c_int), P]),
    "osi_conv_wino_weights_bytes": (c_size_t, [_PD]),
    "osi_conv_wino_slab_bytes": (c_size_t, []),
    "osi_conv_wino_transform_weights": (c_int, [_PD, P, c_int, P, c_size_t, P]),
    "osi_conv_fwd_wino_pre": (c_int, [_PD, P, P, P, P, P, P, c_size_t, P, c_size_t, POINTER(c_int), POINTER(c_int), P]),
    "osi_conv_dgrad_fused_wino_pre": (c_int, [_PD, P, P, P, P, P, c_size_t, POINTER(c_int), P]),
    "osi_conv_wgrad_wino_workspace": (c_size_t, [_PD]),
    "osi_conv_wgrad_wino": (c_int, [_PD, P, P, P, P, P, P, c_size_t, P]),
    "osi_conv_fwd_bnstats_workspace": (c_size_t, [_PD]),
    "osi_conv_fwd_bnstats": (c_int, [_PD, P, P, P, c_int, P, c_size_t, POINTER(c_int), POINTER(c_int), P]),
    "osi_bn_finalize_stats": (c_int, [P, c_size_t, c_int, c_int, c_int, c_int, P, P, c_float, c_float, P, P, P, P, P, P, P]),
    "osi_conv_dgrad": (c_int, [_PD, P, P, P, c_int, c_int, P]),
    "osi_conv_dgrad_fused_workspace": (c_size_t, [_PD]),
    "osi_conv_dgrad_fused": (c_int, [_PD, P, P, P, P, P, c_int, POINTER(c_int), P]),
    "osi_bn_backward_reduce": (c_int, [P, P, c_int, P, P, c_int, c_int, P, c_size_t, P]),
    "osi_bn_backward_fused": (c_int, [P, P, P, P, P, P, P, c_int, P, P, P, c_int, c_int, P, c_size_t, P]),
    "osi_conv_wgrad_workspace": (c_size_t, [_PD]),
    "osi_conv_wgrad": (c_int, [_PD, P, P, P, P, c_size_t, P]),
    "osi_stem_weight_pack": (c_int, [P, P, c_int, P]),
    "osi_stem_wgrad_direct_workspace": (c_size_t, [_PD]),
    "osi_stem_wgrad_direct": (c_int, [_PD, P, P, P, P, c_size_t, P]),
    "osi_stem_wgrad_fused_workspace": (c_size_t, [_PD]),
    "osi_stem_wgrad_fused": (c_int, [_PD, P, P, P, P, P, P, P, P, P, P, P, c_size_t, P]),
    "osi_stem_grad_unpack": (c_int, [P, P, c_int, P]),
    "osi_stem_dgrad": (c_int, [P, P, P, c_int, c_int, c_int, P]),
    "osi_stem_dgrad_fgsm": (c_int, [P, P, P, P, c_float, c_float, c_float, c_int, c_int, c_int, P]),
    "osi_bn_workspace": (c_size_t, [c_int, c_int]),
    "osi_bn_train_stats": (c_int, [P, c_int, c_int, P, P, c_float, c_float, P, P, P, P, P, P, P, c_size_t, P]),
    "osi_bn_eval_coeffs": (c_int, [P, P, P, P, c_float, c_int, P, P, P]),
    "osi_bn_apply": (c_int, [P, P, P, P, P, c_int, c_int, c_int, P]),
    "osi_bn_backward_workspace": (c_size_t, [c_int, c_int]),
    "osi_bn_backward": (c_int, [P, P, P, P, P, P, P, P, P, P, c_int, c_int, P, c_size_t, P]),
    "osi_bn_relu_mask_bytes": (c_size_t, [c_int, c_int]),
    "osi_bn_apply_relu_mask": (c_int, [P, P, P, P, P, P, c_int, c_int, P]),
    "osi_bn_apply_relu_mask2": (c_int, [P, P, P, P, P, P, P, P, c_int, c_int, P]),
    "osi_bn_backward_relu_mask": (c_int, [P, P, P, P, P, P, P, P, P, P, c_int, c_int, P, c_size_t, P]),
    "osi_nchw3_to_nhwc4": (c_int, [P, P, c_int, c_int, c_int, P]),
    "osi_u8hwc3_to_nhwc4": (c_int, [P, P, P, c_int, c_int, c_int, P]),
    "osi_u8_crop_flip_to_nhwc4": (c_int, [P, P, P, P, c_int, c_int, c_int, c_int, c_int, P]),
    "osi_resnet50_stage_input_u8": (c_int, [c_void_p, P, P, P, P]),
    "osi_resnet50_bind_input_nhwc4": (c_int, [c_void_p, P]),
    "osi_maxpool3x3s2_fwd": (c_int, [P, P, P, c_int, c_int, c_int, c_int, P]),
    "osi_maxpool3x3s2_bwd": (c_int, [P, P, P, c_int, c_int, c_int, c_int, P]),
    "osi_bn_relu_maxpool_fwd": (c_int, [P, P, P, P, P, c_int, c_int, c_int, c_int, P]),
    "osi_bn_relu_maxpool_bwd": (c_int, [P, P, P, P, P, P, P, P, P, c_int, c_int, c_int, c_int, P, c_size_t, P]),
    "osi_avgpool_fwd": (c_int, [P, P, c_int, c_int, c_int, P]),
    "osi_avgpool_bwd": (c_int, [P, P, c_int, c_int, c_int, P]),
    "osi_linear_fwd": (c_int, [P, P, P, P, c_int, c_int, c_int, P]),
    "osi_linear_bwd": (c_int, [P, P, P, P, c_int, P, P, c_int, c_int, c_int, P]),
    "osi_loss_fwd_bwd": (c_int, [c_int, P, P, c_int, c_int, c_float, c_longlong, P, P, c_int, c_float, c_float, P, P, P, P]),
    "osi_softmax": (c_int, [P, P, c_int, c_int, P]),
    "osi_confidence_accumulate": (c_int, [P, P, c_int, c_int, c_float, c_longlong, c_int, P, P]),
    "osi_confidence_from_scores": (c_int, [P, P, c_int, c_int, c_float, c_longlong, c_int, P, P]),
    "osi_oscr_workspace": (c_size_t, [c_int]),
    "osi_oscr_f32": (c_int, [P, P, c_int, c_int, c_longlong, P, c_size_t, P, P, P, P, P]),
    "osi_oscr_f64": (c_int, [P, P, c_int, c_int, c_longlong, P, c_size_t, P, P, P, P, P]),
    "osi_adam_step": (c_int, [P, P, P, P, c_size_t, c_double, c_double, c_double, c_double, c_longlong, c_float, P]),
    "osi_sgd_step": (c_int, [P, P, P, c_size_t, c_float, c_float, c_int, c_float, P]),
    "osi_adam_step_groups": (c_int, [P, P, P, P, P, c_size_t, POINTER(OptSegment), c_int, POINTER(AdamGroup), c_int, c_float, P]),
    "osi_sgd_step_groups": (c_int, [P, P, P, c_size_t, POINTER(OptSegment), c_int, POINTER(SgdGroup), c_int, c_float, P]),
    "osi_fill_f32": (c_int, [P, c_size_t, c_float, P]),
    "osi_scale_f32": (c_int, [P, c_size_t, c_float, P]),
    "osi_grad_accumulate": (c_int, [P, P, c_size_t, P]),
    "osi_i64_add": (c_int, [P, c_int, c_longlong, P]),
    "osi_resnet50_create": (c_int, [POINTER(c_void_p), c_int, c_int, c_int, c_int, c_int, c_int]),
    "osi_resnet50_destroy": (None, [c_void_p]),
    "osi_resnet50_num_tensors": (c_int, [c_void_p]),
    "osi_resnet50_tensor_info": (c_int, [c_void_p, c_int, c_char_p, c_int, POINTER(c_int), POINTER(c_int), POINTER(c_size_t), POINTER(c_size_t)]),
    "osi_resnet50_param_floats": (c_size_t, [c_void_p]),
    "osi_resnet50_num_bn": (c_int, [c_void_p]),
    "osi_resnet50_bn_info": (c_int, [c_void_p, c_int, c_char_p, c_int, POINTER(c_int), POINTER(c_size_t), POINTER(c_size_t)]),
    "osi_resnet50_buffer_floats": (c_size_t, [c_void_p]),
    "osi_resnet50_workspace_bytes": (c_size_t, [c_void_p]),
    "osi_resnet50_num_stages": (c_int, [c_void_p]),
    "osi_resnet50_geometry": (c_int, [c_void_p, POINTER(c_int), POINTER(c_int), POINTER(c_int)]),
    "osi_resnet50_stage_grad_range": (c_int, [c_void_p, c_int, POINTER(c_size_t), POINTER(c_size_t)]),
    "osi_resnet50_grads_ready": (c_int, [c_void_p, P, P]),
    "osi_resnet50_num_units": (c_int, [c_void_p]),
    "osi_resnet50_tensor_unit": (c_int, [c_void_p, c_int]),
    "osi_resnet50_bn_unit": (c_int, [c_void_p, c_int]),
    "osi_resnet50_set_trainable": (c_int, [c_void_p, ctypes.c_uint, c_int]),
    "osi_resnet50_get_trainable": (c_int, [c_void_p, POINTER(ctypes.c_uint), POINTER(c_int)]),
    "osi_resnet50_set_option": (c_int, [c_void_p, c_char_p, c_int]),
    "osi_resnet50_profile": (c_int, [c_void_p, c_int]),
    "osi_resnet50_profile_read": (c_int, [c_void_p, POINTER(ctypes.c_double), POINTER(c_int)]),
    "osi_resnet50_timeline_read": (c_int, [c_void_p, POINTER(ctypes.c_double), POINTER(c_int), POINTER(c_int), c_int, POINTER(c_int)]),
    "osi_resnet50_debug_num_gates": (c_int, [c_void_p]),
    "osi_resnet50_debug_gate_shape": (c_int, [c_void_p, c_int, POINTER(c_int), POINTER(c_int), POINTER(c_int)]),
    "osi_resnet50_debug_gate": (c_int, [c_void_p, P, c_int, P, P, P]),
    "osi_resnet50_forward": (c_int, [c_void_p, P, P, P, P, P, P, P, c_int, P]),
    "osi_bn_frozen_coeffs_multi": (c_int, [POINTER(BnFrozenLayer), c_int, c_float, P]),
    "osi_conv_dgrad_fused_frozen": (c_int, [_PD, P, P, P, P, c_int, POINTER(c_int), P]),
    "osi_bn_backward_frozen": (c_int, [P, P, POINTER(BnFrozenConsumer), c_int, P, c_int, c_int, P, c_size_t, P]),
    "osi_bn_relu_maxpool_bwd_frozen": (c_int, [P, P, P, P, P, P, P, P, P, c_int, c_int, c_int, c_int, P, c_size_t, P]),
    "osi_resnet50_forward_frozen": (c_int, [c_void_p, P, P, P, P, P, P, P]),
    "osi_resnet50_backward": (c_int, [c_void_p, P, P, P, P, P, c_int, c_int, P]),
    "osi_resnet50_backward_ex": (c_int, [c_void_p, P, P, P, P, P, P, c_int, c_int, c_int, P]),
    "osi_resnet50_backward_adv": (c_int, [c_void_p, P, P, P, P, P, P, c_float, c_float, c_float, c_int, c_int, P]),
}

_lib = None
DIAGNOSTIC_LIB = None


class NativeLibraryMissing(RuntimeError):
    pass


def lib():
    global _lib, LIB_PATH
    if _lib is None:
        global DIAGNOSTIC_LIB
        if os.environ.get("OSI_HIP_LIB"):
            if os.environ.get("OSI_DEV") != "1":
                raise NativeLibraryMissing("OSI_HIP_LIB selects a diagnostic build of the native library and is only honoured with OSI_DEV=1")
            LIB_PATH = os.environ["OSI_HIP_LIB"]
            DIAGNOSTIC_LIB = LIB_PATH
            import warnings
            warnings.warn(f"openset_imagenet: DIAGNOSTIC native library {LIB_PATH} (OSI_HIP_LIB + OSI_DEV=1): results may be wrong by design",
                          RuntimeWarning, stacklevel=2)
        if not os.path.isfile(LIB_PATH):
            raise NativeLibraryMissing(
                f"{LIB_PATH} not found: build the gfx950 HIP library first (python __graft_entry__.py, or make -C {CSRC_DIR}). "
                "There is no CPU fallback for the training hot path.")
        handle = ctypes.CDLL(LIB_PATH)
        for name, (res, args) in _SIGS.items():
            fn = getattr(handle, name)
            fn.restype = res
            fn.argtypes = args
        _lib = handle
        for env, knob in (("OSI_WGRAD_TILE", b"wgrad_tile"), ("OSI_WGRAD_BLOCKS", b"wgrad_blocks"), ("OSI_WGRAD_NST", b"wgrad_nst"),
                          ("OSI_WGRAD_GROUP", b"wgrad_group"), ("OSI_BN_GRID", b"bn_grid"), ("OSI_BN_GRID_BWD", b"bn_grid_bwd"), ("OSI_BN_SINGLE_P", b"bn_single_p"), ("OSI_BN_WIDE_P", b"bn_wide_p"), ("OSI_TAIL_GAIN", b"tail_gain"), ("OSI_TAIL_QMAX", b"tail_qmax"), ("OSI_WGRAD3", b"wgrad3"), ("OSI_WGRAD3_BLOCKS", b"wgrad3_blocks"), ("OSI_FWD_WIDE", b"fwd_wide"), ("OSI_DGRAD_WIDE", b"dgrad_wide"), ("OSI_TAIL_SPLIT", b"tail_split"), ("OSI_TAIL_CUS", b"tail_cus"), ("OSI_TAIL_SMAX", b"tail_smax"), ("OSI_TAIL_MINT", b"tail_mint"), ("OSI_STEM_DIRECT", b"stem_direct"), ("OSI_DP_RESERVED_CUS", b"dp_reserved_cus"), ("OSI_FWD_ROWS", b"fwd_rows"), ("OSI_FWD_W3", b"fwd_w3"), ("OSI_DGRAD_W3", b"dgrad_w3"), ("OSI_FWD_WINO", b"fwd_wino"), ("OSI_DGRAD_WINO", b"dgrad_wino"), ("OSI_WINO_STREAMK", b"wino_streamk"), ("OSI_WGRAD_WINO", b"wgrad_wino"), ("OSI_WINO_WIDE", b"wino_wide")):
            if os.environ.get(env):
                check(handle.osi_set_tuning(knob, int(os.environ[env])), f"osi_set_tuning({knob.decode()})")
    return _lib


_ops = None


def ops():
    global _ops
    if _ops is None:
        lib()
        if not os.path.isfile(TORCH_LIB_PATH):
            raise NativeLibraryMissing(f"{TORCH_LIB_PATH} not found: build it first (python __graft_entry__.py, or make -C {CSRC_DIR}).")
        import torch
        torch.ops.load_library(TORCH_LIB_PATH)
        _ops = torch.ops.osi
    return _ops


def declared_symbols():
    return sorted(_SIGS)


def check(code, what=""):
    if code != OSI_OK:
        msg = lib().osi_strerror(code).decode()
        raise RuntimeError(f"libosi_hip {what} failed: {msg} (code {code})")


def ptr(t):
    return None if t is None else t.data_ptr()


def stream_of(t):
    import torch
    return torch.cuda.current_stream(t.device).cuda_stream


def require_gpu_f32(*tensors):
    import torch
    for t in tensors:
        if t is None:
            continue
        if not t.is_cuda:
            raise RuntimeError("openset_imagenet (MI355X build): tensors must live on the GPU — there is no CPU fallback "
                               "(set_device_gpu(index) / model.to('cuda')).")
        if t.dtype != torch.float32 and t.dtype != torch.int64:
            raise RuntimeError(f"unsupported dtype {t.dtype}: the hot path is fp32 (labels int64)")
```

Before: 4445 images/sec.

## Fuse paired BN backward for conv3 and downsample, hoist per-channel coefficients

Adds a fused BN backward that handles both the conv3 and downsample BN consumers of the same incoming gradient in one pass. Reductions are batched via a consumer table indexed by the grid dimension, and the apply kernel reads the gradient once and writes both dy outputs. The elementwise BN apply, backward-apply and frozen kernels also gain a geometry specialisation that loads per-channel coefficients into registers once per thread instead of per element. The final linear layer now writes logits directly instead of going through a workspace copy. The cost is more template instantiations and extra code complexity.

New measurement: 4574 images/sec, median of 6. +2.9%, better.

```diff
diff --git a/include/osi.h b/include/osi.h
--- a/include/osi.h
+++ b/include/osi.h
@@ -150,6 +150,16 @@
                           void* ws, size_t ws_bytes, osi_stream_t stream);
 
 typedef struct {
+    const float *y, *mean, *invstd, *gamma;
+    const float* psum_gx;
+    float* dy;
+    float *dgamma, *dbeta;
+} osi_bn_fused_consumer;
+size_t osi_bn_backward_fused2_workspace(int C);
+int osi_bn_backward_fused2(const float* g, const osi_bn_fused_consumer* consumers, const float* psum_g, int P, int M, int C, void* ws,
+                           size_t ws_bytes, osi_stream_t stream);
+
+typedef struct {
     const float *y, *mean, *invstd;
     const float* scale;
     float* dy;
diff --git a/openset-imagenet_amd/csrc/abi.hip b/openset-imagenet_amd/csrc/abi.hip
--- a/openset-imagenet_amd/csrc/abi.hip
+++ b/openset-imagenet_amd/csrc/abi.hip
@@ -40,7 +40,7 @@
 }
 
 extern "C" {
-int osi_abi_version(void) { return 13; }
+int osi_abi_version(void) { return 14; }
 int osi_set_tuning(const char* name, int value) {
     int* s = tuning_slot(name);
     if (!s) return OSI_ERR_ARG;
diff --git a/openset-imagenet_amd/csrc/bn.hip b/openset-imagenet_amd/csrc/bn.hip
--- a/openset-imagenet_amd/csrc/bn.hip
+++ b/openset-imagenet_amd/csrc/bn.hip
@@ -283,27 +283,41 @@
 #ifndef OSI_BN_REVERSE
 #define OSI_BN_REVERSE 3
 #endif
-template <int RES, bool RELU, bool BITS>
+struct FwdCoef { f32x4 sc, sh, rs, rh; };
+template <int RES>
+__device__ __forceinline__ FwdCoef fwd_coef(const f32x4* __restrict__ scale, const f32x4* __restrict__ shift,
+                                            const f32x4* __restrict__ rscale, const f32x4* __restrict__ rshift, int c4) {
+    FwdCoef k;
+    k.sc = scale[c4]; k.sh = shift[c4];
+    if (RES == 2) { k.rs = rscale[c4]; k.rh = rshift[c4]; } else { k.rs = k.sc; k.rh = k.sh; }
+    return k;
+}
+template <int RES, bool RELU, bool BITS, int GEO>
 __global__ __launch_bounds__(NT) void k_bn_apply(const f32x4* __restrict__ y, const f32x4* __restrict__ res,
                                                 const f32x4* __restrict__ scale, const f32x4* __restrict__ shift,
                                                 const f32x4* __restrict__ rscale, const f32x4* __restrict__ rshift,
                                                 f32x4* __restrict__ out, u64* __restrict__ bits, size_t n4, int c4n) {
     const size_t nq = (n4 + NT - 1) / NT;
+    const int tid = threadIdx.x;
+    FwdCoef k0 = {}, k1 = {};
+    if (GEO == 1) k0 = fwd_coef<RES>(scale, shift, rscale, rshift, tid % c4n);
+    if (GEO == 2) { k0 = fwd_coef<RES>(scale, shift, rscale, rshift, tid); k1 = fwd_coef<RES>(scale, shift, rscale, rshift, NT + tid); }
     for (size_t q = blockIdx.x; q < nq; q += gridDim.x) {
-        const size_t i = ((OSI_BN_REVERSE & 1) ? nq - 1 - q : q) * NT + threadIdx.x;
+        const size_t t = (OSI_BN_REVERSE & 1) ? nq - 1 - q : q;
+        const size_t i = t * NT + tid;
         if (i >= n4) continue;
-        int c4 = (int)(i % (size_t)c4n);
-        const f32x4 yv = __builtin_nontemporal_load(y + i), sc = scale[c4], sh = shift[c4];
+        const FwdCoef k = GEO == 1 ? k0 : GEO == 2 ? ((t & 1) ? k1 : k0) : fwd_coef<RES>(scale, shift, rscale, rshift, (int)(i % (size_t)c4n));
+        const f32x4 yv = __builtin_nontemporal_load(y + i), sc = k.sc, sh = k.sh;
         f32x4 v;
 #pragma unroll
         for (int e = 0; e < 4; ++e) v[e] = __builtin_fmaf(yv[e], sc[e], sh[e]);
         if (RES == 1) v += __builtin_nontemporal_load(res + i);
         if (RES == 2) {
-            const f32x4 rv = __builtin_nontemporal_load(res + i), rs = rscale[c4], rh = rshift[c4];
-            f32x4 t;
+            const f32x4 rv = __builtin_nontemporal_load(res + i), rs = k.rs, rh = k.rh;
+            f32x4 t2;
 #pragma unroll
-            for (int e = 0; e < 4; ++e) t[e] = __builtin_fmaf(rv[e], rs[e], rh[e]);
-            v += t;
+            for (int e = 0; e < 4; ++e) t2[e] = __builtin_fmaf(rv[e], rs[e], rh[e]);
+            v += t2;
         }
         if (BITS) {
             const u64 b0 = __ballot(v.x > 0.f), b1 = __ballot(v.y > 0.f), b2 = __ballot(v.z > 0.f), b3 = __ballot(v.w > 0.f);
@@ -420,9 +434,12 @@
     }
 }
 
-__global__ __launch_bounds__(NT) void k_bn_bwd_final(const float* __restrict__ pdb, const float* __restrict__ pdg, int P, int M,
-                                                    int C, float* __restrict__ dgamma, float* __restrict__ dbeta,
-                                                    float* __restrict__ c1, float* __restrict__ c2) {
+struct BwdCons { const float *pa, *pb; float *ga, *gb, *dgamma, *dbeta, *c1, *c2; };
+struct BwdConsTable { BwdCons k[2]; };
+__global__ __launch_bounds__(NT) void k_bn_bwd_final(BwdConsTable t, bool grouped, int P, int M, int C) {
+    const BwdCons& o = t.k[blockIdx.y];
+    const float* __restrict__ pdb = grouped ? o.ga : o.pa;
+    const float* __restrict__ pdg = grouped ? o.gb : o.pb;
     const int lane = threadIdx.x & 63;
     const int c = blockIdx.x * (NT / 64) + (threadIdx.x >> 6);
     if (c >= C) return;
@@ -430,20 +447,22 @@
     for (int b = lane; b < P; b += 64) { ab += pdb[(size_t)c * P + b]; ag += pdg[(size_t)c * P + b]; }
     ab = wave_sum(ab); ag = wave_sum(ag);
     if (lane == 0) {
-        dbeta[c] = ab; dgamma[c] = ag;
-        c1[c] = ab / (float)M; c2[c] = ag / (float)M;
-    }
-}
-
-__global__ __launch_bounds__(NT) void k_colsum2_group(const float* __restrict__ a, const float* __restrict__ b, int P, int Pc, int C,
-                                                     int S, float* __restrict__ ga, float* __restrict__ gb) {
+        o.dbeta[c] = ab; o.dgamma[c] = ag;
+        o.c1[c] = ab / (float)M; o.c2[c] = ag / (float)M;
+    }
+}
+
+__global__ __launch_bounds__(NT) void k_colsum2_group(BwdConsTable t, int P, int Pc, int C, int S) {
     __shared__ float ra[16][16], rb[16][16];
+    const BwdCons& o = t.k[blockIdx.z];
+    float* __restrict__ ga = o.ga;
+    float* __restrict__ gb = o.gb;
     const int cl = threadIdx.x & 15, pl = threadIdx.x >> 4;
     const int c = min(blockIdx.x * 16 + cl, C - 1), s = blockIdx.y;
     const bool ok = blockIdx.x * 16 + cl < C;
     const int b0 = s * Pc, b1 = min(P, b0 + Pc);
-    const float* pa = a + c;
-    const float* pb = b + c;
+    const float* __restrict__ pa = o.pa + c;
+    const float* __restrict__ pb = o.pb + c;
     float xa0 = 0.f, xa1 = 0.f, xb0 = 0.f, xb1 = 0.f;
     int r = b0 + pl;
     for (; r + 48 < b1; r += 64) {
@@ -462,15 +481,14 @@
     }
 }
 
-__global__ __launch_bounds__(16 * WPL) void k_bn_bwd_final_wide(const float* __restrict__ a, const float* __restrict__ b, int P, int M, int C,
-                                                               float* __restrict__ dgamma, float* __restrict__ dbeta,
-                                                               float* __restrict__ c1, float* __restrict__ c2) {
+__global__ __launch_bounds__(16 * WPL) void k_bn_bwd_final_wide(BwdConsTable t, int P, int M, int C) {
     __shared__ float red[WPL][16];
+    const BwdCons& o = t.k[blockIdx.y];
     const int cl = threadIdx.x & 15, pl = threadIdx.x >> 4;
     const int c = min(blockIdx.x * 16 + cl, C - 1);
     const bool ok = blockIdx.x * 16 + cl < C;
-    const float* pa = a + c;
-    const float* pb = b + c;
+    const float* __restrict__ pa = o.pa + c;
+    const float* __restrict__ pb = o.pb + c;
     float xa0 = 0.f, xa1 = 0.f, xb0 = 0.f, xb1 = 0.f;
     int r = pl;
     for (; r + 3 * WPL < P; r += 4 * WPL) {
@@ -483,46 +501,93 @@
     const float sa = wide_reduce(red, xa0 + xa1, pl, cl);
     const float sb = wide_reduce(red, xb0 + xb1, pl, cl);
     if (pl == 0 && ok) {
-        dbeta[c] = sa; dgamma[c] = sb;
-        c1[c] = sa / (float)M; c2[c] = sb / (float)M;
-    }
-}
-
-template <int MODE, bool EMITG>
+        o.dbeta[c] = sa; o.dgamma[c] = sb;
+        o.c1[c] = sa / (float)M; o.c2[c] = sb / (float)M;
+    }
+}
+
+struct BwdCoef { f32x4 mu, is, c1, c2, gis; };
+__device__ __forceinline__ BwdCoef bwd_coef(const f32x4* __restrict__ mean, const f32x4* __restrict__ invstd, const f32x4* __restrict__ gamma,
+                                            const f32x4* __restrict__ c1, const f32x4* __restrict__ c2, int c4) {
+    BwdCoef k;
+    k.mu = mean[c4]; k.is = invstd[c4]; k.c1 = c1[c4]; k.c2 = c2[c4];
+    k.gis = gamma[c4] * k.is;
+    return k;
+}
+__device__ __forceinline__ f32x4 bwd_elem(f32x4 gv, f32x4 yv, const BwdCoef& k) {
+    const f32x4 xh = (yv - k.mu) * k.is;
+    return (gv - k.c1 - xh * k.c2) * k.gis;
+}
+template <int MODE, bool EMITG, int GEO>
 __global__ __launch_bounds__(NT) void k_bn_bwd_apply(const f32x4* dA , const void* __restrict__ msk,
                                                     const f32x4* __restrict__ y, const f32x4* __restrict__ mean,
                                                     const f32x4* __restrict__ invstd, const f32x4* __restrict__ gamma,
                                                     const f32x4* __restrict__ c1, const f32x4* __restrict__ c2,
                                                     f32x4* dy, f32x4* __restrict__ gout, size_t n4, int c4n, PoolSrc ps) {
     const size_t nq = (n4 + NT - 1) / NT;
+    const int tid = threadIdx.x;
+    BwdCoef k0 = {}, k1 = {};
+    if (GEO == 1) k0 = bwd_coef(mean, invstd, gamma, c1, c2, tid % c4n);
+    if (GEO == 2) { k0 = bwd_coef(mean, invstd, gamma, c1, c2, tid); k1 = bwd_coef(mean, invstd, gamma, c1, c2, NT + tid); }
     for (size_t q = blockIdx.x; q < nq; q += gridDim.x) {
-        const size_t i = ((OSI_BN_REVERSE & 2) ? nq - 1 - q : q) * NT + threadIdx.x;
+        const size_t t = (OSI_BN_REVERSE & 2) ? nq - 1 - q : q;
+        const size_t i = t * NT + tid;
         if (i >= n4) continue;
-        int c4 = (int)(i % (size_t)c4n);
+        const int c4 = GEO == 1 ? tid % c4n : GEO == 2 ? (int)(t & 1) * NT + tid : (int)(i % (size_t)c4n);
         f32x4 gv = MODE == 3 ? pool_gather(dA, ps, (uint32_t)(i / (size_t)c4n), c4, c4n) : masked<MODE>(__builtin_nontemporal_load(dA + i), msk, i);
-        f32x4 is = invstd[c4];
-        f32x4 xh = (__builtin_nontemporal_load(y + i) - mean[c4]) * is;
-        f32x4 r = (gv - c1[c4] - xh * c2[c4]) * (gamma[c4] * is);
+        const BwdCoef k = GEO == 1 ? k0 : GEO == 2 ? ((t & 1) ? k1 : k0) : bwd_coef(mean, invstd, gamma, c1, c2, c4);
+        f32x4 r = bwd_elem(gv, __builtin_nontemporal_load(y + i), k);
         if (EMITG) gout[i] = gv;
         dy[i] = r;
     }
 }
 
-template <int MODE, bool EMITG, bool TWO>
+struct BwdApplyCons { const f32x4 *y, *mean, *invstd, *gamma, *c1, *c2; f32x4* dy; };
+template <int GEO>
+__global__ __launch_bounds__(NT) void k_bn_bwd_apply2(const f32x4* g, BwdApplyCons a, BwdApplyCons b, size_t n4, int c4n) {
+    const size_t nq = (n4 + NT - 1) / NT;
+    const int tid = threadIdx.x;
+    const size_t tfirst = (OSI_BN_REVERSE & 2) ? nq - 1 - blockIdx.x : blockIdx.x;
+    const int ck = GEO == 1 ? tid % c4n : (int)(tfirst & 1) * NT + tid;
+    BwdCoef a0 = {}, b0 = {};
+    if (GEO != 0) { a0 = bwd_coef(a.mean, a.invstd, a.gamma, a.c1, a.c2, ck); b0 = bwd_coef(b.mean, b.invstd, b.gamma, b.c1, b.c2, ck); }
+    for (size_t q = blockIdx.x; q < nq; q += gridDim.x) {
+        const size_t t = (OSI_BN_REVERSE & 2) ? nq - 1 - q : q;
+        const size_t i = t * NT + tid;
+        if (i >= n4) continue;
+        const f32x4 gv = __builtin_nontemporal_load(g + i);
+        const f32x4 ya = __builtin_nontemporal_load(a.y + i), yb = __builtin_nontemporal_load(b.y + i);
+        const BwdCoef ka = GEO != 0 ? a0 : bwd_coef(a.mean, a.invstd, a.gamma, a.c1, a.c2, (int)(i % (size_t)c4n));
+        const BwdCoef kb = GEO != 0 ? b0 : bwd_coef(b.mean, b.invstd, b.gamma, b.c1, b.c2, (int)(i % (size_t)c4n));
+        const f32x4 ra = bwd_elem(gv, ya, ka), rb = bwd_elem(gv, yb, kb);
+        b.dy[i] = rb;
+        a.dy[i] = ra;
+    }
+}
+
+template <int MODE, bool EMITG, bool TWO, int GEO>
 __global__ __launch_bounds__(NT) void k_bn_frozen_apply(const f32x4* dA, const void* __restrict__ msk, const f32x4* __restrict__ scale0,
                                                        const f32x4* __restrict__ scale1, f32x4* dy0, f32x4* __restrict__ dy1,
                                                        f32x4* __restrict__ gout, size_t n4, int c4n, PoolSrc ps) {
     const size_t nq = (n4 + NT - 1) / NT;
+    const int tid = threadIdx.x;
+    f32x4 s00 = {}, s01 = {}, s10 = {}, s11 = {};
+    if (GEO == 1) { s00 = scale0[tid % c4n]; if (TWO) s10 = scale1[tid % c4n]; }
+    if (GEO == 2) { s00 = scale0[tid]; s01 = scale0[NT + tid]; if (TWO) { s10 = scale1[tid]; s11 = scale1[NT + tid]; } }
     for (size_t q = blockIdx.x; q < nq; q += gridDim.x) {
-        const size_t i = ((OSI_BN_REVERSE & 2) ? nq - 1 - q : q) * NT + threadIdx.x;
+        const size_t t = (OSI_BN_REVERSE & 2) ? nq - 1 - q : q;
+        const size_t i = t * NT + tid;
         if (i >= n4) continue;
-        const int c4 = (int)(i % (size_t)c4n);
+        const int c4 = GEO == 1 ? tid % c4n : GEO == 2 ? (int)(t & 1) * NT + tid : (int)(i % (size_t)c4n);
         const f32x4 gv = MODE == 3 ? pool_gather(dA, ps, (uint32_t)(i / (size_t)c4n), c4, c4n) : masked<MODE>(__builtin_nontemporal_load(dA + i), msk, i);
         if (EMITG) gout[i] = gv;
-        if (TWO) dy1[i] = gv * scale1[c4];
-        dy0[i] = gv * scale0[c4];
-    }
-}
+        if (TWO) dy1[i] = gv * (GEO == 1 ? s10 : GEO == 2 ? ((t & 1) ? s11 : s10) : scale1[c4]);
+        dy0[i] = gv * (GEO == 1 ? s00 : GEO == 2 ? ((t & 1) ? s01 : s00) : scale0[c4]);
+    }
+}
+
+static int stream_geo(int c4n) { return NT % c4n == 0 ? 1 : c4n == 2 * NT ? 2 : 0; }
+#define OSI_BY_GEO(geo_, X_) do { if ((geo_) == 1) { X_(1); } else if ((geo_) == 2) { X_(2); } else { X_(0); } } while (0)
 
 static int rows_per_block(int M, int C, int& P) {
     long rows = (256l * 1024) / ((long)C * 4);
@@ -655,7 +720,9 @@
     auto Y = (const f32x4*)y; auto R = (const f32x4*)residual; auto S = (const f32x4*)scale; auto H = (const f32x4*)shift;
     auto RS = (const f32x4*)rscale; auto RH = (const f32x4*)rshift;
     auto O = (f32x4*)out; auto B = (u64*)bits;
-#define OSI_APPLY(RES_, RELU_, BITS_) hipLaunchKernelGGL((k_bn_apply<RES_, RELU_, BITS_>), dim3(grid), dim3(NT), 0, st, Y, R, S, H, RS, RH, O, B, n4, c4n)
+    const int geo = stream_geo(c4n);
+#define OSI_APPLY_G(RES_, RELU_, BITS_, GEO_) hipLaunchKernelGGL((k_bn_apply<RES_, RELU_, BITS_, GEO_>), dim3(grid), dim3(NT), 0, st, Y, R, S, H, RS, RH, O, B, n4, c4n)
+#define OSI_APPLY(RES_, RELU_, BITS_) do { if (geo == 1) OSI_APPLY_G(RES_, RELU_, BITS_, 1); else if (geo == 2) OSI_APPLY_G(RES_, RELU_, BITS_, 2); else OSI_APPLY_G(RES_, RELU_, BITS_, 0); } while (0)
     if (rscale) OSI_APPLY(2, true, true);
     else if (bits && residual) OSI_APPLY(1, true, true);
     else if (bits) OSI_APPLY(0, true, true);
@@ -664,6 +731,7 @@
     else if (relu) OSI_APPLY(0, true, false);
     else OSI_APPLY(0, false, false);
 #undef OSI_APPLY
+#undef OSI_APPLY_G
     OSI_LAUNCH_CHECK();
     return OSI_OK;
 }
@@ -689,6 +757,12 @@
                             const float* res_shift, float* out, void* relu_mask, int M, int C, osi_stream_t stream) {
     OSI_REQUIRE(relu_mask && res_y && res_scale && res_shift);
     return bn_apply_impl(y, res_y, scale, shift, out, relu_mask, M, C, 1, (hipStream_t)stream, res_scale, res_shift);
+}
+
+static BwdConsTable one_cons(const float* pa, const float* pb, float* ga, float* gb, float* dgamma, float* dbeta, float* c1, float* c2) {
+    BwdConsTable t{};
+    t.k[0] = BwdCons{pa, pb, ga, gb, dgamma, dbeta, c1, c2};
+    return t;
 }
 
 static int bn_backward_impl(const float* dout, const void* msk, int mode, const float* y, const float* mean, const float* invstd,
@@ -708,7 +782,7 @@
     else if (mode == 1) hipLaunchKernelGGL(k_bn_bwd_partial<1>, dim3(P), dim3(NT), 0, st, dout, msk, y, mean, invstd, M, C, rpb, pdb, pdg, ps);
     else hipLaunchKernelGGL(k_bn_bwd_partial<0>, dim3(P), dim3(NT), 0, st, dout, msk, y, mean, invstd, M, C, rpb, pdb, pdg, ps);
     OSI_LAUNCH_CHECK();
-    hipLaunchKernelGGL(k_bn_bwd_final, dim3(osi_cdiv(C, NT / 64)), dim3(NT), 0, st, pdb, pdg, P, M, C, dgamma, dbeta, c1, c2);
+    hipLaunchKernelGGL(k_bn_bwd_final, dim3(osi_cdiv(C, NT / 64)), dim3(NT), 0, st, one_cons(pdb, pdg, nullptr, nullptr, dgamma, dbeta, c1, c2), false, P, M, C);
     OSI_LAUNCH_CHECK();
     if (!dy) return OSI_OK;
     const size_t n4 = (size_t)M * C / 4;
@@ -717,29 +791,36 @@
     auto MU = (const f32x4*)mean; auto IS = (const f32x4*)invstd; auto G = (const f32x4*)gamma;
     auto C1 = (const f32x4*)c1; auto C2 = (const f32x4*)c2;
     auto DY = (f32x4*)dy; auto GO = (f32x4*)gmasked;
-#define OSI_BWD_APPLY(MODE_, EMIT_) hipLaunchKernelGGL((k_bn_bwd_apply<MODE_, EMIT_>), dim3(grid), dim3(NT), 0, st, D, msk, Y, MU, IS, G, C1, C2, DY, GO, n4, c4n, ps)
-    if (mode == 3) OSI_BWD_APPLY(3, false);
+    const int geo = stream_geo(c4n);
+#define OSI_BWD_APPLY_G(MODE_, EMIT_, GEO_) hipLaunchKernelGGL((k_bn_bwd_apply<MODE_, EMIT_, GEO_>), dim3(grid), dim3(NT), 0, st, D, msk, Y, MU, IS, G, C1, C2, DY, GO, n4, c4n, ps)
+#define OSI_BWD_APPLY(MODE_, EMIT_) do { if (geo == 1) OSI_BWD_APPLY_G(MODE_, EMIT_, 1); else if (geo == 2) OSI_BWD_APPLY_G(MODE_, EMIT_, 2); else OSI_BWD_APPLY_G(MODE_, EMIT_, 0); } while (0)
+    if (mode == 3) OSI_BWD_APPLY_G(3, false, 0);
     else if (mode == 2) { if (gmasked) OSI_BWD_APPLY(2, true); else OSI_BWD_APPLY(2, false); }
     else if (mode == 1) { if (gmasked) OSI_BWD_APPLY(1, true); else OSI_BWD_APPLY(1, false); }
     else { if (gmasked) OSI_BWD_APPLY(0, true); else OSI_BWD_APPLY(0, false); }
 #undef OSI_BWD_APPLY
-    OSI_LAUNCH_CHECK();
-    return OSI_OK;
-}
-
-static int bwd_reduce_partials(const float* psum_g, const float* psum_gx, int P, int M, int C, float* gb, float* gg, int S, int Pc,
-                               float* dgamma, float* dbeta, float* c1, float* c2, hipStream_t st) {
+#undef OSI_BWD_APPLY_G
+    OSI_LAUNCH_CHECK();
+    return OSI_OK;
+}
+
+static int bwd_reduce_partials(const BwdConsTable& t, int n, int P, int M, int C, int S, int Pc, hipStream_t st) {
     if (P <= g_osi_tuning.bn_wide_p) {
-        hipLaunchKernelGGL(k_bn_bwd_final_wide, dim3(osi_cdiv(C, 16)), dim3(16 * WPL), 0, st, psum_g, psum_gx, P, M, C, dgamma, dbeta, c1, c2);
+        hipLaunchKernelGGL(k_bn_bwd_final_wide, dim3(osi_cdiv(C, 16), n), dim3(16 * WPL), 0, st, t, P, M, C);
         OSI_LAUNCH_CHECK();
         return OSI_OK;
     }
-    hipLaunchKernelGGL(k_colsum2_group, dim3(osi_cdiv(C, 16), S), dim3(NT), 0, st, psum_g, psum_gx, P, Pc, C, S, gb, gg);
-    OSI_LAUNCH_CHECK();
-    hipLaunchKernelGGL(k_bn_bwd_final, dim3(osi_cdiv(C, NT / 64)), dim3(NT), 0, st, (const float*)gb, (const float*)gg, S, M, C, dgamma,
-                       dbeta, c1, c2);
-    OSI_LAUNCH_CHECK();
-    return OSI_OK;
+    hipLaunchKernelGGL(k_colsum2_group, dim3(osi_cdiv(C, 16), S, n), dim3(NT), 0, st, t, P, Pc, C, S);
+    OSI_LAUNCH_CHECK();
+    hipLaunchKernelGGL(k_bn_bwd_final, dim3(osi_cdiv(C, NT / 64), n), dim3(NT), 0, st, t, true, S, M, C);
+    OSI_LAUNCH_CHECK();
+    return OSI_OK;
+}
+static void bwd_groups(int P, int& S, int& Pc) {
+    S = osi_cdiv(P, 64);
+    if (S > OSI_BN_GROUPS) S = OSI_BN_GROUPS;
+    Pc = osi_cdiv(P, S);
+    S = osi_cdiv(P, Pc);
 }
 
 int osi_bn_backward_fused(const float* g, const float* y, const float* mean, const float* invstd, const float* gamma,
@@ -747,21 +828,65 @@
                           void* ws, size_t ws_bytes, osi_stream_t stream) {
     OSI_REQUIRE(g && y && mean && invstd && gamma && psum_g && psum_gx && dy && dgamma && dbeta && ws);
     OSI_REQUIRE(M > 0 && C > 0 && C % 4 == 0 && P > 0);
-    int S = osi_cdiv(P, 64);
-    if (S > OSI_BN_GROUPS) S = OSI_BN_GROUPS;
-    const int Pc = osi_cdiv(P, S);
-    S = osi_cdiv(P, Pc);
+    int S, Pc;
+    bwd_groups(P, S, Pc);
     OSI_REQUIRE(ws_bytes >= ((size_t)2 * S * C + 2 * (size_t)C) * sizeof(float));
     hipStream_t st = (hipStream_t)stream;
     float* gb = (float*)ws;
     float* gg = gb + (size_t)S * C;
     float* c1 = gg + (size_t)S * C;
     float* c2 = c1 + C;
-    if (int e = bwd_reduce_partials(psum_g, psum_gx, P, M, C, gb, gg, S, Pc, dgamma, dbeta, c1, c2, st)) return e;
+    if (int e = bwd_reduce_partials(one_cons(psum_g, psum_gx, gb, gg, dgamma, dbeta, c1, c2), 1, P, M, C, S, Pc, st)) return e;
     const size_t n4 = (size_t)M * C / 4;
-    hipLaunchKernelGGL((k_bn_bwd_apply<0, false>), dim3(stream_grid(n4, true)), dim3(NT), 0, st, (const f32x4*)g, (const void*)nullptr,
-                       (const f32x4*)y, (const f32x4*)mean, (const f32x4*)invstd, (const f32x4*)gamma, (const f32x4*)c1,
-                       (const f32x4*)c2, (f32x4*)dy, (f32x4*)nullptr, n4, C / 4, PoolSrc{});
+    const int c4n = C / 4;
+#define OSI_FUSED_APPLY(GEO_) hipLaunchKernelGGL((k_bn_bwd_apply<0, false, GEO_>), dim3(stream_grid(n4, true)), dim3(NT), 0, st, (const f32x4*)g, \
+                       (const void*)nullptr, (const f32x4*)y, (const f32x4*)mean, (const f32x4*)invstd, (const f32x4*)gamma, (const f32x4*)c1, \
+                       (const f32x4*)c2, (f32x4*)dy, (f32x4*)nullptr, n4, c4n, PoolSrc{})
+    OSI_BY_GEO(stream_geo(c4n), OSI_FUSED_APPLY);
+#undef OSI_FUSED_APPLY
+    OSI_LAUNCH_CHECK();
+    return OSI_OK;
+}
+
+size_t osi_bn_backward_fused2_workspace(int C) {
+    if (C <= 0) return 0;
+    return 2 * ((size_t)2 * OSI_BN_GROUPS * C + 2 * (size_t)C) * sizeof(float);
+}
+
+int osi_bn_backward_fused2(const float* g, const osi_bn_fused_consumer* consumers, const float* psum_g, int P, int M, int C, void* ws,
+                           size_t ws_bytes, osi_stream_t stream) {
+    OSI_REQUIRE(g && consumers && psum_g && ws && M > 0 && C > 0 && C % 4 == 0 && P > 0);
+    for (int k = 0; k < 2; ++k) {
+        const osi_bn_fused_consumer& c = consumers[k];
+        OSI_REQUIRE(c.y && c.mean && c.invstd && c.gamma && c.psum_gx && c.dy && c.dgamma && c.dbeta);
+    }
+    OSI_REQUIRE(consumers[1].dy != consumers[0].dy && consumers[1].dy != g);
+    OSI_REQUIRE(ws_bytes >= osi_bn_backward_fused2_workspace(C));
+    int S, Pc;
+    bwd_groups(P, S, Pc);
+    hipStream_t st = (hipStream_t)stream;
+    const size_t per = (size_t)2 * OSI_BN_GROUPS * C + 2 * (size_t)C;
+    BwdConsTable t{};
+    BwdApplyCons a[2];
+    for (int k = 0; k < 2; ++k) {
+        const osi_bn_fused_consumer& c = consumers[k];
+        float* gb = (float*)ws + k * per;
+        float* gg = gb + (size_t)S * C;
+        float* c1 = gg + (size_t)S * C;
+        float* c2 = c1 + C;
+        t.k[k] = BwdCons{psum_g, c.psum_gx, gb, gg, c.dgamma, c.dbeta, c1, c2};
+        a[k] = BwdApplyCons{(const f32x4*)c.y, (const f32x4*)c.mean, (const f32x4*)c.invstd, (const f32x4*)c.gamma, (const f32x4*)c1,
+                            (const f32x4*)c2, (f32x4*)c.dy};
+    }
+    if (int e = bwd_reduce_partials(t, 2, P, M, C, S, Pc, st)) return e;
+    const size_t n4 = (size_t)M * C / 4;
+    const int c4n = C / 4;
+    const int grid = stream_grid(n4, true);
+    int geo = stream_geo(c4n);
+    if (geo == 2 && (grid & 1) && (size_t)grid < (n4 + NT - 1) / NT) geo = 0;
+#define OSI_FUSED_APPLY2(GEO_) hipLaunchKernelGGL((k_bn_bwd_apply2<GEO_>), dim3(grid), dim3(NT), 0, st, (const f32x4*)g, a[0], a[1], n4, c4n)
+    OSI_BY_GEO(geo, OSI_FUSED_APPLY2);
+#undef OSI_FUSED_APPLY2
     OSI_LAUNCH_CHECK();
     return OSI_OK;
 }
@@ -769,17 +894,15 @@
 int osi_bn_backward_reduce(const float* psum_g, const float* psum_gx, int P, float* dgamma, float* dbeta, int M, int C, void* ws,
                            size_t ws_bytes, osi_stream_t stream) {
     OSI_REQUIRE(psum_g && psum_gx && dgamma && dbeta && ws && M > 0 && C > 0 && P > 0);
-    int S = osi_cdiv(P, 64);
-    if (S > OSI_BN_GROUPS) S = OSI_BN_GROUPS;
-    const int Pc = osi_cdiv(P, S);
-    S = osi_cdiv(P, Pc);
+    int S, Pc;
+    bwd_groups(P, S, Pc);
     OSI_REQUIRE(ws_bytes >= ((size_t)2 * S * C + 2 * (size_t)C) * sizeof(float));
     hipStream_t st = (hipStream_t)stream;
     float* gb = (float*)ws;
     float* gg = gb + (size_t)S * C;
     float* c1 = gg + (size_t)S * C;
     float* c2 = c1 + C;
-    if (int e = bwd_reduce_partials(psum_g, psum_gx, P, M, C, gb, gg, S, Pc, dgamma, dbeta, c1, c2, st)) return e;
+    if (int e = bwd_reduce_partials(one_cons(psum_g, psum_gx, gb, gg, dgamma, dbeta, c1, c2), 1, P, M, C, S, Pc, st)) return e;
     return OSI_OK;
 }
 
@@ -807,15 +930,17 @@
         else if (mode == 2) hipLaunchKernelGGL(k_bn_bwd_partial<2>, dim3(P), dim3(NT), 0, st, dout, msk, cs[k].y, cs[k].mean, cs[k].invstd, M, C, rpb, pdb, pdg, ps);
         else hipLaunchKernelGGL(k_bn_bwd_partial<0>, dim3(P), dim3(NT), 0, st, dout, msk, cs[k].y, cs[k].mean, cs[k].invstd, M, C, rpb, pdb, pdg, ps);
         OSI_LAUNCH_CHECK();
-        hipLaunchKernelGGL(k_bn_bwd_final, dim3(osi_cdiv(C, NT / 64)), dim3(NT), 0, st, pdb, pdg, P, M, C, cs[k].dgamma, cs[k].dbeta, c1, c1 + C);
+        hipLaunchKernelGGL(k_bn_bwd_final, dim3(osi_cdiv(C, NT / 64)), dim3(NT), 0, st, one_cons(pdb, pdg, nullptr, nullptr, cs[k].dgamma, cs[k].dbeta, c1, c1 + C), false, P, M, C);
         OSI_LAUNCH_CHECK();
     }
     const size_t n4 = (size_t)M * C / 4;
     const int grid = stream_grid(n4, true), c4n = C / 4;
     auto D = (const f32x4*)dout; auto S0 = (const f32x4*)cs[0].scale; auto S1 = (const f32x4*)(n == 2 ? cs[1].scale : nullptr);
     auto DY0 = (f32x4*)cs[0].dy; auto DY1 = (f32x4*)(n == 2 ? cs[1].dy : nullptr); auto GO = (f32x4*)gmasked;
-#define OSI_FRZ_APPLY(MODE_, EMIT_, TWO_) hipLaunchKernelGGL((k_bn_frozen_apply<MODE_, EMIT_, TWO_>), dim3(grid), dim3(NT), 0, st, D, msk, S0, S1, DY0, DY1, GO, n4, c4n, ps)
-    if (mode == 3) OSI_FRZ_APPLY(3, false, false);
+    const int geo = stream_geo(c4n);
+#define OSI_FRZ_APPLY_G(MODE_, EMIT_, TWO_, GEO_) hipLaunchKernelGGL((k_bn_frozen_apply<MODE_, EMIT_, TWO_, GEO_>), dim3(grid), dim3(NT), 0, st, D, msk, S0, S1, DY0, DY1, GO, n4, c4n, ps)
+#define OSI_FRZ_APPLY(MODE_, EMIT_, TWO_) do { if (geo == 1) OSI_FRZ_APPLY_G(MODE_, EMIT_, TWO_, 1); else if (geo == 2) OSI_FRZ_APPLY_G(MODE_, EMIT_, TWO_, 2); else OSI_FRZ_APPLY_G(MODE_, EMIT_, TWO_, 0); } while (0)
+    if (mode == 3) OSI_FRZ_APPLY_G(3, false, false, 0);
     else if (mode == 2) {
         if (n == 2) { if (gmasked) OSI_FRZ_APPLY(2, true, true); else OSI_FRZ_APPLY(2, false, true); }
         else { if (gmasked) OSI_FRZ_APPLY(2, true, false); else OSI_FRZ_APPLY(2, false, false); }
@@ -824,6 +949,7 @@
         else { if (gmasked) OSI_FRZ_APPLY(0, true, false); else OSI_FRZ_APPLY(0, false, false); }
     }
 #undef OSI_FRZ_APPLY
+#undef OSI_FRZ_APPLY_G
     OSI_LAUNCH_CHECK();
     return OSI_OK;
 }
diff --git a/openset-imagenet_amd/csrc/resnet50_exec.hip b/openset-imagenet_amd/csrc/resnet50_exec.hip
--- a/openset-imagenet_amd/csrc/resnet50_exec.hip
+++ b/openset-imagenet_amd/csrc/resnet50_exec.hip
@@ -65,7 +65,7 @@
     size_t param_floats = 0, buffer_floats = 0, ws_floats = 0;
     int t_fc_w, t_fc_b, t_lg_w, t_lg_b;
     int Hs, Ws, Hp, Wp;
-    size_t x4, wpack, gpack, a_pool, pool_idx, pooled, feat, logits_ws;
+    size_t x4, wpack, gpack, a_pool, pool_idx, pooled, feat;
     size_t bn_ws, bn_ws2, bn_ws_bytes, wg_ws, wg_ws_bytes, dg_ws, dg_ws_bytes;
     size_t stem_ws = 0, stem_ws_bytes = 0;
     size_t wino_ws = 0, wino_ws_bytes = 0;
@@ -288,7 +288,6 @@
     n->stage_hi[0] = n->param_floats;
     n->pooled = n->ws_alloc((size_t)B * 2048);
     n->feat = n->ws_alloc((size_t)B * fc_dim);
-    n->logits_ws = n->ws_alloc((size_t)B * out_features);
     n->dfeat = n->ws_alloc((size_t)B * fc_dim);
     n->dpooled = n->ws_alloc((size_t)B * 2048);
     size_t maxact = 0, bnws = 0, wgws = 0, dgws = 0, winows = 0;
@@ -302,6 +301,8 @@
         if (b2 > bnws) bnws = b2;
         size_t b3 = osi_conv_fwd_bnstats_workspace(&c.d);
         if (b3 > bnws) bnws = b3;
+        size_t b4 = osi_bn_backward_fused2_workspace(c.d.Cout);
+        if (b4 > bnws) bnws = b4;
         size_t wg = osi_conv_wgrad_workspace(&c.d);
         if (wg > wgws) wgws = wg;
         wg = osi_stem_wgrad_direct_workspace(&c.d);
@@ -485,10 +486,8 @@
     const Tensor& fw = n->tensors[n->t_fc_w]; const Tensor& fb = n->tensors[n->t_fc_b]; const Tensor& lw = n->tensors[n->t_lg_w];
     OSI_TRY(osi_linear_fwd(ws + n->pooled, params + fw.off, params + fb.off, ws + n->feat, n->B, 2048, n->F, st));
     const float* lb = n->t_lg_b >= 0 ? params + n->tensors[n->t_lg_b].off : nullptr;
-    OSI_TRY(osi_linear_fwd(ws + n->feat, params + lw.off, lb, ws + n->logits_ws, n->B, n->F, n->O, st));
+    OSI_TRY(osi_linear_fwd(ws + n->feat, params + lw.off, lb, logits, n->B, n->F, n->O, st));
     if (hipMemcpyAsync(features, ws + n->feat, (size_t)n->B * n->F * sizeof(float), hipMemcpyDeviceToDevice, st) != hipSuccess)
-        return OSI_ERR_LAUNCH;
-    if (hipMemcpyAsync(logits, ws + n->logits_ws, (size_t)n->B * n->O * sizeof(float), hipMemcpyDeviceToDevice, st) != hipSuccess)
         return OSI_ERR_LAUNCH;
     return OSI_OK;
 }
@@ -763,6 +762,22 @@
     return OSI_OK;
 }
 
+static int bn_bwd_fused_pair(osi_resnet50* n, int ci, int cj, const float* params, float* grads, float* ws, int gi, int dyi, int dyj,
+                             hipStream_t st) {
+    const float* psum_g = ws + n->dg_ws;
+    osi_bn_fused_consumer cs[2];
+    const int idx[2] = {ci, cj}, out[2] = {dyi, dyj};
+    for (int k = 0; k < 2; ++k) {
+        Conv& c = n->convs[idx[k]];
+        BN& b = n->bns[c.bn];
+        cs[k] = osi_bn_fused_consumer{ws + c.y, ws + b.mean, ws + b.invstd, params + b.g_off, psum_g + (size_t)(1 + k) * n->fused_P * b.C,
+                                      ws + n->scratch[out[k]], n->dgam(grads, ws, b), n->dbet(grads, ws, b)};
+    }
+    BN& b = n->bns[n->convs[ci].bn];
+    OSI_TRY(osi_bn_backward_fused2(ws + n->scratch[gi], cs, psum_g, n->fused_P, b.M, b.C, ws + n->bn_ws, n->bn_ws_bytes, st));
+    return n->mark(OSI_PROF_BN_BWD, st);
+}
+
 static int bn_reduce_frozen(osi_resnet50* n, int ci, float* grads, float* ws, int which, hipStream_t st) {
     if (!n->bw_pg) return OSI_OK;
     BN& b = n->bns[n->convs[ci].bn];
@@ -873,7 +888,10 @@
             Conv& cd = n->convs[k.ds];
             int t1 = n->take(st);
             if (t1 < 0) return t1;
-            OSI_TRY(bn_bwd_fused(n, k.ds, params, grads, ws, go, t1, 1, st));
+            d3 = n->take(st);
+            if (d3 < 0) return d3;
+            OSI_TRY(bn_bwd_fused_pair(n, k.c3, k.ds, params, grads, ws, go, d3, t1, st));
+            n->give(go);
             OSI_TRY(wgrad(n, k.ds, grads, ws, t1, x, st));
             if (!no_dx) {
                 dxbase = n->take(st);
@@ -881,12 +899,12 @@
                 OSI_TRY(dgrad_plain(n, &cd.d, S(t1), params + cd.w_off, S(dxbase), ds_sparse ? 2 : 0, st));
             }
             n->give(t1);
-        }
-        d3 = n->take(st);
-        if (d3 < 0) return d3;
-        OSI_TRY(bn_bwd_fused(n, k.c3, params, grads, ws, go, d3, 0, st));
-        if (has_ds) n->give(go);
-        else dxbase = go;
+        } else {
+            d3 = n->take(st);
+            if (d3 < 0) return d3;
+            OSI_TRY(bn_bwd_fused(n, k.c3, params, grads, ws, go, d3, 0, st));
+            dxbase = go;
+        }
     } else {
         dxbase = n->take(st);
         if (dxbase < 0) return dxbase;
diff --git a/openset-imagenet_amd/openset_imagenet/_native.py b/openset-imagenet_amd/openset_imagenet/_native.py
--- a/openset-imagenet_amd/openset_imagenet/_native.py
+++ b/openset-imagenet_amd/openset_imagenet/_native.py
@@ -39,6 +39,11 @@
 class BnFrozenConsumer(Structure):
     _fields_ = [("y", c_void_p), ("mean", c_void_p), ("invstd", c_void_p), ("scale", c_void_p), ("dy", c_void_p), ("dgamma", c_void_p),
                 ("dbeta", c_void_p)]
+
+
+class BnFusedConsumer(Structure):
+    _fields_ = [("y", c_void_p), ("mean", c_void_p), ("invstd", c_void_p), ("gamma", c_void_p), ("psum_gx", c_void_p), ("dy", c_void_p),
+                ("dgamma", c_void_p), ("dbeta", c_void_p)]
 
 
 class OptSegment(Structure):
@@ -93,6 +98,8 @@
     "osi_conv_dgrad_fused": (c_int, [_PD, P, P, P, P, P, c_int, POINTER(c_int), P]),
     "osi_bn_backward_reduce": (c_int, [P, P, c_int, P, P, c_int, c_int, P, c_size_t, P]),
     "osi_bn_backward_fused": (c_int, [P, P, P, P, P, P, P, c_int, P, P, P, c_int, c_int, P, c_size_t, P]),
+    "osi_bn_backward_fused2_workspace": (c_size_t, [c_int]),
+    "osi_bn_backward_fused2": (c_int, [P, P, P, c_int, c_int, c_int, P, c_size_t, P]),
     "osi_conv_wgrad_workspace": (c_size_t, [_PD]),
     "osi_conv_wgrad": (c_int, [_PD, P, P, P, P, c_size_t, P]),
     "osi_stem_weight_pack": (c_int, [P, P, c_int, P]),
```
